# LunaJang/Metabuli_work

Hardware: AMD Instinct MI355X
Metric: reads/sec classified (150bp & 10kb) vs GTDB-scale DB at 1/2/4/8 MI355X (higher is better)
Workload: dtype u64

## Files before the change

metabuli_work_amd/csrc/mtb_api.hip:

```cpp
#include <chrono>
#include <cmath>
#include <cstdio>
#include <cstring>
#include <string>
#include <vector>
#include <algorithm>
#include <memory>
#include <charconv>
#include <mutex>
#include <unordered_map>

#include "mtb_host.h"
#include "mtb_launch.h"
#include <cstdlib>

using namespace mtb;

#define HIP_TRY(x)                                                                                   \
    do {                                                                                             \
        hipError_t e_ = (x);                                                                         \
        if (e_ != hipSuccess) {                                                                      \
            set_error(std::string("HIP error ") + hipGetErrorString(e_) + " at " #x);                 \
            return e_ == hipErrorOutOfMemory ? MTB_ERR_OOM : MTB_ERR_HIP;                            \
        }                                                                                            \
    } while (0)

namespace {

struct WsBudget {
    size_t cap = 0;
    size_t used = 0;
    double grow = 1.0;
};

struct DevBuf {
    void* p = nullptr;
    size_t bytes = 0;
    WsBudget* budget = nullptr;
    hipError_t ensure(size_t need) {
        if (need <= bytes) return hipSuccess;
        static const bool trace = getenv("MTB_ALLOC_TRACE") != nullptr;
        const auto t0 = std::chrono::steady_clock::now();
        const size_t old = bytes;
        if (p) hipFree(p);
        const auto t1 = std::chrono::steady_clock::now();
        p = nullptr;
        if (budget) budget->used -= bytes;
        bytes = 0;
        size_t b = need + need / 8 + 256;
        hipError_t e = hipErrorOutOfMemory;
        if (budget && budget->grow > 1.125) {
            const size_t big = (size_t)((double)need * budget->grow) + 256;
            if (!budget->cap || budget->used + big <= budget->cap) {
                e = hipMalloc(&p, big);
                if (e == hipSuccess) b = big;
                else (void)hipGetLastError();
            }
        }
        if (e != hipSuccess) {
            if (budget && budget->cap && budget->used + b > budget->cap) return hipErrorOutOfMemory;
            e = hipMalloc(&p, b);
        }
        if (e == hipSuccess) bytes = b;
        if (e == hipSuccess && budget) budget->used += b;
        if (trace) {
            const auto t2 = std::chrono::steady_clock::now();
            const double f = std::chrono::duration<double>(t1 - t0).count(), m = std::chrono::duration<double>(t2 - t1).count();
            if (f + m > 0.02) fprintf(stderr, "[alloc] %.3f GB -> %.3f GB: free %.3f s, malloc %.3f s\n", old * 1e-9, b * 1e-9, f, m);
        }
        return e;
    }
    void release() {
        if (!p) return;
        hipFree(p);
        p = nullptr;
        if (budget) budget->used -= bytes;
        bytes = 0;
    }
    DevBuf() = default;
    DevBuf(const DevBuf&) = delete;
    DevBuf& operator=(const DevBuf&) = delete;
    ~DevBuf() { release(); }
    template <typename T>
    T* as() const { return (T*)p; }
};

struct DbArrays {
    int device = 0;
    std::vector<void*> own;
    ~DbArrays() {
        hipSetDevice(device);
        for (void* p : own)
            if (p) hipFree(p);
    }
};

}

struct mtb_ctx {
    int device = 0;
    mtb_params par{};
    hipStream_t stream = nullptr;
    bool ownStream = false;
    HostTables tables{};
    uint64_t D = 0;
    DbRec* db = nullptr;
    bool borrowedDb = false;
    std::shared_ptr<DbArrays> dbArrays;
    uint64_t* dirMem = nullptr;
    ProbeLine* lines = nullptr;
    uint64_t* lineP = nullptr;
    uint16_t* runOff = nullptr;
    ProbeExt* lineExt = nullptr;
    uint64_t* link = nullptr;
    AADir dir{};
    uint64_t rankLo = 0, rankHi = ~0ull;
    int joinMode = 0;
    uint64_t* tileRec = nullptr;
    uint32_t* tilePre = nullptr;
    uint64_t nTiles = 0;
    uint32_t sweepNom = 2048;
    uint32_t sweepLdsCap = ~0u;
    bool sweepSmall = false;
    bool filterThreadMajor = false;
    int sweepPersist = 1;
    uint32_t matchWinCap = ~0u;
    bool directJoin = true;
    bool directRetry = false;
    int pruneAfter = 2;
    int bigGroups = 1;
    bool fuseFilter = true;
    bool radixDigits = true;
    bool radixAtomicFirst = false;
    int binnedSort = 0;
    uint64_t binRcForce = 0;
    bool binDigits = true;
    bool uniformUnits = true;
    uint32_t upr = 0;
    uint64_t binHost[kSortBins] = {};
    bool noFilter = false;
    uint32_t spillShift = 0;
    bool sparse = false;
    uint32_t maxW = 0;
    int sortLoFine = kQuerySortLoFine;
    bool forceGeneric = false;
    bool segsortGlobal = false;
    uint32_t mergeSeg = 0;
    int waveTaxon = -1;
    int emulateAll = 0;
    bool pruneCompact = true;
    bool noAlias = false;
    uint64_t aliasBytes = 0;
    int32_t* spOf = nullptr;
    int32_t maxTax = 0;
    int32_t *tNodeOf = nullptr, *tNodeTax = nullptr, *tParent = nullptr, *tDepth = nullptr, *tSpParent = nullptr;
    uint8_t* tFlags = nullptr;
    uint32_t cladePerMatch = 2;
    std::vector<int32_t> hNodeOf;
    std::vector<std::string> hRank;
    HostTaxonomy hTax;
    mutable std::vector<std::string> lineage;
    mutable std::once_flag lineageOnce;
    std::shared_ptr<void> pipelineCache;
    mutable mtb::TaxText taxText;
    mutable std::once_flag taxTextOnce;
    WsBudget ws;
    DevBuf seq1, off1, seq2, off2, meta, reserve, slotOff, qlen, scanTmp;
    DevBuf keysA, valsA, keysB, valsB, radixCounts, radixOffs;
    DevBuf readCnt, mOff, matches, matchesSorted, segScratch, maxSeg, errFlag;
    DevBuf ordKA, ordVA, ordKB, ordVB, matchWin, unitRead, unitInfo, mStage, mRank, mTotal, mDirect, ovFlag, waveList, waveCount, devStats;
    DevBuf qFrom, probeStats;
    DevBuf longList, longCnt;
    DevBuf qStart;
    uint32_t longCap = 0;
    DevBuf chunkIn, chunkCnt, chunkSrcOff;
    DevBuf liveCnt, liveOff;
    DevBuf segLen;
    DevBuf sizeLists;
    DevBuf digA, digB;
    DevBuf binCnt, binTab;
    DevBuf maskOut1, maskOut2, maskProb, maskScale;
    DevBuf readLens;
    DevBuf readCnt64;
    uint64_t liveM = 0;
    double openS[8] = {0, 0, 0, 0, 0, 0, 0, 0};
    static constexpr int kNumStats = 20;
    uint64_t stats[kNumStats] = {};
    uint32_t chunkC = 1;
    uint64_t stageRegion = 0;
    uint64_t spillCap = 0;
    DevBuf emMap, emCnt, emScratch, emPacked, emCnt32, emOff;
    bool emValid = false;
    bool emPackedValid = false;
    std::vector<mtb_em_map> emHost;
    std::vector<uint32_t> spKmers;
    std::string dbDir;
    DevBuf local, paths, comb, conn, spScore, spKeep,
        gFlag, sFlag, pathCnt, gScan, sScan, gStart, sStart, clade, tcPool, tcLen, tcOff, tcOut, results;
    uint32_t nReads = 0;
    uint64_t Q = 0, M = 0, nTaxcnt = 0;
    uint64_t Qall = 0;
    double presentShare = 0.5;
    const uint64_t* qKeys = nullptr;
    const uint32_t* qSlots = nullptr;
    bool keepStages = false;
    bool probed = false;
    bool matchOnly = false;
    float stageMs[5] = {0, 0, 0, 0, 0};
    hipEvent_t ev[6]{};
    static constexpr int kNumKern = 7;
    float kernMs[kNumKern] = {0, 0, 0, 0, 0, 0, 0};
    hipEvent_t kev[2 * kNumKern]{};
};

static std::vector<DevBuf*> batch_bufs(mtb_ctx* c);

static void bind_workspace(mtb_ctx* c, size_t cap) {
    c->ws.cap = cap;
    if (const char* e = getenv("MTB_WORKSPACE_CAP")) {
        char* end = nullptr;
        double v = strtod(e, &end);
        const char u = end ? *end : 0;
        v *= u == 'G' || u == 'g' ? 1e9 : u == 'M' || u == 'm' ? 1e6 : u == 'K' || u == 'k' ? 1e3 : 1.0;
        c->ws.cap = v > 0 ? (size_t)v : 0;
    }
    for (DevBuf* b : batch_bufs(c)) b->budget = &c->ws;
}

static void free_db(mtb_ctx* c) {
    if (c->dbArrays) {
        c->dbArrays.reset();
        c->db = nullptr;
        c->dirMem = nullptr;
        c->lines = nullptr;
        c->lineP = nullptr;
        c->runOff = nullptr;
        c->lineExt = nullptr;
        c->link = nullptr;
        return;
    }
    if (c->borrowedDb) c->db = nullptr;
    void* ptrs[] = {c->db, c->dirMem, c->lines, c->lineP, c->runOff, c->lineExt, c->link, c->spOf, c->tNodeOf, c->tNodeTax, c->tParent, c->tDepth, c->tSpParent, c->tFlags};
    for (void* p : ptrs)
        if (p) hipFree(p);
    c->db = nullptr;
    c->dirMem = nullptr;
    c->lines = nullptr;
    c->lineP = nullptr;
    c->runOff = nullptr;
    c->lineExt = nullptr;
    c->link = nullptr;
}

template <typename T>
static hipError_t upload(T** dst, const std::vector<T>& v, hipStream_t s) {
    hipError_t e = hipMalloc((void**)dst, std::max<size_t>(1, v.size()) * sizeof(T));
    if (e != hipSuccess) return e;
    if (!v.empty()) e = hipMemcpyAsync(*dst, v.data(), v.size() * sizeof(T), hipMemcpyHostToDevice, s);
    return e;
}

static int validate_params(const mtb_params* p) {
    if (p->reduced_aa) { set_error("reduced-AA DBs (ReducedKmerMatcher) are out of scope"); return MTB_ERR_UNSUPPORTED; }
    if (p->em && p->db_parts > 1) { set_error("--em needs the whole DB in one context"); return MTB_ERR_UNSUPPORTED; }
    if (p->mask_mode && !(p->mask_prob > 0.0f && p->mask_prob <= 1.0f)) { set_error("mask_prob must be in (0, 1]"); return MTB_ERR_ARG; }
    if (p->kmer_format != 1 && p->kmer_format != 2) { set_error("kmer_format must be 1 or 2"); return MTB_ERR_UNSUPPORTED; }
    if (p->syncmer && p->kmer_format != 2) { set_error("syncmer requires kmer_format 2"); return MTB_ERR_UNSUPPORTED; }
    if (p->syncmer && (p->smer_len < 1 || p->smer_len > 8)) { set_error("smer_len must be in [1, 8]"); return MTB_ERR_ARG; }
    if (p->seq_mode < 1 || p->seq_mode > 3) { set_error("seq_mode must be 1, 2 or 3"); return MTB_ERR_ARG; }
    return MTB_OK;
}

static double since(std::chrono::steady_clock::time_point& t) {
    const auto now = std::chrono::steady_clock::now();
    const double d = std::chrono::duration<double>(now - t).count();
    t = now;
    return d;
}

static int decode_db_chunked(mtb_ctx* c, HostDb& db, uint32_t mask, hipStream_t s) {
    const uint64_t nDiff = db.nDiff, D = c->D;
    uint64_t W = 1ull << 30;
    if (const char* e = getenv("MTB_DECODE_CHUNK_WORDS")) W = std::max<uint64_t>(8, strtoull(e, nullptr, 10));
    W = std::max<uint64_t>(std::min(W, nDiff), 1);
    DevBuf dDiff, dFlag, dIdx, dTmp, dVal, dInfo;
    HIP_TRY(dDiff.ensure(W * sizeof(uint16_t)));
    HIP_TRY(dFlag.ensure(W * sizeof(uint32_t)));
    HIP_TRY(dIdx.ensure((W + 2) * sizeof(uint64_t)));
    HIP_TRY(dTmp.ensure(scan_tmp_elems(W) * sizeof(uint64_t)));
    HIP_TRY(dVal.ensure(W * sizeof(uint64_t)));
    HIP_TRY(dInfo.ensure(W * sizeof(uint32_t)));
    auto a0 = std::chrono::steady_clock::now();
    HIP_TRY(hipMalloc(&c->db, (D + kDbPad) * sizeof(DbRec)));
    c->openS[7] = since(a0);
    const bool fromFile = !db.diffFile.empty();
    double upS = 0;
    auto l0 = std::chrono::steady_clock::now();
    StageLanes lanes(c->device);
    upS += since(l0);
    uint64_t w0 = 0, k0 = 0, carry = 0, seen = 0;
    HIP_TRY(hipStreamSynchronize(s));
    while (w0 < nDiff) {
        const uint64_t n = std::min(W, nDiff - w0);
        auto u0 = std::chrono::steady_clock::now();
        const bool got = fromFile ? read_to_device(db.diffFile, dDiff.p, n * sizeof(uint16_t), w0 * sizeof(uint16_t), &lanes)
                                  : upload_to_device(db.diffP + w0, dDiff.p, n * sizeof(uint16_t), &lanes);
        if (!got) return MTB_ERR_IO;
        upS += since(u0);
        uint64_t lastTerm = 0, lastValue = 0;
        const uint64_t terms = decode_diff_chunk(dDiff.as<uint16_t>(), n, carry, dVal.as<uint64_t>(),
                                                 dFlag.as<uint32_t>(), dIdx.as<uint64_t>(), dTmp.p, &lastTerm,
                                                 &lastValue, s);
        HIP_TRY(hipGetLastError());
        const bool lastChunk = w0 + n == nDiff;
        if (terms == 0) {
            set_error("diffIdx ends mid k-mer");
            return MTB_ERR_DB;
        }
        if (lastChunk && lastTerm != n - 1) {
            set_error("diffIdx ends mid k-mer");
            return MTB_ERR_DB;
        }
        seen += terms;
        if (seen <= D) {
            u0 = std::chrono::steady_clock::now();
            const bool gotInfo = fromFile ? read_to_device(db.infoFile, dInfo.p, terms * sizeof(uint32_t),
                                                           k0 * sizeof(uint32_t), &lanes)
                                          : upload_to_device(db.infoP + k0, dInfo.p, terms * sizeof(uint32_t), &lanes);
            if (!gotInfo) return MTB_ERR_IO;
            upS += since(u0);
            launch_mask_info(dInfo.as<uint32_t>(), terms, mask, s);
            if (c->par.kmer_format == 2) launch_to_rank_form(dVal.as<uint64_t>(), terms, s);
            launch_pack_db(dVal.as<uint64_t>(), dInfo.as<uint32_t>(), terms, c->db + k0, s);
            HIP_TRY(hipStreamSynchronize(s));
            k0 += terms;
        }
        carry = lastValue;
        w0 += lastTerm + 1;
    }
    if (seen != D) {
        set_error("diffIdx k-mer count " + std::to_string(seen) + " != info entries " + std::to_string(D));
        return MTB_ERR_DB;
    }
    c->openS[0] += upS;
    return MTB_OK;
}

static int open_into(mtb_ctx* c, HostDb& db, const mtb_params* par, int device, const mtb_db_resident* res,
                     double readS, std::chrono::steady_clock::time_point t0) {
    auto tp = t0;
    c->device = device;
// ... 163 lines not shown
        if (!res->records || res->n_kmers < 2) { set_error("resident DB needs >= 2 k-mers"); return MTB_ERR_DB; }
    } else {
        if (!check_db(db)) return MTB_ERR_DB;
        if (db.nInfo < 2) { set_error("DB has fewer than 2 k-mers"); return MTB_ERR_DB; }
        if (par->db_parts > 1 && !slice_db_part(db, par->db_part, par->db_parts)) return MTB_ERR_DB;
    }
    mtb_ctx* c = new mtb_ctx();
    rc = open_into(c, db, par, device, res, readS, t0);
    if (rc != MTB_OK) {
        const std::string msg = mtb_last_error();
        mtb_close(c);
        set_error(msg);
        return rc;
    }
    *out = c;
    return MTB_OK;
}

extern "C" {

int mtb_open(const char* db_dir, const mtb_params* par, int device, mtb_ctx** out) {
    if (!db_dir || !par || !out) { set_error("null argument"); return MTB_ERR_ARG; }
    HostDb db;
    const auto t0 = std::chrono::steady_clock::now();
    if (!load_db_files(db_dir, db, par->db_parts <= 1)) return MTB_ERR_IO;
    const double readS = std::chrono::duration<double>(std::chrono::steady_clock::now() - t0).count();
    const int rc = open_common(db, par, device, out, nullptr, readS);
    if (rc == MTB_OK) (*out)->dbDir = db_dir;
    return rc;
}

int mtb_open_host(const mtb_db_host* h, const mtb_params* par, int device, mtb_ctx** out) {
    if (!h || !par || !out) { set_error("null argument"); return MTB_ERR_ARG; }
    HostDb db;
    if (par->db_parts > 1) {
        db.diffIdx.assign(h->diff_idx, h->diff_idx + h->n_diff_idx);
        db.info.assign(h->info, h->info + h->n_info);
        db.use_vectors();
    } else {
        db.diffP = h->diff_idx;
        db.nDiff = h->n_diff_idx;
        db.infoP = h->info;
        db.nInfo = h->n_info;
    }
    if (h->split) db.split.assign(h->split, h->split + 3 * h->n_split);
    db.taxIdList.assign(h->taxid_list, h->taxid_list + h->n_taxid_list);
    std::vector<std::string> ranks(h->n_nodes), names(h->n_nodes);
    for (uint64_t i = 0; i < h->n_nodes; i++) {
        ranks[i] = h->rank_pool + h->rank_off[i];
        if (h->name_pool) names[i] = h->name_pool + h->name_off[i];
    }
    if (!build_taxonomy(h->node_taxid, h->node_parent, h->n_nodes, ranks, names, h->merged_old, h->merged_new,
                        h->n_merged, db.tax) ||
        !build_species_map(db))
        return MTB_ERR_DB;
    return open_common(db, par, device, out);
}

int mtb_open_resident(const mtb_db_resident* r, const mtb_db_host* h, const mtb_params* par, int device,
                      mtb_ctx** out) {
    if (!r || !h || !par || !out) { set_error("null argument"); return MTB_ERR_ARG; }
    HostDb db;
    db.taxIdList.assign(h->taxid_list, h->taxid_list + h->n_taxid_list);
    std::vector<std::string> ranks(h->n_nodes), names(h->n_nodes);
    for (uint64_t i = 0; i < h->n_nodes; i++) {
        ranks[i] = h->rank_pool + h->rank_off[i];
        if (h->name_pool) names[i] = h->name_pool + h->name_off[i];
    }
    if (!build_taxonomy(h->node_taxid, h->node_parent, h->n_nodes, ranks, names, h->merged_old, h->merged_new,
                        h->n_merged, db.tax) ||
        !build_species_map(db))
        return MTB_ERR_DB;
    return open_common(db, par, device, out, r);
}

int mtb_clone(const mtb_ctx* src, mtb_ctx** out) {
    if (!src || !out) { set_error("null argument"); return MTB_ERR_ARG; }
    mtb_ctx* c = new mtb_ctx();
    c->device = src->device;
    c->par = src->par;
    c->tables = src->tables;
    HIP_TRY(hipSetDevice(c->device));
    HIP_TRY(hipStreamCreateWithFlags(&c->stream, hipStreamNonBlocking));
    c->ownStream = true;
    for (auto& e : c->ev) HIP_TRY(hipEventCreate(&e));
    for (auto& e : c->kev) HIP_TRY(hipEventCreate(&e));
    c->dbArrays = src->dbArrays;
    c->D = src->D;
    c->db = src->db;
    c->borrowedDb = src->borrowedDb;
    c->dirMem = src->dirMem;
    c->lines = src->lines;
    c->lineP = src->lineP;
    c->runOff = src->runOff;
    c->lineExt = src->lineExt;
    c->link = src->link;
    c->dir = src->dir;
    c->rankLo = src->rankLo;
    c->rankHi = src->rankHi;
    c->spOf = src->spOf;
    c->maxTax = src->maxTax;
    c->tNodeOf = src->tNodeOf;
    c->tNodeTax = src->tNodeTax;
    c->tParent = src->tParent;
    c->tDepth = src->tDepth;
    c->tSpParent = src->tSpParent;
    c->tFlags = src->tFlags;
    c->cladePerMatch = src->cladePerMatch;
    c->hNodeOf = src->hNodeOf;
    c->hRank = src->hRank;
    c->hTax = src->hTax;
    c->dbDir = src->dbDir;
    c->spKmers = src->spKmers;
    c->joinMode = src->joinMode;
    c->sweepNom = src->sweepNom;
    c->sweepLdsCap = src->sweepLdsCap;
    c->sweepSmall = src->sweepSmall;
    c->filterThreadMajor = src->filterThreadMajor;
    c->sweepPersist = src->sweepPersist;
    c->matchWinCap = src->matchWinCap;
    c->directJoin = src->directJoin;
    c->directRetry = src->directRetry;
    c->pruneAfter = src->pruneAfter;
    c->bigGroups = src->bigGroups;
    c->fuseFilter = src->fuseFilter;
    c->presentShare = src->presentShare;
    c->spillShift = src->spillShift;
    c->sortLoFine = src->sortLoFine;
    c->forceGeneric = src->forceGeneric;
    c->segsortGlobal = src->segsortGlobal;
    c->mergeSeg = src->mergeSeg;
    c->waveTaxon = src->waveTaxon;
    c->emulateAll = src->emulateAll;
    c->pruneCompact = src->pruneCompact;
    c->noAlias = src->noAlias;
    c->noFilter = src->noFilter;
    c->radixDigits = src->radixDigits;
    c->radixAtomicFirst = src->radixAtomicFirst;
    c->binnedSort = src->binnedSort;
    c->binRcForce = src->binRcForce;
    c->binDigits = src->binDigits;
    c->uniformUnits = src->uniformUnits;
    bind_workspace(c, src->ws.cap);
    *out = c;
    return MTB_OK;
}

#define MTB_BATCH_BUFS(X) \
    X(seq1) X(off1) X(seq2) X(off2) X(meta) X(reserve) X(slotOff) X(qlen) X(scanTmp) X(keysA) X(valsA) X(keysB) \
    X(valsB) X(radixCounts) X(radixOffs) X(readCnt) X(mOff) X(matches) X(matchesSorted) X(segScratch) X(maxSeg) \
    X(errFlag) X(ordKA) X(ordVA) X(ordKB) X(ordVB) X(matchWin) X(unitRead) X(unitInfo) X(waveList) X(waveCount) \
    X(devStats) X(mStage) X(mRank) X(mDirect) X(ovFlag) X(mTotal) X(qFrom) X(probeStats) X(longList) X(longCnt) \
    X(qStart) X(chunkIn) X(chunkCnt) X(chunkSrcOff) X(liveCnt) X(liveOff) X(segLen) X(sizeLists) X(digA) \
    X(digB) X(binCnt) X(binTab) X(local) X(paths) X(comb) X(conn) X(spScore) X(spKeep) X(gFlag) X(sFlag) \
    X(pathCnt) X(gScan) X(sScan) X(gStart) X(sStart) X(clade) X(tcPool) X(tcLen) X(tcOff) X(tcOut) X(results) \
    X(emMap) X(emCnt) X(emScratch) X(emPacked) X(emCnt32) X(emOff) X(maskOut1) X(maskOut2) X(maskProb) \
    X(maskScale) X(readLens) X(readCnt64)
static std::vector<DevBuf*> batch_bufs(mtb_ctx* c) {
#define MTB_BUF_PTR(n) &c->n,
    return {MTB_BATCH_BUFS(MTB_BUF_PTR)};
#undef MTB_BUF_PTR
}

static const char* const* batch_buf_names() {
#define MTB_BUF_NAME(n) #n,
    static const char* const names[] = {MTB_BATCH_BUFS(MTB_BUF_NAME)};
#undef MTB_BUF_NAME
    return names;
}

void mtb_close(mtb_ctx* c) {
    if (!c) return;
    hipSetDevice(c->device);
    if (c->stream) hipStreamSynchronize(c->stream);
    free_db(c);
    if (c->tileRec) hipFree(c->tileRec);
    if (c->tilePre) hipFree(c->tilePre);
    c->pipelineCache.reset();
    hipSetDevice(c->device);
    for (DevBuf* b : batch_bufs(c)) b->release();
    for (auto& e : c->ev)
        if (e) hipEventDestroy(e);
    for (auto& e : c->kev)
        if (e) hipEventDestroy(e);
    if (c->ownStream && c->stream) hipStreamDestroy(c->stream);
    delete c;
}

int mtb_set_stream(mtb_ctx* c, void* stream) {
    if (!c) return MTB_ERR_ARG;
    if (c->ownStream && c->stream) hipStreamDestroy(c->stream);
    if (stream) {
        c->stream = (hipStream_t)stream;
        c->ownStream = false;
    } else {
        HIP_TRY(hipStreamCreateWithFlags(&c->stream, hipStreamNonBlocking));
        c->ownStream = true;
    }
    return MTB_OK;
}

uint64_t mtb_db_kmers(const mtb_ctx* c) { return c ? c->D : 0; }

uint64_t mtb_workspace_bytes(const mtb_ctx* c) { return c ? c->ws.used : 0; }

int mtb_open_phases(const mtb_ctx* c, double* sec, int n) {
    if (!c || !sec) return MTB_ERR_ARG;
    for (int i = 0; i < n && i < 8; i++) sec[i] = c->openS[i];
    return MTB_OK;
}

int mtb_set_workspace_cap(mtb_ctx* c, uint64_t bytes) {
    if (!c) return MTB_ERR_ARG;
    c->ws.cap = bytes;
    return MTB_OK;
}

int mtb_release_workspace(mtb_ctx* c) {
    if (!c) return MTB_ERR_ARG;
    mtb::ctx_release_workspace(c);
    void* p = nullptr;
    if (hipMalloc(&p, 64u << 20) == hipSuccess) hipFree(p);
    return hipDeviceSynchronize() == hipSuccess ? MTB_OK : MTB_ERR_HIP;
}

int mtb_ctx_device(const mtb_ctx* c) { return c ? c->device : 0; }

}

static AssignArgs assign_args(const mtb_params& p) {
    AssignArgs a;
    a.em = p.em ? 1 : 0;
    a.kmerFormat = p.kmer_format;
    if (p.syncmer) {
        a.dnaShift = (8 - p.smer_len) * 3;
        a.maxCodonShift = 8 - p.smer_len;
    } else {
        a.dnaShift = 3;
        a.maxCodonShift = 1;
    }
    a.denominator = (p.seq_mode == 1 || p.seq_mode == 2) ? 100 : 1000;
    a.minConsCnt = p.min_cons_cnt;
    a.minConsCntEuk = p.min_cons_cnt_euk;
    a.accessionLevel = p.accession_level;
    a.minScore = p.min_score;
    a.minSpScore = p.min_sp_score;
    a.tieRatio = p.tie_ratio;
    a.generic = 0;
    return a;
}

static int assign_stage(mtb_ctx* c, uint32_t n, bool keep) {
    hipStream_t s = c->stream;
    HIP_TRY(c->errFlag.ensure(sizeof(int)));
    const uint64_t M = c->M;
    AssignArgs a = assign_args(c->par);
    a.generic = c->forceGeneric ? 1 : 0;
    a.waveTaxon = c->waveTaxon;
    a.bigGroups = c->bigGroups;
    a.emulateAll = c->emulateAll;
    if (a.dnaShift <= 0) { set_error("syncmer smer_len 8 gives a zero dnaShift"); return MTB_ERR_ARG; }
    HIP_TRY(c->readCnt.ensure(sizeof(uint32_t) * (n + 1)));
    const uint64_t Mc = std::max<uint64_t>(M, 1);
    HIP_TRY(c->results.ensure(sizeof(mtb_result) * std::max<uint32_t>(n, 1)));
    HIP_TRY(c->matchesSorted.ensure(sizeof(mtb_match) * Mc));
    HIP_TRY(c->maxSeg.ensure(sizeof(uint32_t)));
    launch_max_seg(c->mOff.as<uint64_t>(), n, c->maxSeg.as<uint32_t>(), s);
    uint32_t maxSeg = 0;
    HIP_TRY(hipMemcpyAsync(&maxSeg, c->maxSeg.p, sizeof(uint32_t), hipMemcpyDeviceToHost, s));
    HIP_TRY(hipStreamSynchronize(s));
    const bool prune = !keep && !c->forceGeneric;
    if (maxSeg > kSegSortLds || c->forceGeneric || c->segsortGlobal || (c->mergeSeg && maxSeg > c->mergeSeg))
        HIP_TRY(c->segScratch.ensure(6 * sizeof(uint64_t) * Mc));
    const bool compact = prune && maxSeg > kSegSortRegs && !c->segsortGlobal && c->pruneCompact;
    if (compact) HIP_TRY(c->segLen.ensure(sizeof(uint32_t) * (n + 1)));
    if (maxSeg > 128) HIP_TRY(c->sizeLists.ensure(sizeof(uint32_t) * (4 * (size_t)n + 4)));
    c->keepStages = !prune;
    HIP_TRY(c->liveCnt.ensure(sizeof(uint32_t) * (n + 1)));
    HIP_TRY(c->liveOff.ensure(sizeof(uint64_t) * (n + 1)));
    HIP_TRY(c->scanTmp.ensure(sizeof(uint64_t) * scan_tmp_elems(n + 1)));
    HIP_TRY(hipEventRecord(c->kev[10], s));
    if (c->sparse && (!prune || (maxSeg > kSegSortSparse && !compact) || c->segsortGlobal ||
                      (c->mergeSeg && maxSeg > c->mergeSeg))) {
        launch_compact_segments(c->mDirect.as<SegMatch>(), c->slotOff.as<uint64_t>(), c->chunkC,
                                c->mOff.as<uint64_t>(), n, c->matches.as<mtb_match>(), c->spillShift, s,
                                c->stats[13] ? 2 : 0);
        c->sparse = false;
    }
    HIP_TRY(launch_segsort(c->matches.as<mtb_match>(), c->mOff.as<uint64_t>(), n, Mc, c->matchesSorted.as<mtb_match>(),
                           c->segScratch.as<uint64_t>(), maxSeg, c->forceGeneric || c->segsortGlobal,
                           prune ? c->liveCnt.as<uint32_t>() : nullptr, c->mergeSeg,
                           prune_min_matches(a.minConsCnt, a.minConsCntEuk, a.maxCodonShift), s,
                           c->sparse ? c->mDirect.as<SegMatch>() : nullptr, c->slotOff.as<uint64_t>(),
                           c->chunkC | c->spillShift << 16,
                           compact ? c->segLen.as<uint32_t>() : nullptr,
                           c->maxSeg.as<uint32_t>(), c->pruneAfter, maxSeg > 128 ? c->sizeLists.as<uint32_t>() : nullptr));
    c->sparse = false;
    const mtb_match* kIn = c->matchesSorted.as<mtb_match>();
    const uint64_t* kOff = c->mOff.as<uint64_t>();
    uint64_t kM = M;
    if (prune) {
        exclusive_scan_u32(c->liveCnt.as<uint32_t>(), n, c->liveOff.as<uint64_t>(), c->scanTmp.p, s);
        HIP_TRY(hipMemcpyAsync(&kM, c->liveOff.as<uint64_t>() + n, sizeof(uint64_t), hipMemcpyDeviceToHost, s));
        launch_pack_live(c->matchesSorted.as<mtb_match>(), c->mOff.as<uint64_t>(), c->liveOff.as<uint64_t>(), n,
                         c->matches.as<mtb_match>(), c->errFlag.as<int>(), s);
        HIP_TRY(hipStreamSynchronize(s));
        if (kM > M) { set_error("internal error: K5 kept more matches than it sorted"); return MTB_ERR_INTERNAL; }
        kIn = c->matches.as<mtb_match>();
        kOff = c->liveOff.as<uint64_t>();
    }
    c->liveM = kM;
    c->stats[11] = kM;
    const uint64_t Kc = std::max<uint64_t>(kM, 1);
    const uint64_t Mn = std::max<uint64_t>(Kc, n);
    std::vector<std::pair<char*, size_t>> dead;
    if (!c->noAlias) {
        std::vector<DevBuf*> d = {&c->mDirect, &c->segScratch, &c->mStage, &c->mRank, &c->matchWin, &c->chunkIn};
        if (prune) {
            for (DevBuf* b : {&c->matchesSorted, &c->keysA, &c->valsA, &c->keysB, &c->valsB}) d.push_back(b);
        } else {
            d.push_back(&c->matches);
        }
        for (DevBuf* b : d)
            if (b->p && b->bytes >= (1u << 20)) dead.push_back({b->as<char>(), b->bytes});
        std::sort(dead.begin(), dead.end(), [](auto& a, auto& b) { return a.second > b.second; });
    }
    struct Need {
        DevBuf* own;
        uint64_t bytes;
        void* p;
    };
    Need need[] = {{&c->local, path_bytes() * Kc, nullptr},
                   {&c->paths, path_bytes() * Kc, nullptr},
                   {&c->comb, path_bytes() * Kc, nullptr},
                   {&c->conn, Kc, nullptr},
                   {&c->spScore, sizeof(float) * Kc, nullptr},
                   {&c->spKeep, Kc, nullptr},
                   {&c->waveList, sizeof(uint64_t) * Kc, nullptr},
                   {&c->gFlag, sizeof(uint32_t) * (Kc + 1), nullptr},
                   {&c->pathCnt, sizeof(uint32_t) * (Kc + 1), nullptr},
                   {&c->sFlag, std::max<uint64_t>(sizeof(uint32_t) * (Kc + 1), run_index_tmp_bytes(Kc)), nullptr},
                   {&c->gScan, sizeof(uint64_t) * (Kc + 1), nullptr},
                   {&c->sScan, sizeof(uint64_t) * (Kc + 1), nullptr},
                   {&c->gStart, sizeof(uint64_t) * (Kc + 1), nullptr},
                   {&c->sStart, sizeof(uint64_t) * (Kc + 1), nullptr},
                   {&c->clade, clade_bytes() * Kc * c->cladePerMatch, nullptr},
                   {&c->tcPool, sizeof(mtb_taxcnt) * Kc, nullptr},
                   {&c->ordKA, sizeof(uint64_t) * (Mn + 1), nullptr},
                   {&c->ordVA, sizeof(uint64_t) * (Mn + 1), nullptr},
                   {&c->ordKB, sizeof(uint64_t) * (Mn + 1), nullptr},
                   {&c->ordVB, sizeof(uint64_t) * (Mn + 1), nullptr}};
    std::vector<Need*> order;
    for (Need& x : need) order.push_back(&x);
    std::stable_sort(order.begin(), order.end(), [](Need* a, Need* b) { return a->bytes > b->bytes; });
    c->aliasBytes = 0;
    for (Need* x : order) {
        const size_t b = (x->bytes + 255) & ~(size_t)255;
        for (auto& r : dead)
            if (r.second >= b) {
                x->p = r.first;
                r.first += b;
                r.second -= b;
                c->aliasBytes += b;
                break;
            }
        if (!x->p) {
            HIP_TRY(x->own->ensure(x->bytes));
            x->p = x->own->p;
        }
    }
    HIP_TRY(c->waveCount.ensure(sizeof(uint32_t)));
    HIP_TRY(hipEventRecord(c->kev[11], s));
    HIP_TRY(hipEventRecord(c->kev[12], s));
    HIP_TRY(c->radixCounts.ensure(sizeof(uint32_t) * radix_counts_elems(Mn + 1)));
    HIP_TRY(c->radixOffs.ensure(sizeof(uint64_t) * (radix_counts_elems(Mn + 1) + 1)));
    HIP_TRY(c->scanTmp.ensure(sizeof(uint64_t) * scan_tmp_elems(radix_counts_elems(Mn + 1) + n + Mn + 2)));
    TaxDevice t{c->tNodeOf, c->tNodeTax, c->tParent, c->tDepth, c->tFlags, c->tSpParent, c->maxTax};
    AssignScratch sc{need[0].p,
                     need[1].p,
                     need[2].p,
                     (uint8_t*)need[3].p,
                     (uint32_t*)need[7].p,
                     (uint32_t*)need[9].p,
                     (uint32_t*)need[8].p,
                     (uint64_t*)need[10].p,
                     (uint64_t*)need[11].p,
                     (uint64_t*)need[12].p,
                     (uint64_t*)need[13].p,
                     (float*)need[4].p,
                     (uint64_t*)need[6].p,
                     c->waveCount.as<uint32_t>(),
                     (uint8_t*)need[5].p,
                     c->scanTmp.p,
                     (uint64_t*)need[16].p,
                     (uint64_t*)need[17].p,
                     (uint64_t*)need[18].p,
                     (uint64_t*)need[19].p,
                     c->radixCounts.as<uint32_t>(),
                     c->radixOffs.as<uint64_t>(),
                     need[14].p,
                     c->cladePerMatch};
    mtb_taxcnt* tcPool = (mtb_taxcnt*)need[15].p;
    c->stats[3] = M;
    c->stats[4] = maxSeg;
    launch_assign(kIn, kOff, c->qlen.as<uint32_t>(), n, kM, a, t, sc, tcPool,
                  c->results.as<mtb_result>(), c->devStats.as<unsigned long long>(), c->stats + 5, s);
    HIP_TRY(hipEventRecord(c->kev[13], s));
    HIP_TRY(c->tcLen.ensure(sizeof(uint32_t) * (n + 1)));
    HIP_TRY(c->tcOff.ensure(sizeof(uint64_t) * (n + 1)));
    launch_taxcnt_len(c->results.as<mtb_result>(), n, c->tcLen.as<uint32_t>(), s);
    exclusive_scan_u32(c->tcLen.as<uint32_t>(), n, c->tcOff.as<uint64_t>(), c->scanTmp.p, s);
    uint64_t NT = 0;
    HIP_TRY(hipMemcpyAsync(&NT, c->tcOff.as<uint64_t>() + n, sizeof(uint64_t), hipMemcpyDeviceToHost, s));
    HIP_TRY(hipStreamSynchronize(s));
    HIP_TRY(c->tcOut.ensure(sizeof(mtb_taxcnt) * std::max<uint64_t>(NT, 1)));
    launch_compact_taxcnt(tcPool, kOff, c->results.as<mtb_result>(), c->tcOff.as<uint64_t>(), n,
                          c->tcOut.as<mtb_taxcnt>(), s);
    c->nTaxcnt = NT;
    c->emValid = false;
    c->emPackedValid = false;
    if (c->par.em) {
        const uint64_t nS = std::max<uint64_t>(c->stats[7], 1);
        HIP_TRY(c->emScratch.ensure(8 * nS));
        HIP_TRY(c->emMap.ensure(8 * (uint64_t)kEmTop * std::max<uint32_t>(n, 1)));
        HIP_TRY(c->emCnt.ensure(std::max<uint32_t>(n, 1)));
        launch_em_top(kIn, kOff, n, sc, c->results.as<mtb_result>(), c->emScratch.p, c->emMap.p,
                      c->emCnt.as<uint8_t>(), s);
        HIP_TRY(hipGetLastError());
        c->emValid = true;
    }
    return MTB_OK;
}

static int join_stage(mtb_ctx* c, const uint8_t* dSeq1, const uint64_t* dOff1, const uint8_t* dSeq2,
                      const uint64_t* dOff2, uint32_t n, uint64_t U, uint32_t C, uint64_t R, uint64_t Rc) {
    hipStream_t s = c->stream;
    const bool probe = c->probed;
    const bool filt = c->lines && (!c->noFilter || probe);
    const bool fused = filt && !probe && c->fuseFilter;
    if (!fused) {
        HIP_TRY(c->keysA.ensure(8 * Rc));
        HIP_TRY(c->valsA.ensure(4 * Rc));
        HIP_TRY(c->keysB.ensure(8 * Rc));
        HIP_TRY(c->valsB.ensure(4 * Rc));
    }
    HIP_TRY(c->radixCounts.ensure(sizeof(uint32_t) * radix_counts_elems(Rc)));
    HIP_TRY(c->radixOffs.ensure(sizeof(uint64_t) * (radix_counts_elems(Rc) + 1)));
    HIP_TRY(c->scanTmp.ensure(sizeof(uint64_t) * scan_tmp_elems(radix_counts_elems(Rc) + n + 1)));
    HIP_TRY(c->mTotal.ensure(sizeof(unsigned long long) * kStageRegions));
    HIP_TRY(c->probeStats.ensure(sizeof(unsigned long long) * kProbeStatsLen));
    HIP_TRY(hipMemsetAsync(c->probeStats.p, 0, sizeof(unsigned long long) * kProbeStatsLen, s));
    HIP_TRY(hipEventRecord(c->kev[0], s));
    if (!fused)
        launch_extract(dSeq1, dOff1, dSeq2, dOff2, c->meta.as<ReadMeta>(), c->slotOff.as<uint64_t>(),
                       c->unitRead.as<uint32_t>(), U, C, c->tables, c->par.kmer_format, c->par.syncmer,
                       c->par.smer_len, c->keysA.as<uint64_t>(), c->unitInfo.as<uint64_t>(), s, c->upr);
    HIP_TRY(hipEventRecord(c->kev[1], s));
    uint64_t Q = R;
    const uint64_t* qk = c->keysA.as<uint64_t>();
    const uint32_t* qi = nullptr;
    const uint64_t* qf = nullptr;
    HIP_TRY(hipEventRecord(c->kev[2], s));
    const bool digits = fused && c->radixDigits && c->sortLoFine == kQuerySortLo;
    uint64_t binRc = 0;
    if (fused) {
        uint64_t cap = std::min<uint64_t>(R, (uint64_t)((double)R * c->presentShare) + 4096);
        bool binned = digits && c->binnedSort && (c->binnedSort == 2 || cap >= (1ull << 22));
        for (int pass = 0; pass < 2 && binned; pass++) {
            uint64_t rc = c->binRcForce ? c->binRcForce : (cap + cap / 16) / kSortBins + 256;
            rc = (rc + 63) / 64 * 64;
            const uint64_t slots = rc * kSortBins;
            HIP_TRY(c->keysB.ensure(8 * slots));
            HIP_TRY(c->valsB.ensure(4 * slots));
            HIP_TRY(c->digA.ensure(slots));
            HIP_TRY(c->binCnt.ensure(sizeof(unsigned long long) * kSortBins));
            Q = launch_extract_filter(dSeq1, dOff1, dSeq2, dOff2, c->meta.as<ReadMeta>(), c->slotOff.as<uint64_t>(),
                                      c->unitRead.as<uint32_t>(), U, C, c->tables, c->par.kmer_format, c->par.syncmer,
                                      c->par.smer_len, c->unitInfo.as<uint64_t>(), c->lines, c->keysB.as<uint64_t>(),
                                      c->valsB.as<uint32_t>(), c->mTotal.as<unsigned long long>(), c->rankLo,
                                      c->rankHi, &c->Qall, slots, false, s,
                                      c->binDigits ? c->digA.as<uint8_t>() : nullptr,
                                      c->binCnt.as<unsigned long long>(), rc, c->binHost, c->upr);
            HIP_TRY(hipGetLastError());
            if (R) c->presentShare = std::max(c->presentShare, std::min(1.0, 1.125 * (double)Q / (double)R));
            bool over = false;
            for (int r = 0; r < kSortBins; r++) over |= c->binHost[r] > rc;
            if (!over) {
                binRc = rc;
                break;
            }
            c->stats[15]++;
            cap = std::min<uint64_t>(R, Q + Q / 8);
            binned = false;
        }
        for (int pass = 0; pass < 2 && !binRc; pass++) {
            HIP_TRY(c->keysB.ensure(8 * cap));
            HIP_TRY(c->valsB.ensure(4 * cap));
            if (digits) HIP_TRY(c->digA.ensure(cap));
            cap = std::min<uint64_t>(c->keysB.bytes / 8, c->valsB.bytes / 4);
            if (digits) cap = std::min<uint64_t>(cap, c->digA.bytes);
            Q = launch_extract_filter(dSeq1, dOff1, dSeq2, dOff2, c->meta.as<ReadMeta>(), c->slotOff.as<uint64_t>(),
                                      c->unitRead.as<uint32_t>(), U, C, c->tables, c->par.kmer_format, c->par.syncmer,
                                      c->par.smer_len, c->unitInfo.as<uint64_t>(), c->lines, c->keysB.as<uint64_t>(),
                                      c->valsB.as<uint32_t>(), c->mTotal.as<unsigned long long>(), c->rankLo,
                                      c->rankHi, &c->Qall, cap, c->filterThreadMajor, s,
                                      digits ? c->digA.as<uint8_t>() : nullptr, nullptr, 0, nullptr, c->upr, c->link);
            HIP_TRY(hipGetLastError());
            if (Q == ~0ull) {
                set_error("internal error: K1F sequence stage overflow");
                return MTB_ERR_INTERNAL;
            }
            if (R) c->presentShare = std::max(c->presentShare, std::min(1.0, 1.125 * (double)Q / (double)R));
            if (Q <= cap) break;
            cap = std::min<uint64_t>(R, Q + Q / 8);
            c->stats[15]++;
        }
        HIP_TRY(c->keysA.ensure(8 * std::max<uint64_t>(Q, 1)));
        HIP_TRY(c->valsA.ensure(4 * std::max<uint64_t>(Q, 1)));
        if (digits) HIP_TRY(c->digB.ensure(std::max<uint64_t>(Q, 16)));
        qk = c->keysB.as<uint64_t>();
        qi = c->valsB.as<uint32_t>();
    } else if (filt) {
        if (probe) HIP_TRY(c->qFrom.ensure(8 * Rc + 8 * kDbPad));
        Q = launch_filter(c->keysA.as<uint64_t>(), R, c->lines, c->keysB.as<uint64_t>(), c->valsB.as<uint32_t>(),
                          probe ? c->qFrom.as<uint64_t>() : nullptr, c->mTotal.as<unsigned long long>(), c->rankLo,
                          c->rankHi, &c->Qall, s);
        qk = c->keysB.as<uint64_t>();
        qi = c->valsB.as<uint32_t>();
        qf = c->qFrom.as<uint64_t>();
    }
    HIP_TRY(hipEventRecord(c->kev[3], s));
    HIP_TRY(hipEventRecord(c->ev[1], s));
    HIP_TRY(hipEventRecord(c->kev[4], s));
    const bool sweepJoin = c->joinMode == 3 && !probe && c->directJoin && !c->forceGeneric;
    const int sortLo = !sweepJoin && unstaged_join(c->lines != nullptr, c->D, Q, std::min<uint32_t>(c->matchWinCap, 3072))
                           ? c->sortLoFine : kQuerySortLo;
    if (!probe) {
        bool inB = false;
        if (binRc) {
            HIP_TRY(c->binTab.ensure(sizeof(uint64_t) * std::max<uint64_t>(radix_binned_tiles(c->binHost, binRc), 1)));
            const uint64_t rcn = radix_counts_elems(Q) + 256ull * kSortBins;
            HIP_TRY(c->radixCounts.ensure(sizeof(uint32_t) * rcn));
            HIP_TRY(c->radixOffs.ensure(sizeof(uint64_t) * (rcn + 1)));
            HIP_TRY(c->scanTmp.ensure(sizeof(uint64_t) * scan_tmp_elems(rcn + n + 1)));
            Q = radix_sort_binned(c->keysB.as<uint64_t>(), c->valsB.as<uint32_t>(), c->keysA.as<uint64_t>(),
                                  c->valsA.as<uint32_t>(), c->binHost, c->binCnt.as<unsigned long long>(), binRc,
                                  kQuerySortLo, kQuerySortHi, c->radixCounts.as<uint32_t>(),
                                  c->radixOffs.as<uint64_t>(), c->scanTmp.p, c->binTab.as<uint64_t>(), &inB, s,
                                  c->binDigits ? c->digA.as<uint8_t>() : nullptr, c->digB.as<uint8_t>());
            qk = inB ? c->keysA.as<uint64_t>() : c->keysB.as<uint64_t>();
            qi = inB ? c->valsA.as<uint32_t>() : c->valsB.as<uint32_t>();
        } else if (filt) {
            const bool dg = digits && sortLo == kQuerySortLo;
            Q = radix_sort_pairs(c->keysB.as<uint64_t>(), c->valsB.as<uint32_t>(), c->keysA.as<uint64_t>(),
                                 c->valsA.as<uint32_t>(), Q, sortLo, kQuerySortHi, false, false,
// ... 1175 lines not shown
```

metabuli_work_amd/csrc/mtb_assign.hip:

```cpp
#include <algorithm>
#include <vector>

#include "mtb_launch.h"
#include "mtb_stdsort.h"

namespace mtb {

struct Path {
    int start, end;
    float score;
    int hd, depth;
    uint32_t sm, em;
};

__device__ __forceinline__ void match_key(const mtb_match& m, uint64_t& hi, uint64_t& lo) {
    hi = ((uint64_t)m.species_id << 32) | ((uint64_t)info_frame(m.qinfo) << 29) | (info_pos(m.qinfo) & 0x1FFFFFFFu);
    lo = ((uint64_t)m.hamming << 56) | ((uint64_t)(m.dna_encoding & 0xFFFFFFu) << 32) | m.target_id;
}

__device__ __forceinline__ bool key_gt(uint64_t ah, uint64_t al, uint64_t bh, uint64_t bl) {
    return ah > bh || (ah == bh && al > bl);
}

constexpr int kSmallSeg = 512;
// ... 1351 lines not shown
        for (long i = threadIdx.x; i < (long)surv; i += kLargeThreads) io[base + i] = stage[base + i];
    if (threadIdx.x == 0) segLen[r] = surv;
}

__global__ void __launch_bounds__(256) k_max_seg_len(const uint32_t* __restrict__ segLen, uint32_t n,
                                                     uint32_t* __restrict__ out) {
    uint32_t v = 0;
#pragma unroll
    for (uint32_t k = 0; k < kMaxPer; k++)
        if (max_elem(k) < n && segLen[max_elem(k)] != kSegSkip) v = max(v, segLen[max_elem(k)]);
    block_max_to(v, out);
}

constexpr int kSizeClasses = 4;
constexpr int kSizeListReads = 1024;

__global__ void __launch_bounds__(256) k_size_lists(const uint64_t* __restrict__ mOff, const uint32_t* __restrict__ segLen,
                                                    uint32_t nReads, uint32_t maxSeg, uint32_t* __restrict__ lists,
                                                    uint32_t* __restrict__ counts) {
    __shared__ uint32_t sCnt[kSizeClasses], sBase[kSizeClasses];
    if (threadIdx.x < kSizeClasses) sCnt[threadIdx.x] = 0;
    __syncthreads();
    constexpr int kPer = kSizeListReads / 256;
    int cls[kPer];
    uint32_t at[kPer];
#pragma unroll
    for (int k = 0; k < kPer; k++) {
        const uint32_t r = blockIdx.x * kSizeListReads + k * 256 + threadIdx.x;
        cls[k] = -1;
        at[k] = 0;
        if (r < nReads) {
            const long n = seg_len(mOff, segLen, r);
            cls[k] = n > (long)maxSeg ? -1 : n > kMidSeg ? 3 : n > kSmallSeg ? 2 : n > 256 ? 1 : n > 128 ? 0 : -1;
        }
        if (cls[k] >= 0) at[k] = atomicAdd(&sCnt[cls[k]], 1u);
    }
    __syncthreads();
    if (threadIdx.x < kSizeClasses)
        sBase[threadIdx.x] = sCnt[threadIdx.x] ? atomicAdd(&counts[threadIdx.x], sCnt[threadIdx.x]) : 0u;
    __syncthreads();
#pragma unroll
    for (int k = 0; k < kPer; k++)
        if (cls[k] >= 0)
            lists[(uint64_t)cls[k] * nReads + sBase[cls[k]] + at[k]] = blockIdx.x * kSizeListReads + k * 256 + threadIdx.x;
}

static hipError_t launch_sorts(const mtb_match* in, const uint64_t* mOff, uint32_t nReads, uint64_t M, mtb_match* out,
                               uint64_t* gScratch, uint32_t maxSeg, uint32_t* liveCnt, long chunk, uint32_t pm,
                               const uint32_t* segLen, hipStream_t s, const SegMatch* seg, const uint64_t* inOff,
                               uint32_t inC, int mode, uint32_t* lists) {
    k_segsort_small<<<nReads, 64, 0, s>>>(in, mOff, seg, inOff, inC, nReads, out, liveCnt, pm, segLen);
    if (maxSeg <= 128) return hipGetLastError();
    static const bool useLists = !(getenv("MTB_SIZE_LISTS") && atoi(getenv("MTB_SIZE_LISTS")) == 0);
    if (!useLists || !lists) {
#define MTB_REGS(E, M) k_segsort_regs<E, M><<<nReads, 64, 0, s>>>(in, mOff, seg, inOff, inC, nReads, out, liveCnt, pm, segLen, nullptr)
        if (!liveCnt) mode = 3;
        if (maxSeg > 128) {
            if (mode == 1) MTB_REGS(4, 1);
            else if (mode == 0) MTB_REGS(4, 0);
            else if (mode == 3) MTB_REGS(4, 3);
            else MTB_REGS(4, 2);
        }
        if (maxSeg > 256) {
            if (mode == 1) MTB_REGS(8, 1);
            else if (mode == 0) MTB_REGS(8, 0);
            else if (mode == 3) MTB_REGS(8, 3);
            else MTB_REGS(8, 2);
        }
#undef MTB_REGS
        if (maxSeg > kSmallSeg)
            k_segsort_mid<<<nReads, kMidThreads, 0, s>>>(in, mOff, nReads, out, liveCnt, chunk, pm, segLen, seg, inOff,
                                                         inC, mode == 2 ? 1 : mode == 4 ? 2 : 0, nullptr);
        if (maxSeg > kMidSeg)
            k_segsort_large<<<nReads, kLargeThreads, 0, s>>>(in, mOff, nReads, M, out, gScratch, 0, liveCnt, chunk, pm,
                                                             segLen, mode == 2 ? 1 : mode == 4 ? 2 : 0, nullptr);
        MTB_HIP_RET(hipGetLastError());
        if (maxSeg > chunk) return launch_merge_path(in, mOff, nReads, M, out, gScratch, liveCnt, chunk, pm, segLen, s);
        return hipSuccess;
    }
    uint32_t* dCnt = lists + (size_t)kSizeClasses * nReads;
    uint32_t cnt[kSizeClasses] = {0, 0, 0, 0};
    hipError_t e = hipMemsetAsync(dCnt, 0, sizeof(cnt), s);
    if (e == hipSuccess) {
        k_size_lists<<<(nReads + kSizeListReads - 1) / kSizeListReads, 256, 0, s>>>(mOff, segLen, nReads, maxSeg, lists, dCnt);
        e = hipGetLastError();
    }
    if (e == hipSuccess) e = hipMemcpyAsync(cnt, dCnt, sizeof(cnt), hipMemcpyDeviceToHost, s);
    if (e == hipSuccess) e = hipStreamSynchronize(s);
    const uint32_t* list4 = lists;
    const uint32_t* list8 = lists + (size_t)nReads;
    const uint32_t* listMid = lists + 2 * (size_t)nReads;
    const uint32_t* listLarge = lists + 3 * (size_t)nReads;
    static const size_t segPad = getenv("MTB_SEGSORT_PAD") ? (size_t)atoi(getenv("MTB_SEGSORT_PAD")) : 0;
#define MTB_REGS(E, M, N, L) \
    k_segsort_regs<E, M><<<N, 64, segPad, s>>>(in, mOff, seg, inOff, inC, nReads, out, liveCnt, pm, segLen, L)
    if (!liveCnt) mode = 3;
    if (e == hipSuccess && cnt[0]) {
        if (mode == 1) MTB_REGS(4, 1, cnt[0], list4);
        else if (mode == 0) MTB_REGS(4, 0, cnt[0], list4);
        else if (mode == 3) MTB_REGS(4, 3, cnt[0], list4);
        else MTB_REGS(4, 2, cnt[0], list4);
    }
    if (e == hipSuccess && cnt[1]) {
        if (mode == 1) MTB_REGS(8, 1, cnt[1], list8);
        else if (mode == 0) MTB_REGS(8, 0, cnt[1], list8);
        else if (mode == 3) MTB_REGS(8, 3, cnt[1], list8);
        else MTB_REGS(8, 2, cnt[1], list8);
    }
#undef MTB_REGS
    if (e == hipSuccess && cnt[2])
        k_segsort_mid<<<cnt[2], kMidThreads, 0, s>>>(in, mOff, nReads, out, liveCnt, chunk, pm, segLen, seg, inOff, inC,
                                                     mode == 2 ? 1 : mode == 4 ? 2 : 0, listMid);
    if (e == hipSuccess && cnt[3])
        k_segsort_large<<<cnt[3], kLargeThreads, 0, s>>>(in, mOff, nReads, M, out, gScratch, 0, liveCnt, chunk, pm,
                                                         segLen, mode == 2 ? 1 : mode == 4 ? 2 : 0, listLarge);
    if (e == hipSuccess) e = hipGetLastError();
    MTB_HIP_RET(e);
    if (maxSeg > chunk) return launch_merge_path(in, mOff, nReads, M, out, gScratch, liveCnt, chunk, pm, segLen, s);
    return hipSuccess;
}

hipError_t launch_segsort(const mtb_match* in, const uint64_t* mOff, uint32_t nReads, uint64_t M, mtb_match* out,
                          uint64_t* gScratch, uint32_t maxSeg, bool global, uint32_t* liveCnt, uint32_t mergeSeg,
                          uint32_t pm, hipStream_t s, const SegMatch* seg, const uint64_t* inOff, uint32_t inC,
                          uint32_t* segLen, uint32_t* maxTmp, int after, uint32_t* lists) {
    pm = max(pm, 2u);
    if (nReads == 0) return hipSuccess;
    const bool thin = liveCnt && segLen;
    if (seg && (global || (maxSeg > kSegSortSparse && !thin))) return hipErrorInvalidValue;
    const long chunk = std::max<long>(kSmallSeg, std::min<long>(mergeSeg ? mergeSeg : kBlockSeg, kBlockSeg));
    if (global) {
        k_segsort_large<<<nReads, kLargeThreads, 0, s>>>(in, mOff, nReads, M, out, gScratch, 1, liveCnt, chunk, pm,
                                                         nullptr, 0, nullptr);
        return hipGetLastError();
    }
    const long thinAbove = std::min<long>(chunk, kMidSeg);
    if (!liveCnt || maxSeg <= (uint32_t)thinAbove || !segLen)
        return launch_sorts(in, mOff, nReads, M, out, gScratch, maxSeg, liveCnt, chunk, pm, nullptr, s, seg, inOff, inC, after,
                            lists);
    MTB_HIP_RET(launch_sorts(in, mOff, nReads, M, out, gScratch, (uint32_t)thinAbove, liveCnt, chunk, pm, nullptr, s,
                             seg, inOff, inC, after, lists));
    mtb_match* io = const_cast<mtb_match*>(in);
    k_thin_big<<<nReads, kLargeThreads, 0, s>>>(io, out, mOff, nReads, thinAbove, pm, segLen, seg, inOff, inC);
    MTB_HIP_RET(hipMemsetAsync(maxTmp, 0, sizeof(uint32_t), s));
    k_max_seg_len<<<max_blocks(nReads), 256, 0, s>>>(segLen, nReads, maxTmp);
    uint32_t maxSurv = 0;
    MTB_HIP_RET(hipMemcpyAsync(&maxSurv, maxTmp, sizeof(uint32_t), hipMemcpyDeviceToHost, s));
    MTB_HIP_RET(hipStreamSynchronize(s));
    if (maxSurv == 0) return hipSuccess;
    return launch_sorts(in, mOff, nReads, M, out, gScratch, maxSurv, liveCnt, chunk, pm, segLen, s, nullptr, nullptr, 0, after,
                        lists);
}

__global__ void __launch_bounds__(256) k_pack_live(const mtb_match* __restrict__ in, const uint64_t* __restrict__ mOff,
                                                   const uint64_t* __restrict__ liveOff, uint32_t nReads,
                                                   mtb_match* __restrict__ out, int* __restrict__ err) {
    const uint32_t r = blockIdx.x * 4 + threadIdx.x / 64;
    const uint32_t lane = threadIdx.x & 63;
    if (r >= nReads) return;
    const uint64_t live = liveOff[r + 1] - liveOff[r];
    if (live > mOff[r + 1] - mOff[r] || liveOff[r + 1] > mOff[nReads]) {
        if (lane == 0) atomicExch(err, kErrLiveCount);
        return;
    }
    const uint64_t* src = reinterpret_cast<const uint64_t*>(in + mOff[r]);
    uint64_t* dst = reinterpret_cast<uint64_t*>(out + liveOff[r]);
    for (uint64_t w = lane; w < live * 3; w += 64) dst[w] = src[w];
}

void launch_pack_live(const mtb_match* in, const uint64_t* mOff, const uint64_t* liveOff, uint32_t nReads,
                      mtb_match* out, int* err, hipStream_t s) {
    if (nReads) k_pack_live<<<(nReads + 3) / 4, 256, 0, s>>>(in, mOff, liveOff, nReads, out, err);
}

__global__ void __launch_bounds__(256) k_max_seg(const uint64_t* __restrict__ off, uint32_t n, uint32_t* __restrict__ out) {
    uint32_t v = 0;
#pragma unroll
    for (uint32_t k = 0; k < kMaxPer; k++)
        if (max_elem(k) < n) v = max(v, (uint32_t)min<uint64_t>(off[max_elem(k) + 1] - off[max_elem(k)], 0xFFFFFFFFull));
    block_max_to(v, out);
}

void launch_max_seg(const uint64_t* off, uint32_t n, uint32_t* out, hipStream_t s) {
    hipMemsetAsync(out, 0, sizeof(uint32_t), s);
    if (n) k_max_seg<<<max_blocks(n), 256, 0, s>>>(off, n, out);
}

void launch_max_u32(const uint32_t* x, uint32_t n, uint32_t* out, hipStream_t s) {
    hipMemsetAsync(out, 0, sizeof(uint32_t), s);
    if (n) k_max_u32<<<max_blocks(n), 256, 0, s>>>(x, n, out);
}

struct TaxView {
    const int32_t* nodeOf;
    const int32_t* nodeTax;
    const int32_t* parent;
    const int32_t* depth;
    const uint8_t* flags;
    const int32_t* spParent;
    int32_t maxTax;
    __device__ bool exists(int32_t t) const { return t >= 0 && t <= maxTax && nodeOf[t] >= 0; }
    __device__ int lca_node(int i, int j) const {
        if (i == 0 || j == 0) return 0;
        while (i != j) {
            int di = depth[i], dj = depth[j];
            if (di >= dj) i = parent[i];
            if (dj >= di) j = parent[j];
        }
        return i;
    }
    __device__ int32_t lca(int32_t a, int32_t b) const {
        if (!exists(a)) return b;
        if (!exists(b)) return a;
        return nodeTax[lca_node(nodeOf[a], nodeOf[b])];
    }
};

struct AssignCfg {
    int kmerFormat, dnaShift, maxCodonShift, denominator, minConsCnt, minConsCntEuk, accessionLevel;
    float minScore, minSpScore, tieRatio;
    int generic;
    int emulateAll;
    int em;
};

struct Clade {
    int32_t tax, parentTax;
    uint32_t count;
    int32_t removed;
};




__global__ void k_group_keys(const uint64_t* __restrict__ gStart, uint64_t nG, uint64_t* __restrict__ keys,
                             uint64_t* __restrict__ vals, uint32_t* __restrict__ pathCnt, uint32_t minGroup) {
    const uint64_t g = (uint64_t)blockIdx.x * blockDim.x + threadIdx.x;
    if (g >= nG) return;
    const uint64_t n = gStart[g + 1] - gStart[g];
    if (n < minGroup) {
        pathCnt[g] = 0;
        keys[g] = kSentinel;
    } else {
        keys[g] = g;
    }
    vals[g] = 0;
}


constexpr int kRegPos = 4;
constexpr uint64_t kBigGroup = 256;

struct GlobalRecs {
    const mtb_match* __restrict__ M;
    __device__ __forceinline__ uint32_t pos(uint64_t k) const { return info_pos(M[k].qinfo); }
    __device__ __forceinline__ uint32_t dna(uint64_t k) const { return M[k].dna_encoding; }
    __device__ __forceinline__ uint32_t reh(uint64_t k) const { return M[k].right_end_hamming; }
    __device__ __forceinline__ uint32_t ham(uint64_t k) const { return M[k].hamming; }
};
struct LdsRecs {
    const uint32_t* p;
    const uint32_t* dh;
    const uint16_t* rh;
    uint64_t base;
    __device__ __forceinline__ uint32_t pos(uint64_t k) const { return p[k - base]; }
    __device__ __forceinline__ uint32_t dna(uint64_t k) const { return dh[k - base] & 0xFFFFFFu; }
    __device__ __forceinline__ uint32_t reh(uint64_t k) const { return rh[k - base]; }
    __device__ __forceinline__ uint32_t ham(uint64_t k) const { return dh[k - base] >> 24; }
};

template <typename R>
__device__ __forceinline__ bool match_paths_regs(const R& M, uint64_t start, uint64_t end,
                                                 const AssignCfg& cfg, int minDepth, bool fwd,
                                                 Path* __restrict__ P, uint64_t& nPout, bool emitLone = false) {
    Path cp[kRegPos], np[kRegPos];
    uint32_t cd[kRegPos], nd[kRegPos], nr[kRegPos];
    bool cc[kRegPos];
    int nc = 0, nn = 0;
    uint64_t nP = start;
    uint64_t k = start;
    uint32_t currPos = M.pos(k);
    while (k < end) {
        if (M.pos(k) != currPos) break;
        if (nc == kRegPos) return false;
        const uint32_t mreh = M.reh(k), mham = M.ham(k), mdna = M.dna(k);
#pragma unroll
        for (int x = 0; x < kRegPos; x++)
            if (x == nc) {
                cp[x].start = (int)currPos;
                cp[x].end = (int)currPos + 23;
                cp[x].score = score_fields(mreh, 8, false);
                cp[x].hd = (int)mham;
                cp[x].depth = 1;
                cp[x].sm = cp[x].em = (uint32_t)k;
                cd[x] = mdna;
                cc[x] = false;
            }
        nc++;
        k++;
    }
    const bool stepped = k < end;
    while (k < end) {
        const uint32_t nextPos = M.pos(k);
        nn = 0;
        while (k < end) {
            if (M.pos(k) != nextPos) break;
            if (nn == kRegPos) return false;
            const uint32_t mreh = M.reh(k), mham = M.ham(k), mdna = M.dna(k);
#pragma unroll
            for (int x = 0; x < kRegPos; x++)
                if (x == nn) {
                    np[x].start = (int)nextPos;
                    np[x].end = (int)nextPos + 23;
                    np[x].score = score_fields(mreh, 8, false);
                    np[x].hd = (int)mham;
                    np[x].depth = 1;
                    np[x].sm = np[x].em = (uint32_t)k;
                    nd[x] = mdna;
                    nr[x] = mreh;
                }
            nn++;
            k++;
        }
        const int shift = (int)((nextPos - currPos) / 3);
        if (shift > 0 && shift <= cfg.maxCodonShift) {
            const uint32_t sh = kBitsPerCodon * (uint32_t)shift;
            const uint32_t lowMask = (1u << (kTotalDnaBits - sh)) - 1u;
#pragma unroll
            for (int x = 0; x < kRegPos; x++) {
                if (x >= nn) continue;
                const float inc = score_fields(nr[x], shift, false);
                const int hinc = ham_fields(nr[x], shift, false);
                bool found = false;
                float bestScore = 0.0f;
                Path bp{};
#pragma unroll
                for (int y = 0; y < kRegPos; y++) {
                    if (y >= nc) continue;
                    if (consecutive(cd[y], nd[x], sh, lowMask, fwd, cfg.kmerFormat)) {
                        cc[y] = true;
                        if (cp[y].score > bestScore) { found = true; bestScore = cp[y].score; bp = cp[y]; }
                    }
                }
                if (found) {
                    np[x].start = bp.start;
                    np[x].score = bp.score + inc;
                    np[x].hd = bp.hd + hinc;
                    np[x].depth = bp.depth + shift;
                    np[x].sm = bp.sm;
                }
            }
        }
#pragma unroll
        for (int y = 0; y < kRegPos; y++)
            if (y < nc && !cc[y] && cp[y].depth >= minDepth) P[nP++] = cp[y];
        if (k == end) {
#pragma unroll
            for (int x = 0; x < kRegPos; x++)
                if (x < nn && np[x].depth >= minDepth) P[nP++] = np[x];
        }
#pragma unroll
        for (int x = 0; x < kRegPos; x++) {
            cp[x] = np[x];
            cd[x] = nd[x];
            cc[x] = false;
        }
        nc = nn;
        currPos = nextPos;
    }
    if (!stepped && emitLone)
#pragma unroll
        for (int y = 0; y < kRegPos; y++)
            if (y < nc && cp[y].depth >= minDepth) P[nP++] = cp[y];
    nPout = nP;
    return true;
}

template <typename R>
__device__ uint64_t match_paths_serial(const R& M, uint64_t start, uint64_t end,
                                       const AssignCfg& cfg, int minDepth, bool fwd, Path* __restrict__ L,
                                       Path* __restrict__ P, uint8_t* __restrict__ conn, bool emitLone) {
    for (uint64_t x = start; x < end; x++) conn[x] = 0;
    uint64_t nP = start;
    uint64_t k = start;
    uint64_t currPos = M.pos(start);
    bool stepped = false;
    auto initPath = [&](uint64_t idx) {
        Path p;
        p.start = (int)M.pos(idx);
        p.end = p.start + 23;
        p.score = score_fields(M.reh(idx), 8, false);
        p.hd = (int)M.ham(idx);
        p.depth = 1;
        p.sm = p.em = (uint32_t)idx;
        L[idx] = p;
    };
    uint64_t curS = k;
    while (k < end && M.pos(k) == currPos) { initPath(k); ++k; }
    uint64_t curE = k;
    while (k < end) {
        const uint32_t nextPos = M.pos(k);
        const uint64_t nxS = k;
        while (k < end && M.pos(k) == nextPos) { initPath(k); ++k; }
        const uint64_t nxE = k;
        stepped = true;
        const int shift = (int)(((uint64_t)nextPos - currPos) / 3);
        if (shift > 0 && shift <= cfg.maxCodonShift) {
            const uint32_t sh = kBitsPerCodon * (uint32_t)shift;
            const uint32_t lowMask = (1u << (kTotalDnaBits - sh)) - 1u;
            for (uint64_t nx = nxS; nx < nxE; nx++) {
                const uint32_t nreh = M.reh(nx);
                const float inc = score_fields(nreh, shift, false);
                const int hinc = ham_fields(nreh, shift, false);
                int64_t best = -1;
                float bestScore = 0.0f;
                const uint32_t dn = M.dna(nx);
                for (uint64_t cu = curS; cu < curE; cu++) {
                    const uint32_t dc = M.dna(cu);
                    if (consecutive(dc, dn, sh, lowMask, fwd, cfg.kmerFormat)) {
                        conn[cu] = 1;
                        if (L[cu].score > bestScore) { best = (int64_t)cu; bestScore = L[cu].score; }
                    }
                }
                if (best >= 0) {
                    const Path bp = L[best];
                    Path& np = L[nx];
                    np.start = bp.start;
                    np.score = bp.score + inc;
                    np.hd = bp.hd + hinc;
                    np.depth = bp.depth + shift;
                    np.sm = bp.sm;
                }
            }
        }
        for (uint64_t cu = curS; cu < curE; cu++)
            if (!conn[cu] && L[cu].depth >= minDepth) P[nP++] = L[cu];
        if (k == end)
            for (uint64_t nx = nxS; nx < nxE; nx++)
                if (L[nx].depth >= minDepth) P[nP++] = L[nx];
        curS = nxS;
        curE = nxE;
        currPos = nextPos;
    }
    if (!stepped && emitLone)
        for (uint64_t cu = start; cu < end; cu++)
            if (L[cu].depth >= minDepth) P[nP++] = L[cu];
    return nP;
}

template <typename R>
__device__ __forceinline__ void match_paths_group(const R& recs, const mtb_match* __restrict__ M, uint64_t g,
                                                  uint64_t start, uint64_t end, const AssignCfg& cfg,
                                                  const TaxView& tax, Path* __restrict__ L, Path* __restrict__ P,
                                                  uint8_t* __restrict__ conn, uint32_t* __restrict__ pathCnt) {
    const int32_t sp = (int32_t)M[start].species_id;
    const uint32_t curFrame = info_frame(M[start].qinfo);
    int minDepth = cfg.minConsCnt;
    if (tax.exists(sp) && (tax.flags[tax.nodeOf[sp]] & 1u)) minDepth = cfg.minConsCntEuk;
    const bool fwd = curFrame < 3;
    {
        uint64_t nPr = start;
        if (!cfg.generic && match_paths_regs(recs, start, end, cfg, minDepth, fwd, P, nPr)) {
            pathCnt[g] = (uint32_t)(nPr - start);
            return;
        }
    }
    const uint64_t nP = match_paths_serial(recs, start, end, cfg, minDepth, fwd, L, P, conn, false);
    pathCnt[g] = (uint32_t)(nP - start);
}

constexpr int kPathStage = 1024;

template <bool kLds, int kW>
__global__ void __launch_bounds__(64) __attribute__((amdgpu_waves_per_eu(kW))) k_match_paths(const mtb_match* __restrict__ M, const uint64_t* __restrict__ gStart,
                                                    const uint64_t* __restrict__ order, uint64_t nWork, AssignCfg cfg,
                                                    TaxView tax, Path* __restrict__ L, Path* __restrict__ P,
                                                    uint8_t* __restrict__ conn, uint32_t* __restrict__ pathCnt,
                                                    uint64_t* __restrict__ bigList, uint32_t* __restrict__ bigCount) {
    __shared__ uint32_t sPos[kLds ? kPathStage : 1], sDh[kLds ? kPathStage : 1];
    __shared__ uint16_t sReh[kLds ? kPathStage : 1];
    const uint64_t w0 = (uint64_t)blockIdx.x * 64;
    const uint64_t i = w0 + threadIdx.x;
    const uint64_t wLast = min(w0 + 63, nWork - 1);
    const uint64_t spanLo = kLds ? gStart[(uint32_t)order[w0]] : 0, spanHi = kLds ? gStart[(uint32_t)order[wLast] + 1] : 0;
    const bool staged = kLds && spanHi - spanLo <= (uint64_t)kPathStage;
    if (staged) {
        for (uint64_t k = spanLo + threadIdx.x; k < spanHi; k += 64) {
            const mtb_match m = M[k];
            sPos[k - spanLo] = info_pos(m.qinfo);
            sDh[k - spanLo] = (m.dna_encoding & 0xFFFFFFu) | ((uint32_t)m.hamming << 24);
            sReh[k - spanLo] = m.right_end_hamming;
        }
        __syncthreads();
    }
    if (i >= nWork) return;
    const uint64_t g = (uint32_t)order[i];
    const uint64_t start = gStart[g], end = gStart[g + 1];
    if (bigList && end - start >= kBigGroup) {
        bigList[atomicAdd(bigCount, 1u)] = g;
        return;
    }
    if (staged)
        match_paths_group(LdsRecs{sPos, sDh, sReh, spanLo}, M, g, start, end, cfg, tax, L, P, conn, pathCnt);
    else
        match_paths_group(GlobalRecs{M}, M, g, start, end, cfg, tax, L, P, conn, pathCnt);
}

__device__ __forceinline__ bool group_break(const mtb_match* __restrict__ M, uint64_t start, uint64_t i,
                                            int maxCodonShift) {
    if (i == start) return true;
    const uint32_t p = info_pos(M[i].qinfo), pp = info_pos(M[i - 1].qinfo);
    if (p == pp) return false;
    const int shift = (int)((p - pp) / 3);
    return !(shift > 0 && shift <= maxCodonShift);
}

__global__ void __launch_bounds__(64) k_match_paths_wave(const mtb_match* __restrict__ M,
                                                         const uint64_t* __restrict__ gStart,
                                                         const uint64_t* __restrict__ bigList, AssignCfg cfg,
                                                         TaxView tax, Path* __restrict__ L, Path* __restrict__ P,
                                                         uint8_t* __restrict__ conn, uint32_t* __restrict__ pathCnt) {
    const uint64_t g = bigList[blockIdx.x];
    const int lane = threadIdx.x;
    const uint64_t start = gStart[g], end = gStart[g + 1], n = end - start;
    const int32_t sp = (int32_t)M[start].species_id;
    int minDepth = cfg.minConsCnt;
    if (tax.exists(sp) && (tax.flags[tax.nodeOf[sp]] & 1u)) minDepth = cfg.minConsCntEuk;
    const bool fwd = info_frame(M[start].qinfo) < 3;
    const bool multi = info_pos(M[start].qinfo) != info_pos(M[end - 1].qinfo);
    uint64_t a = start + n * (uint64_t)lane / 64;
    while (a < end && !group_break(M, start, a, cfg.maxCodonShift)) a++;
    uint64_t b = __shfl_down(a, 1, 64);
    if (lane == 63) b = end;
    if (b < a) b = a;
    uint64_t cnt = 0;
    if (a < b) {
        uint64_t nPr = a;
        if (!cfg.generic && match_paths_regs(GlobalRecs{M}, a, b, cfg, minDepth, fwd, P, nPr, multi)) cnt = nPr - a;
        else cnt = match_paths_serial(GlobalRecs{M}, a, b, cfg, minDepth, fwd, L, P, conn, multi) - a;
    }
    uint64_t inc = cnt;
#pragma unroll
    for (int d = 1; d < 64; d <<= 1) {
        const uint64_t y = __shfl_up(inc, d, 64);
        if (lane >= d) inc += y;
    }
    const uint64_t off = inc - cnt, total = __shfl(inc, 63, 64);
    __syncthreads();
    for (uint64_t k = 0; k < cnt; k++) L[start + off + k] = P[a + k];
    __syncthreads();
    for (uint64_t k = lane; k < total; k += 64) P[start + k] = L[start + k];
    if (lane == 0) pathCnt[g] = (uint32_t)total;
}

__device__ __forceinline__ void trim_path(const mtb_match* __restrict__ M, Path& p, const Path& c, int ol) {
    const int range = ol / 3;
    if (p.start < c.start) {
        const uint32_t reh = M[p.em].right_end_hamming;
        p.end = c.start - 1;
        p.hd = max(0, p.hd - ham_fields(reh, range, false));
        p.score = p.score - score_fields(reh, range, false) - (float)(ol % 3);
    } else {
        const uint32_t reh = M[p.sm].right_end_hamming;
        p.start = c.end + 1;
        p.hd = max(0, p.hd - ham_fields(reh, range, true));
        p.score = p.score - score_fields(reh, range, true) - (float)(ol % 3);
    }
}

__device__ __forceinline__ void trim_path_reh(Path& p, const Path& c, int ol, uint32_t rehS, uint32_t rehE) {
    const int range = ol / 3;
    if (p.start < c.start) {
        p.end = c.start - 1;
        p.hd = max(0, p.hd - ham_fields(rehE, range, false));
        p.score = p.score - score_fields(rehE, range, false) - (float)(ol % 3);
    } else {
        p.start = c.end + 1;
        p.hd = max(0, p.hd - ham_fields(rehS, range, true));
        p.score = p.score - score_fields(rehS, range, true) - (float)(ol % 3);
    }
}

__device__ float combine_serial(const mtb_match* __restrict__ M, Path* Ps, long nP, Path* Cs) {
    stdsort::sort(Ps, Ps + nP, [](const Path& a, const Path& b) {
        if (a.score != b.score) return a.score > b.score;
        if (a.hd != b.hd) return a.hd < b.hd;
        return a.start > b.start;
    });
    long nC = 0;
    float score = 0.0f;
    for (long pi = 0; pi < nP; pi++) {
        if (nC == 0) {
            Cs[nC++] = Ps[pi];
            score += Ps[pi].score;
            continue;
        }
        bool overlapped = false;
        for (long j = 0; j < nC; j++) {
            Path& p = Ps[pi];
            const Path c = Cs[j];
            if ((p.end < c.start) || (c.end < p.start)) continue;
            const int ol = min(p.end, c.end) - max(p.start, c.start) + 1;
            if (ol == p.end - p.start + 1) { overlapped = true; break; }
            if (ol < 24) {
                trim_path(M, p, c, ol);
                continue;
            }
            overlapped = true;
            break;
        }
        if (!overlapped) {
            Cs[nC++] = Ps[pi];
            score += Ps[pi].score;
        }
    }
    return score;
}

__device__ __forceinline__ void species_score(float score, int readLength, const AssignCfg& cfg, float* spScore,
                                              uint8_t* spKeep, uint64_t s) {
    score = score / (float)readLength;
    score = (1.0f < score) ? 1.0f : score;
    spScore[s] = score;
    spKeep[s] = !(score < cfg.minScore);
}

constexpr int kWaveCombineMin = 24;
constexpr int kWaveCombineMax = 1024;

__global__ void __launch_bounds__(256) k_combine_paths(const mtb_match* __restrict__ M, const uint64_t* __restrict__ sStart,
                                                       uint64_t nS, const uint64_t* __restrict__ gScan,
                                                       const uint64_t* __restrict__ gStart,
                                                       const uint32_t* __restrict__ pathCnt,
                                                       const uint32_t* __restrict__ qlen, AssignCfg cfg,
                                                       Path* __restrict__ P, Path* __restrict__ C,
                                                       float* __restrict__ spScore, uint8_t* __restrict__ spKeep,
                                                       uint64_t* __restrict__ waveList, uint32_t* __restrict__ waveCount) {
    const uint64_t s = (uint64_t)blockIdx.x * blockDim.x + threadIdx.x;
    if (s >= nS) return;
    const uint64_t ss = sStart[s], se = sStart[s + 1];
    uint64_t w = ss;
    for (uint64_t g = gScan[ss]; gStart[g] < se; g++) {
        const uint64_t src = gStart[g];
        const uint32_t cnt = pathCnt[g];
        if (src != w)
            for (uint32_t k = 0; k < cnt; k++) P[w + k] = P[src + k];
        w += cnt;
    }
    if (w == ss) { spKeep[s] = 0; return; }
    const long nP = (long)(w - ss);
    if (!cfg.generic && nP > kWaveCombineMin && nP <= kWaveCombineMax) {
        waveList[atomicAdd(waveCount, 1u)] = ((uint64_t)nP << 32) | s;
        return;
    }
    const int readLength = (int)qlen[info_seq(M[ss].qinfo) - 1];
    species_score(combine_serial(M, P + ss, nP, C + ss), readLength, cfg, spScore, spKeep, s);
}

__global__ void __launch_bounds__(64) k_combine_wave(const mtb_match* __restrict__ M, const uint64_t* __restrict__ sStart,
                                                     const uint64_t* __restrict__ waveList,
                                                     const uint32_t* __restrict__ qlen, AssignCfg cfg,
                                                     Path* __restrict__ P, Path* __restrict__ C,
                                                     float* __restrict__ spScore, uint8_t* __restrict__ spKeep,
                                                     unsigned long long* __restrict__ stats,
                                                     const uint64_t* __restrict__ order) {
    __shared__ uint64_t kbuf[2 * kWaveCombineMax];
    uint64_t* kh = kbuf;
    uint64_t* kl = kbuf + kWaveCombineMax;
    __shared__ uint16_t qrs[kWaveCombineMax], qre[kWaveCombineMax];
    const uint64_t e = waveList[order ? order[blockIdx.x] : blockIdx.x];
    const uint64_t s = (uint32_t)e;
    const int nP = (int)(e >> 32);
    const uint64_t ss = sStart[s];
    const Path* Ps = P + ss;
    const int lane = threadIdx.x;
    const int readLength = (int)qlen[info_seq(M[ss].qinfo) - 1];
    int p2 = 2;
    while (p2 < nP) p2 <<= 1;
    for (int i = lane; i < p2; i += 64) {
        if (i < nP) {
            const Path p = Ps[i];
            kh[i] = ((uint64_t)(~__float_as_uint(p.score)) << 32) | (uint32_t)p.hd;
            kl[i] = ((uint64_t)(~(uint32_t)p.start) << 32) | (uint32_t)i;
        } else {
            kh[i] = ~0ull;
            kl[i] = ~0ull;
        }
    }
    __syncthreads();
    for (int k = 2; k <= p2; k <<= 1) {
        for (int j = k >> 1; j > 0; j >>= 1) {
            for (int t = lane; t < (p2 >> 1); t += 64) {
                const int i = ((t & ~(j - 1)) << 1) | (t & (j - 1));
                const int ixj = i + j;
                const bool up = (i & k) == 0;
                const uint64_t ah = kh[i], al = kl[i], bh = kh[ixj], bl = kl[ixj];
                if (key_gt(ah, al, bh, bl) == up) {
                    kh[i] = bh; kl[i] = bl; kh[ixj] = ah; kl[ixj] = al;
                }
            }
            __syncthreads();
        }
    }
    bool tie = false;
    for (int i = lane; i + 1 < nP; i += 64) {
        if (kh[i] != kh[i + 1] || (kl[i] >> 32) != (kl[i + 1] >> 32)) continue;
        const Path a = Ps[(uint32_t)kl[i]], b = Ps[(uint32_t)kl[i + 1]];
        tie |= a.end != b.end || M[a.sm].right_end_hamming != M[b.sm].right_end_hamming ||
               M[a.em].right_end_hamming != M[b.em].right_end_hamming;
    }
    struct EmuKey {
        float score;
        int hd, start;
        uint32_t idx;
    };
    static_assert(sizeof(EmuKey) * kWaveCombineMax == sizeof(uint64_t) * 2 * kWaveCombineMax, "emulation keys fit");
    EmuKey* K = reinterpret_cast<EmuKey*>(kbuf);
    const bool emulate = __syncthreads_or(tie || cfg.emulateAll);
    if (emulate) {
        if (lane == 0) atomicAdd(&stats[1], 1ull);
        for (int i = lane; i < nP; i += 64) {
            const Path q = Ps[i];
            K[i] = EmuKey{q.score, q.hd, q.start, (uint32_t)i};
        }
        __syncthreads();
        if (lane == 0)
            stdsort::sort(K, K + nP, [](const EmuKey& a, const EmuKey& b) {
                if (a.score != b.score) return a.score > b.score;
                if (a.hd != b.hd) return a.hd < b.hd;
                return a.start > b.start;
            });
        __syncthreads();
    }
    constexpr int kPerLane = kWaveCombineMax / 64;
    uint32_t src[kPerLane];
#pragma unroll
    for (int t = 0; t < kPerLane; t++) {
        const int i = lane + 64 * t;
        src[t] = i < nP ? (emulate ? K[i].idx : (uint32_t)kl[i]) : 0u;
    }
    __syncthreads();
    int* qs = reinterpret_cast<int*>(kh);
    int* qe = qs + kWaveCombineMax;
    float* qsc = reinterpret_cast<float*>(kl);
    int* qhd = reinterpret_cast<int*>(kl) + kWaveCombineMax;
#pragma unroll
    for (int t = 0; t < kPerLane; t++) {
        const int i = lane + 64 * t;
        if (i < nP) {
            const Path q = Ps[src[t]];
            qs[i] = q.start; qe[i] = q.end; qsc[i] = q.score; qhd[i] = q.hd;
            qrs[i] = M[q.sm].right_end_hamming;
            qre[i] = M[q.em].right_end_hamming;
        }
    }
    __syncthreads();
    constexpr int kSlots = kWaveCombineMax / 64;
    int rs[kSlots], re[kSlots];
#pragma unroll
    for (int t = 0; t < kSlots; t++) { rs[t] = 0; re[t] = -1; }
    float score = 0.0f;
    int nC = 0;
    for (int pi = 0; pi < nP; pi++) {
        Path p;
        p.start = qs[pi]; p.end = qe[pi]; p.score = qsc[pi]; p.hd = qhd[pi]; p.sm = 0; p.em = 0;
        const uint32_t rehS = qrs[pi], rehE = qre[pi];
        p.depth = 0;
        bool keep = true;
#pragma unroll
        for (int t = 0; t < kSlots; t++) {
            if (!keep || 64 * t >= nC) break;
            unsigned long long m = __ballot(64 * t + lane < nC && !(p.end < rs[t] || re[t] < p.start));
            while (keep && m) {
                const int l = __ffsll((long long)m) - 1;
                m &= m - 1;
                Path c;
                c.start = __shfl(rs[t], l, 64);
                c.end = __shfl(re[t], l, 64);
                if ((p.end < c.start) || (c.end < p.start)) continue;
                const int ol = min(p.end, c.end) - max(p.start, c.start) + 1;
                if (ol == p.end - p.start + 1) { keep = false; break; }
                if (ol < 24) { trim_path_reh(p, c, ol, rehS, rehE); continue; }
                keep = false;
            }
        }
        if (keep) {
#pragma unroll
            for (int t = 0; t < kSlots; t++)
                if (t == (nC >> 6) && lane == (nC & 63)) { rs[t] = p.start; re[t] = p.end; }
            nC++;
            score += p.score;
        }
    }
    if (lane == 0) species_score(score, readLength, cfg, spScore, spKeep, s);
}

__device__ long filter_redundant_serial(const mtb_match* __restrict__ M, uint64_t bestFirst, uint64_t bestSecond,
                                        const uint64_t* __restrict__ gScan, const uint64_t* __restrict__ gStart,
                                        uint32_t dnaShift, const TaxView& tax, mtb_taxcnt* __restrict__ tc) {
    uint32_t fc[6], fin[6], head[6];
    const mtb_match* B = M + bestFirst;
    int nf = 0;
    for (uint64_t g = gScan[bestFirst]; nf < 6 && gStart[g] < bestSecond; g++) {
        fc[nf] = (uint32_t)(gStart[g] - bestFirst);
        fin[nf] = (uint32_t)(gStart[g + 1] - bestFirst);
        nf++;
    }
#pragma unroll
    for (int f = 0; f < 6; f++) head[f] = (f < nf) ? info_pos(B[fc[f]].qinfo) / dnaShift : 0xFFFFFFFFu;
    constexpr int kRegTc = 4;
    int32_t rt[kRegTc];
    uint32_t rc[kRegTc];
    long nTc = 0;
    while (true) {
        uint32_t qmin = 0xFFFFFFFFu;
#pragma unroll
        for (int f = 0; f < 6; f++) qmin = min(qmin, head[f]);
        if (qmin == 0xFFFFFFFFu) break;
        uint32_t minH = 256;
        int32_t t = 0;
#pragma unroll
        for (int f = 0; f < 6; f++) {
            while (head[f] == qmin) {
                const mtb_match& x = B[fc[f]];
                const uint32_t h = x.hamming;
                if (h < minH) { minH = h; t = (int32_t)x.target_id; }
                else if (h == minH) t = tax.lca(t, (int32_t)x.target_id);
                fc[f]++;
                head[f] = fc[f] < fin[f] ? info_pos(B[fc[f]].qinfo) / dnaShift : 0xFFFFFFFFu;
            }
        }
        long e = -1;
#pragma unroll
        for (int k = 0; k < kRegTc; k++)
            if (k < nTc && rt[k] == t) e = k;
        if (e >= 0) {
#pragma unroll
            for (int k = 0; k < kRegTc; k++)
                if (k == e) rc[k]++;
            continue;
        }
        if (nTc < kRegTc) {
#pragma unroll
            for (int k = 0; k < kRegTc; k++)
                if (k == nTc) { rt[k] = t; rc[k] = 1; }
            nTc++;
            continue;
        }
        e = kRegTc;
        while (e < nTc && tc[e].tax_id != t) e++;
        if (e == nTc) { tc[nTc].tax_id = t; tc[nTc].count = 0; nTc++; }
        tc[e].count++;
    }
#pragma unroll
    for (int k = 0; k < kRegTc; k++)
        if (k < nTc) { tc[k].tax_id = rt[k]; tc[k].count = rc[k]; }
    for (long a = 1; a < nTc; a++) {
        mtb_taxcnt v = tc[a];
        long b = a;
        while (b > 0 && tc[b - 1].tax_id > v.tax_id) { tc[b] = tc[b - 1]; b--; }
        tc[b] = v;
    }
    return nTc;
}

__device__ void classify_tail(mtb_result& res, const mtb_taxcnt* __restrict__ tc, long nTc, float spTotal,
                              int32_t bestTax, int readLength, const AssignCfg& cfg, const TaxView& tax,
                              Clade* __restrict__ cl, long clCap) {
    res.taxcnt_offset = (uint32_t)0;
    res.taxcnt_len = (uint32_t)nTc;
    res.is_classified = 1;
    res.score = spTotal;
    if (spTotal < cfg.minSpScore) {
        res.classification = tax.exists(bestTax) ? tax.spParent[tax.nodeOf[bestTax]] : 0;
        return;
    }
    if (cfg.em) {
        res.classification = bestTax;
        return;
    }
    const int32_t spT = bestTax;
    long nCl = 0;
    auto findOrAdd = [&](int32_t t) -> long {
        for (long z = 0; z < nCl; z++)
            if (cl[z].tax == t) return z;
        if (nCl >= clCap) return -1;
        cl[nCl].tax = t;
        cl[nCl].parentTax = 0;
        cl[nCl].count = 0;
        cl[nCl].removed = 0;
        return nCl++;
    };
    for (long e = 0; e < nTc; e++) {
        const uint32_t c = tc[e].count;
        int node = tax.nodeOf[tc[e].tax_id];
        int32_t t = tax.nodeTax[node];
        long z = findOrAdd(t);
        if (z < 0) break;
        cl[z].count += c;
        int guard = 0;
        while (t != spT && guard++ < 64) {
            const int pnode = tax.parent[node];
            const int32_t pt = tax.nodeTax[pnode];
            cl[z].parentTax = pt;
            long pz = findOrAdd(pt);
            if (pz < 0) break;
            cl[pz].count += c;
            node = pnode;
            t = pt;
            z = pz;
        }
    }
    if (cfg.accessionLevel == 2) {
        for (long z = 0; z < nCl; z++)
            if (cl[z].tax != spT && (tax.flags[tax.nodeOf[cl[z].tax]] & 2u)) cl[z].removed = 1;
    }
    const uint32_t thr = (uint32_t)((readLength - 1) / cfg.denominator);
    int32_t cur = spT;
    for (int step = 0; step < 64; step++) {
        uint32_t maxCnt = thr;
        long nBest = 0, best = -1, nChild = 0;
        for (long z = 0; z < nCl; z++) {
            if (cl[z].tax == spT || cl[z].removed || cl[z].parentTax != cur) continue;
            nChild++;
            const uint32_t cc = cl[z].count;
            if (cc > maxCnt) { maxCnt = cc; best = z; nBest = 1; }
            else if (cc == maxCnt) { if (nBest == 0) best = z; nBest++; }
        }
        if (nChild == 0 || nBest != 1) break;
        cur = cl[best].tax;
    }
    res.classification = cur;
}

__device__ __forceinline__ mtb_result empty_result(int readLength) {
    mtb_result res;
    res.classification = 0;
    res.score = 0.0f;
    res.hamming_dist = 0;
    res.query_length = (uint32_t)readLength;
    res.taxcnt_offset = (uint32_t)0;
    res.taxcnt_len = 0;
    res.is_classified = 0;
    for (int k = 0; k < 7; k++) res.pad[k] = 0;
    return res;
}

__global__ void __launch_bounds__(256) k_choose_taxon(const mtb_match* __restrict__ M, const uint64_t* __restrict__ mOff,
                                                      const uint32_t* __restrict__ qlen, uint32_t nReads,
                                                      const uint64_t* __restrict__ sScan,
                                                      const uint64_t* __restrict__ sStart,
                                                      const uint64_t* __restrict__ gScan,
                                                      const uint64_t* __restrict__ gStart,
                                                      const float* __restrict__ spScore,
                                                      const uint8_t* __restrict__ spKeep, AssignCfg cfg, TaxView tax,
                                                      Clade* __restrict__ cladeP,
                                                      uint32_t cladePerMatch, mtb_taxcnt* __restrict__ tcP,
                                                      mtb_result* __restrict__ results) {
    const uint32_t r = blockIdx.x * blockDim.x + threadIdx.x;
    if (r >= nReads) return;
    const uint64_t base = mOff[r];
    const long n = (long)(mOff[r + 1] - base);
    const int readLength = (int)qlen[r];
    mtb_result res = empty_result(readLength);
    if (n == 0) { results[r] = res; return; }

    const uint64_t s0 = sScan[base], s1 = sScan[base + n];
    long meaningful = 0;
    float bestSpScore = 0.0f;
    uint64_t bestFirst = 0, bestSecond = 0;
    for (uint64_t s = s0; s < s1; s++) {
        if (!spKeep[s]) continue;
        const float score = spScore[s];
        if (score > 0.f) meaningful++;
        if (score > bestSpScore) { bestSpScore = score; bestFirst = sStart[s]; bestSecond = sStart[s + 1]; }
    }

    float spTotal = 0.0f;
    int32_t bestTax = 0;
    bool isLCA = false;
    if (meaningful > 0) {
        const float thr = bestSpScore * cfg.tieRatio;
        long cnt = 0;
        int lcaNode = -1;
        for (uint64_t s = s0; s < s1; s++) {
            if (!spKeep[s]) continue;
            if (spScore[s] >= thr) {
                cnt++;
                spTotal += spScore[s];
                const int32_t t = (int32_t)M[sStart[s]].species_id;
                if (cnt == 1) bestTax = t;
                if (tax.exists(t)) lcaNode = lcaNode < 0 ? tax.nodeOf[t] : tax.lca_node(lcaNode, tax.nodeOf[t]);
            }
        }
        if (cnt > 1) {
            isLCA = true;
            bestTax = lcaNode >= 0 ? tax.nodeTax[lcaNode] : 0;
            spTotal = spTotal / (float)cnt;
        }
    }
    if (spTotal == 0 || spTotal < cfg.minScore) {
        res.score = spTotal;
        results[r] = res;
        return;
    }
    if (isLCA) {
        res.is_classified = 1;
        res.classification = bestTax;
        res.score = spTotal;
        results[r] = res;
        return;
    }
    mtb_taxcnt* tc = tcP + base;
    const long nTc = filter_redundant_serial(M, bestFirst, bestSecond, gScan, gStart, (uint32_t)cfg.dnaShift, tax, tc);
    classify_tail(res, tc, nTc, spTotal, bestTax, readLength, cfg, tax, cladeP + base * cladePerMatch,
                  n * (long)cladePerMatch);
    results[r] = res;
}

constexpr int kWavePerReadMatches = 256;
constexpr int kQuotLds = 4096;
constexpr int kTcHash = 256;

__device__ __forceinline__ float wave_max_f(float x) {
#pragma unroll
    for (int d = 32; d > 0; d >>= 1) x = fmaxf(x, __shfl_xor(x, d, 64));
    return x;
}
__device__ __forceinline__ long wave_sum_l(long x) {
#pragma unroll
    for (int d = 32; d > 0; d >>= 1) x += __shfl_xor(x, d, 64);
    return x;
}

__global__ void __launch_bounds__(64) k_choose_taxon_wave(const mtb_match* __restrict__ M, const uint64_t* __restrict__ mOff,
                                                          const uint32_t* __restrict__ qlen, uint32_t nReads,
                                                          const uint64_t* __restrict__ sScan,
                                                          const uint64_t* __restrict__ sStart,
                                                          const uint64_t* __restrict__ gScan,
                                                          const uint64_t* __restrict__ gStart,
                                                          const float* __restrict__ spScore,
                                                          const uint8_t* __restrict__ spKeep, AssignCfg cfg,
                                                          TaxView tax, Clade* __restrict__ cladeP,
                                                          uint32_t cladePerMatch, mtb_taxcnt* __restrict__ tcP,
                                                          mtb_result* __restrict__ results,
                                                          const uint64_t* __restrict__ order) {
    __shared__ uint32_t qw[kQuotLds];
    __shared__ int32_t hk[kTcHash];
    __shared__ uint32_t hc[kTcHash];
    __shared__ int sFlag;
    if (blockIdx.x >= nReads) return;
    const uint32_t r = order ? (uint32_t)order[blockIdx.x] : blockIdx.x;
    const int lane = threadIdx.x;
    const uint64_t base = mOff[r];
    const long n = (long)(mOff[r + 1] - base);
    const int readLength = (int)qlen[r];
    mtb_result res = empty_result(readLength);
    if (n == 0) {
        if (lane == 0) results[r] = res;
        return;
    }
    const uint64_t s0 = sScan[base], s1 = sScan[base + n];
    long meaningful = 0;
    float bestSpScore = 0.0f;
    for (uint64_t s = s0 + lane; s < s1; s += 64) {
        if (!spKeep[s]) continue;
        const float score = spScore[s];
        meaningful += score > 0.f;
        bestSpScore = fmaxf(bestSpScore, score);
    }
    meaningful = wave_sum_l(meaningful);
    bestSpScore = wave_max_f(bestSpScore);
    float spTotal = 0.0f;
    int32_t bestTax = 0;
    bool isLCA = false;
    uint64_t bestFirst = 0, bestSecond = 0;
    if (meaningful > 0) {
        for (uint64_t c = s0; c < s1; c += 64) {
            const uint64_t s = c + lane;
            const bool hit = s < s1 && spKeep[s] && spScore[s] == bestSpScore;
            const unsigned long long m = __ballot(hit);
            if (m) {
                const uint64_t sb = c + (uint64_t)(__ffsll((long long)m) - 1);
                bestFirst = sStart[sb];
                bestSecond = sStart[sb + 1];
                break;
            }
        }
        const float thr = bestSpScore * cfg.tieRatio;
        long cnt = 0;
        int lcaNode = -1;
        for (uint64_t c = s0; c < s1; c += 64) {
            const uint64_t s = c + lane;
            const bool in = s < s1 && spKeep[s] && spScore[s] >= thr;
            const float sc = in ? spScore[s] : 0.0f;
            const int32_t sp = in ? (int32_t)M[sStart[s]].species_id : 0;
            unsigned long long m = __ballot(in);
            while (m) {
                const int b = __ffsll((long long)m) - 1;
                m &= m - 1;
                const float v = __shfl(sc, b, 64);
                const int32_t t = __shfl(sp, b, 64);
                cnt++;
                spTotal += v;
                if (cnt == 1) bestTax = t;
                if (tax.exists(t)) lcaNode = lcaNode < 0 ? tax.nodeOf[t] : tax.lca_node(lcaNode, tax.nodeOf[t]);
            }
        }
        if (cnt > 1) {
            isLCA = true;
            bestTax = lcaNode >= 0 ? tax.nodeTax[lcaNode] : 0;
            spTotal = spTotal / (float)cnt;
        }
    }
    if (spTotal == 0 || spTotal < cfg.minScore || isLCA) {
        if (lane == 0) {
            res.score = spTotal;
            if (isLCA && !(spTotal == 0 || spTotal < cfg.minScore)) {
                res.is_classified = 1;
                res.classification = bestTax;
            }
            results[r] = res;
        }
        return;
    }
    mtb_taxcnt* tc = tcP + base;
    const uint32_t dnaShift = (uint32_t)cfg.dnaShift;
    const long maxQ = (readLength + 3) / (long)dnaShift;
    const long nb = (long)(bestSecond - bestFirst);
    const mtb_match* B = M + bestFirst;
    long nTc = -1;
    if (tax.maxTax < 0xFFFFFF) {
        for (int k = lane; k < kTcHash; k += 64) { hk[k] = 0; hc[k] = 0; }
        if (lane == 0) sFlag = 0;
        for (long q0 = 0; q0 <= maxQ; q0 += kQuotLds) {
            const long q1 = min(maxQ + 1, q0 + (long)kQuotLds);
            for (long q = q0 + lane; q < q1; q += 64) qw[q - q0] = 0xFFFFFFFFu;
            __syncthreads();
            for (long i = lane; i < nb; i += 64) {
                const uint32_t q = info_pos(B[i].qinfo) / dnaShift;
                if (q > (uint32_t)maxQ || B[i].hamming > 254u) { sFlag = 1; continue; }
                if ((long)q < q0 || (long)q >= q1) continue;
                atomicMin(&qw[q - q0], (uint32_t)B[i].hamming << 24 | 0xFFFFFFu);
            }
            __syncthreads();
            if (sFlag) break;
            for (long i = lane; i < nb; i += 64) {
                const uint32_t q = info_pos(B[i].qinfo) / dnaShift;
                if ((long)q < q0 || (long)q >= q1) continue;
                const uint32_t h = (uint32_t)B[i].hamming << 24;
                uint32_t old = qw[q - q0];
                if ((old & 0xFF000000u) != h) continue;
                const int32_t t = (int32_t)B[i].target_id;
                while (true) {
                    const uint32_t cur = old & 0xFFFFFFu;
                    const uint32_t nv = h | (uint32_t)(cur == 0xFFFFFFu ? t : tax.lca((int32_t)cur, t));
                    if (nv == old) break;
                    const uint32_t prev = atomicCAS(&qw[q - q0], old, nv);
                    if (prev == old) break;
                    old = prev;
                }
            }
            __syncthreads();
            for (long q = q0 + lane; q < q1; q += 64) {
                const uint32_t wq = qw[q - q0];
                const int32_t t = wq == 0xFFFFFFFFu ? 0 : (int32_t)(wq & 0xFFFFFFu);
                if (t == 0) continue;
                uint32_t h = ((uint32_t)t * 2654435761u) & (kTcHash - 1);
                int probes = 0;
                while (true) {
                    const int32_t prev = atomicCAS(&hk[h], 0, t);
                    if (prev == 0 || prev == t) { atomicAdd(&hc[h], 1u); break; }
                    h = (h + 1) & (kTcHash - 1);
                    if (++probes == kTcHash) { sFlag = 1; break; }
                }
            }
            __syncthreads();
            if (sFlag) break;
        }
        if (!sFlag) {
            long at = 0;
            for (int k0 = 0; k0 < kTcHash; k0 += 64) {
                const int k = k0 + lane;
                const bool v = hk[k] != 0;
                const unsigned long long m = __ballot(v);
                if (v) {
                    const long p = at + (long)__popcll(m & ((1ull << lane) - 1));
                    tc[p].tax_id = hk[k];
                    tc[p].count = hc[k];
                }
                at += (long)__popcll(m);
            }
            nTc = at;
        }
    }
    if (lane != 0) return;
    if (nTc < 0) {
        nTc = filter_redundant_serial(M, bestFirst, bestSecond, gScan, gStart, dnaShift, tax, tc);
    } else {
        for (long a = 1; a < nTc; a++) {
            mtb_taxcnt v = tc[a];
            long b = a;
            while (b > 0 && tc[b - 1].tax_id > v.tax_id) { tc[b] = tc[b - 1]; b--; }
            tc[b] = v;
        }
    }
    classify_tail(res, tc, nTc, spTotal, bestTax, readLength, cfg, tax, cladeP + base * cladePerMatch,
                  n * (long)cladePerMatch);
    results[r] = res;
}

constexpr int kGroupLanes = 16;
constexpr int kGroupQ = 128;
constexpr int kGroupHash = 64;

__device__ __forceinline__ float group_max_f(float x) {
#pragma unroll
    for (int d = kGroupLanes / 2; d > 0; d >>= 1) x = fmaxf(x, __shfl_xor(x, d, kGroupLanes));
    return x;
}
__device__ __forceinline__ long group_sum_l(long x) {
#pragma unroll
    for (int d = kGroupLanes / 2; d > 0; d >>= 1) x += __shfl_xor(x, d, kGroupLanes);
    return x;
}

__global__ void __launch_bounds__(256) k_choose_taxon_group(const mtb_match* __restrict__ M,
                                                            const uint64_t* __restrict__ mOff,
                                                            const uint32_t* __restrict__ qlen, uint32_t nReads,
                                                            const uint64_t* __restrict__ sScan,
                                                            const uint64_t* __restrict__ sStart,
                                                            const uint64_t* __restrict__ gScan,
                                                            const uint64_t* __restrict__ gStart,
                                                            const float* __restrict__ spScore,
                                                            const uint8_t* __restrict__ spKeep, AssignCfg cfg,
                                                            TaxView tax, Clade* __restrict__ cladeP,
                                                            uint32_t cladePerMatch, mtb_taxcnt* __restrict__ tcP,
                                                            mtb_result* __restrict__ results) {
    constexpr int kGroups = 256 / kGroupLanes;
    __shared__ uint32_t qw[kGroups][kGroupQ];
    __shared__ int32_t hk[kGroups][kGroupHash];
    __shared__ uint32_t hc[kGroups][kGroupHash];
    __shared__ int gFlag[kGroups];
    const int g = threadIdx.x / kGroupLanes, gl = threadIdx.x % kGroupLanes;
    const int gLane0 = (threadIdx.x & 63) & ~(kGroupLanes - 1);
    const uint32_t r = blockIdx.x * kGroups + g;
    const bool valid = r < nReads;
    const uint64_t base = valid ? mOff[r] : 0;
    const long n = valid ? (long)(mOff[r + 1] - base) : 0;
    const int readLength = valid ? (int)qlen[r] : 0;
    mtb_result res = empty_result(readLength);
    float spTotal = 0.0f;
    int32_t bestTax = 0;
    bool isLCA = false, filter = false;
    uint64_t bestFirst = 0, bestSecond = 0;
    if (n > 0) {
        const uint64_t s0 = sScan[base], s1 = sScan[base + n];
        long meaningful = 0;
        float bestSpScore = 0.0f;
        for (uint64_t s = s0 + gl; s < s1; s += kGroupLanes) {
            if (!spKeep[s]) continue;
            const float score = spScore[s];
            meaningful += score > 0.f;
            bestSpScore = fmaxf(bestSpScore, score);
        }
        meaningful = group_sum_l(meaningful);
        bestSpScore = group_max_f(bestSpScore);
        if (meaningful > 0) {
            for (uint64_t c = s0; c < s1; c += kGroupLanes) {
                const uint64_t s = c + gl;
                const bool hit = s < s1 && spKeep[s] && spScore[s] == bestSpScore;
                const uint32_t m = (uint32_t)(__ballot(hit) >> gLane0) & 0xFFFFu;
                if (m) {
                    const uint64_t sb = c + (uint64_t)(__ffs((int)m) - 1);
                    bestFirst = sStart[sb];
                    bestSecond = sStart[sb + 1];
                    break;
                }
            }
            const float thr = bestSpScore * cfg.tieRatio;
            long cnt = 0;
            int lcaNode = -1;
            for (uint64_t c = s0; c < s1; c += kGroupLanes) {
                const uint64_t s = c + gl;
                const bool in = s < s1 && spKeep[s] && spScore[s] >= thr;
                const float sc = in ? spScore[s] : 0.0f;
                const int32_t sp = in ? (int32_t)M[sStart[s]].species_id : 0;
                uint32_t m = (uint32_t)(__ballot(in) >> gLane0) & 0xFFFFu;
                while (m) {
                    const int b = __ffs((int)m) - 1;
                    m &= m - 1;
                    const float v = __shfl(sc, b, kGroupLanes);
                    const int32_t t = __shfl(sp, b, kGroupLanes);
                    cnt++;
                    spTotal += v;
                    if (cnt == 1) bestTax = t;
                    if (tax.exists(t)) lcaNode = lcaNode < 0 ? tax.nodeOf[t] : tax.lca_node(lcaNode, tax.nodeOf[t]);
                }
            }
            if (cnt > 1) {
                isLCA = true;
                bestTax = lcaNode >= 0 ? tax.nodeTax[lcaNode] : 0;
                spTotal = spTotal / (float)cnt;
            }
        }
        filter = !(spTotal == 0 || spTotal < cfg.minScore || isLCA);
    }
    const uint32_t dnaShift = (uint32_t)cfg.dnaShift;
    const long maxQ = (readLength + 3) / (long)dnaShift;
    const long nb = (long)(bestSecond - bestFirst);
    const mtb_match* B = M + bestFirst;
    const bool lds = filter && maxQ < kGroupQ && tax.maxTax < 0xFFFFFF;
    if (lds) {
        for (long q = gl; q <= maxQ; q += kGroupLanes) qw[g][q] = 0xFFFFFFFFu;
        for (int k = gl; k < kGroupHash; k += kGroupLanes) {
            hk[g][k] = 0;
            hc[g][k] = 0;
        }
        if (gl == 0) gFlag[g] = 0;
    }
    __syncthreads();
    if (lds) {
        for (long i = gl; i < nb; i += kGroupLanes) {
            const uint32_t q = info_pos(B[i].qinfo) / dnaShift;
            if (q > (uint32_t)maxQ || B[i].hamming > 254u) {
                gFlag[g] = 1;
                continue;
            }
            atomicMin(&qw[g][q], (uint32_t)B[i].hamming << 24 | 0xFFFFFFu);
        }
    }
    __syncthreads();
    const bool ok = lds && !gFlag[g];
    if (ok) {
        for (long i = gl; i < nb; i += kGroupLanes) {
            const uint32_t q = info_pos(B[i].qinfo) / dnaShift;
            const uint32_t h = (uint32_t)B[i].hamming << 24;
            uint32_t old = qw[g][q];
            if ((old & 0xFF000000u) != h) continue;
            const int32_t t = (int32_t)B[i].target_id;
            while (true) {
                const uint32_t cur = old & 0xFFFFFFu;
                const uint32_t nv = h | (uint32_t)(cur == 0xFFFFFFu ? t : tax.lca((int32_t)cur, t));
                if (nv == old) break;
                const uint32_t prev = atomicCAS(&qw[g][q], old, nv);
                if (prev == old) break;
                old = prev;
            }
        }
    }
    __syncthreads();
    if (ok) {
        for (long q = gl; q <= maxQ; q += kGroupLanes) {
            const uint32_t wq = qw[g][q];
            const int32_t t = wq == 0xFFFFFFFFu ? 0 : (int32_t)(wq & 0xFFFFFFu);
            if (t == 0) continue;
            uint32_t h = ((uint32_t)t * 2654435761u) & (kGroupHash - 1);
            int probes = 0;
            while (true) {
                const int32_t prev = atomicCAS(&hk[g][h], 0, t);
                if (prev == 0 || prev == t) {
                    atomicAdd(&hc[g][h], 1u);
                    break;
                }
                h = (h + 1) & (kGroupHash - 1);
                if (++probes == kGroupHash) {
                    gFlag[g] = 1;
                    break;
                }
            }
        }
    }
    __syncthreads();
    mtb_taxcnt* tc = tcP + base;
    long nTc = -1;
    if (ok && !gFlag[g]) {
        long at = 0;
        for (int k0 = 0; k0 < kGroupHash; k0 += kGroupLanes) {
            const int k = k0 + gl;
            const bool v = hk[g][k] != 0;
            const uint32_t m = (uint32_t)(__ballot(v) >> gLane0) & 0xFFFFu;
            if (v) {
                const long p = at + (long)__popc(m & ((1u << gl) - 1));
                tc[p].tax_id = hk[g][k];
                tc[p].count = hc[g][k];
            }
            at += (long)__popc(m);
        }
        nTc = at;
    }
    if (gl != 0 || !valid) return;
    if (!filter) {
        res.score = spTotal;
        if (isLCA && n > 0 && !(spTotal == 0 || spTotal < cfg.minScore)) {
            res.is_classified = 1;
            res.classification = bestTax;
        }
        results[r] = res;
        return;
    }
    if (nTc < 0) {
        nTc = filter_redundant_serial(M, bestFirst, bestSecond, gScan, gStart, dnaShift, tax, tc);
    } else {
        for (long a = 1; a < nTc; a++) {
            mtb_taxcnt v = tc[a];
            long b = a;
            while (b > 0 && tc[b - 1].tax_id > v.tax_id) {
                tc[b] = tc[b - 1];
                b--;
            }
            tc[b] = v;
        }
    }
    classify_tail(res, tc, nTc, spTotal, bestTax, readLength, cfg, tax, cladeP + base * cladePerMatch,
                  n * (long)cladePerMatch);
    results[r] = res;
}

__global__ void k_wave_size_keys(const uint64_t* __restrict__ waveList, uint32_t n, uint64_t* __restrict__ keys) {
    const uint32_t i = blockIdx.x * blockDim.x + threadIdx.x;
    if (i < n) keys[i] = (uint64_t)(kWaveCombineMax - (uint32_t)(waveList[i] >> 32));
}
__global__ void k_read_size_keys(const uint64_t* __restrict__ mOff, uint32_t n, uint64_t* __restrict__ keys) {
    const uint32_t i = blockIdx.x * blockDim.x + threadIdx.x;
    if (i < n) keys[i] = 0xFFFFFFull - min<uint64_t>(mOff[i + 1] - mOff[i], 0xFFFFFFull);
}

static const uint64_t* longest_first(uint32_t n, int bits, const AssignScratch& s, hipStream_t st) {
    bool inB = false;
    radix_sort_pairs(s.ordKA, s.ordVA, s.ordKB, s.ordVB, n, 0, bits, false, true, s.radixCounts, s.radixOffs,
                     s.scanTmp, &inB, st);
    return inB ? s.ordVB : s.ordVA;
}

void launch_assign(const mtb_match* matches, const uint64_t* mOff, const uint32_t* qlen, uint32_t nReads, uint64_t nM, const AssignArgs& a, const TaxDevice& t, const AssignScratch& s,
                   mtb_taxcnt* tcPool, mtb_result* results, unsigned long long* devStats, uint64_t* hostStats,
                   hipStream_t st) {
    for (int i = 0; i < 4; i++) hostStats[i] = 0;
    if (nReads == 0) return;
    AssignCfg cfg{a.kmerFormat, a.dnaShift, a.maxCodonShift, a.denominator, a.minConsCnt, a.minConsCntEuk,
                  a.accessionLevel, a.minScore, a.minSpScore, a.tieRatio, a.generic, a.emulateAll, a.em};
    TaxView tv{t.nodeOf, t.nodeTax, t.parent, t.depth, t.flags, t.spParent, t.maxTax};
    if (nM) {
        launch_run_index(matches, nM, reinterpret_cast<uint8_t*>(s.gFlag),
                         reinterpret_cast<unsigned long long*>(s.sFlag), s.gScan, s.sScan, s.gStart, s.sStart, st);
        uint64_t cnt[2] = {0, 0};
        hipMemcpyAsync(&cnt[0], s.gScan + nM, sizeof(uint64_t), hipMemcpyDeviceToHost, st);
        hipMemcpyAsync(&cnt[1], s.sScan + nM, sizeof(uint64_t), hipMemcpyDeviceToHost, st);
        hipStreamSynchronize(st);
        hostStats[0] = cnt[0];
        hostStats[2] = cnt[1];
        if (cnt[0]) {
            k_group_keys<<<(unsigned)((cnt[0] + 255) / 256), 256, 0, st>>>(
                s.gStart, cnt[0], s.ordKA, s.ordVA, s.pathCnt,
                prune_min_matches(a.minConsCnt, a.minConsCntEuk, a.maxCodonShift));
            bool inB = false;
            const uint64_t heavy = radix_sort_pairs(s.ordKA, s.ordVA, s.ordKB, s.ordVB, cnt[0], 32, 40, true, false,
                                                    s.radixCounts, s.radixOffs, s.scanTmp, &inB, st);
            hostStats[1] = heavy;
            if (heavy) {
                const bool waves = !a.generic && a.bigGroups && nM >= kBigGroup;
                if (waves) hipMemsetAsync(s.waveCount, 0, sizeof(uint32_t), st);
                const char* nl = getenv("MTB_PATHS_NOLDS");
                const int nlw = nl ? atoi(nl) : 0;
#define MTB_PATHS(L, W)                                                                                             \
    k_match_paths<L, W><<<(unsigned)((heavy + 63) / 64), 64, 0, st>>>(                                              \
        matches, s.gStart, inB ? s.ordKB : s.ordKA, heavy, cfg, tv, (Path*)s.local, (Path*)s.paths, s.conn,         \
        s.pathCnt, waves ? s.waveList : nullptr, s.waveCount)
                if (nlw == 6) MTB_PATHS(false, 6);
                else if (nlw == 5) MTB_PATHS(false, 5);
                else if (nlw == 4) MTB_PATHS(false, 4);
                else MTB_PATHS(true, 1);
#undef MTB_PATHS
                if (waves) {
                    uint32_t nBig = 0;
                    hipMemcpyAsync(&nBig, s.waveCount, sizeof(uint32_t), hipMemcpyDeviceToHost, st);
                    hipStreamSynchronize(st);
                    if (nBig)
                        k_match_paths_wave<<<nBig, 64, 0, st>>>(matches, s.gStart, s.waveList, cfg, tv, (Path*)s.local,
                                                                (Path*)s.paths, s.conn, s.pathCnt);
                }
            }
        }
        if (cnt[1]) {
            hipMemsetAsync(s.waveCount, 0, sizeof(uint32_t), st);
            k_combine_paths<<<(unsigned)((cnt[1] + 255) / 256), 256, 0, st>>>(
                matches, s.sStart, cnt[1], s.gScan, s.gStart, s.pathCnt, qlen, cfg, (Path*)s.paths, (Path*)s.comb,
                s.spScore, s.spKeep, s.waveList, s.waveCount);
            uint32_t nWave = 0;
            hipMemcpyAsync(&nWave, s.waveCount, sizeof(uint32_t), hipMemcpyDeviceToHost, st);
            hipStreamSynchronize(st);
            if (nWave) {
                k_wave_size_keys<<<(nWave + 255) / 256, 256, 0, st>>>(s.waveList, nWave, s.ordKA);
                const uint64_t* order = longest_first(nWave, 16, s, st);
                k_combine_wave<<<nWave, 64, 0, st>>>(matches, s.sStart, s.waveList, qlen, cfg, (Path*)s.paths,
                                                     (Path*)s.comb, s.spScore, s.spKeep, devStats, order);
            }
            hostStats[3] = nWave;
        }
    } else {
        hipMemsetAsync(s.sScan, 0, sizeof(uint64_t), st);
    }
    const bool wave = a.waveTaxon >= 0 ? a.waveTaxon == 1 : (!a.generic && nM > (uint64_t)kWavePerReadMatches * nReads);
    const bool group = a.waveTaxon == 2 || (a.waveTaxon < 0 && !wave && !a.generic);
    if (group) {
        k_choose_taxon_group<<<(nReads + 15) / 16, 256, 0, st>>>(matches, mOff, qlen, nReads, s.sScan, s.sStart,
                                                                 s.gScan, s.gStart, s.spScore, s.spKeep, cfg, tv,
                                                                 (Clade*)s.clade, s.cladePerMatch, tcPool, results);
    } else if (wave) {
        k_read_size_keys<<<(nReads + 255) / 256, 256, 0, st>>>(mOff, nReads, s.ordKA);
        const uint64_t* order = longest_first(nReads, 24, s, st);
        k_choose_taxon_wave<<<nReads, 64, 0, st>>>(matches, mOff, qlen, nReads, s.sScan, s.sStart, s.gScan, s.gStart,
                                                   s.spScore, s.spKeep, cfg, tv, (Clade*)s.clade, s.cladePerMatch,
                                                   tcPool, results, order);
    } else {
        const unsigned ctT = nReads < 256u * 256u ? 64u : 256u;
        k_choose_taxon<<<(nReads + ctT - 1) / ctT, ctT, 0, st>>>(matches, mOff, qlen, nReads, s.sScan, s.sStart,
                                                             s.gScan, s.gStart, s.spScore, s.spKeep, cfg, tv,
                                                             (Clade*)s.clade, s.cladePerMatch, tcPool, results);
    }
}

uint64_t path_bytes() { return sizeof(Path); }
uint64_t clade_bytes() { return sizeof(Clade); }

__global__ void k_compact_taxcnt(const mtb_taxcnt* __restrict__ pool, const uint64_t* __restrict__ mOff,
                                 mtb_result* __restrict__ results, const uint64_t* __restrict__ tcOff, uint32_t nReads,
                                 mtb_taxcnt* __restrict__ out) {
    uint32_t r = blockIdx.x * blockDim.x + threadIdx.x;
    if (r >= nReads) return;
    uint32_t len = results[r].taxcnt_len;
    uint64_t dst = tcOff[r];
    results[r].taxcnt_offset = (uint32_t)dst;
    for (uint32_t k = 0; k < len; k++) out[dst + k] = pool[mOff[r] + k];
}

__global__ void k_taxcnt_len(const mtb_result* __restrict__ results, uint32_t nReads, uint32_t* __restrict__ len) {
    uint32_t r = blockIdx.x * blockDim.x + threadIdx.x;
    if (r < nReads) len[r] = results[r].taxcnt_len;
}

void launch_taxcnt_len(const mtb_result* results, uint32_t nReads, uint32_t* len, hipStream_t s) {
    if (nReads) k_taxcnt_len<<<(nReads + 255) / 256, 256, 0, s>>>(results, nReads, len);
}
void launch_compact_taxcnt(const mtb_taxcnt* pool, const uint64_t* mOff, mtb_result* results, const uint64_t* tcOff,
                           uint32_t nReads, mtb_taxcnt* out, hipStream_t s) {
    if (nReads) k_compact_taxcnt<<<(nReads + 255) / 256, 256, 0, s>>>(pool, mOff, results, tcOff, nReads, out);
}

__global__ void k_chunk_totals(const uint32_t* __restrict__ cnt, uint32_t nChunks, uint32_t n,
                               uint32_t* __restrict__ tot) {
    const uint32_t r = blockIdx.x * blockDim.x + threadIdx.x;
    if (r >= n) return;
    uint32_t t = 0;
    for (uint32_t c = 0; c < nChunks; c++) t += cnt[(uint64_t)c * n + r];
    tot[r] = t;
}

__global__ void __launch_bounds__(256) k_regroup_chunks(const uint64_t* __restrict__ src, const uint32_t* __restrict__ cnt,
                                                        const uint64_t* __restrict__ srcOff, uint32_t nChunks, uint32_t n,
                                                        const uint64_t* __restrict__ mOff, uint64_t* __restrict__ dst) {
    const uint32_t r = blockIdx.x * 4 + threadIdx.x / 64;
    const uint32_t lane = threadIdx.x & 63;
    if (r >= n) return;
    uint64_t at = mOff[r] * 3;
    for (uint32_t c = 0; c < nChunks; c++) {
        const uint64_t k = (uint64_t)c * n + r;
        const uint64_t words = (uint64_t)cnt[k] * 3, from = srcOff[k] * 3;
        for (uint64_t w = lane; w < words; w += 64) dst[at + w] = src[from + w];
        at += words;
    }
}

void launch_regroup_chunks(const mtb_match* src, const uint32_t* cnt, uint32_t nChunks, uint32_t n, uint32_t* tot,
                           uint64_t* srcOff, uint64_t* mOff, void* scanTmp, mtb_match* dst, hipStream_t s) {
    if (!n) return;
    k_chunk_totals<<<(n + 255) / 256, 256, 0, s>>>(cnt, nChunks, n, tot);
    exclusive_scan_u32(tot, n, mOff, scanTmp, s);
    exclusive_scan_u32(cnt, (uint64_t)nChunks * n, srcOff, scanTmp, s);
    k_regroup_chunks<<<(n + 3) / 4, 256, 0, s>>>((const uint64_t*)src, cnt, srcOff, nChunks, n, mOff, (uint64_t*)dst);
}

struct EmPair {
    int32_t sp;
    float sc;
};

__global__ void k_em_top(const mtb_match* __restrict__ M, const uint64_t* __restrict__ mOff, uint32_t n,
                         const uint64_t* __restrict__ sScan, const uint64_t* __restrict__ sStart,
                         const float* __restrict__ spScore, const uint8_t* __restrict__ spKeep,
                         const mtb_result* __restrict__ results, EmPair* __restrict__ scratch,
                         EmPair* __restrict__ maps, uint8_t* __restrict__ cnt) {
    const uint32_t r = blockIdx.x * blockDim.x + threadIdx.x;
    if (r >= n) return;
    cnt[r] = 0;
    if (!results[r].is_classified) return;
    const uint64_t base = mOff[r], end = mOff[r + 1];
    const uint64_t s0 = sScan[base], s1 = sScan[end];
    EmPair* v = scratch + s0;
    long k = 0;
    for (uint64_t s = s0; s < s1; s++)
        if (spKeep[s]) v[k++] = EmPair{(int32_t)M[sStart[s]].species_id, spScore[s]};
    stdsort::sort(v, v + k, [](const EmPair& a, const EmPair& b) { return a.sc > b.sc; });
    const long m = k < kEmTop ? k : kEmTop;
    for (long i = 0; i < m; i++) maps[(uint64_t)r * kEmTop + i] = EmPair{v[i].sp, v[i].sc * v[i].sc};
    cnt[r] = (uint8_t)m;
}

void launch_em_top(const mtb_match* M, const uint64_t* mOff, uint32_t n, const AssignScratch& s,
                   const mtb_result* results, void* scratch, void* maps, uint8_t* cnt, hipStream_t st) {
    if (!n) return;
    k_em_top<<<(n + 255) / 256, 256, 0, st>>>(M, mOff, n, s.sScan, s.sStart, s.spScore, s.spKeep, results,
                                              (EmPair*)scratch, (EmPair*)maps, cnt);
}

__global__ void k_em_pack(const EmPair* __restrict__ maps, const uint8_t* __restrict__ cnt,
                          const uint64_t* __restrict__ off, uint32_t n, mtb_em_map* __restrict__ out) {
    const uint32_t r = blockIdx.x * blockDim.x + threadIdx.x;
    if (r >= n) return;
    const uint64_t o = off[r];
    for (uint32_t k = 0; k < cnt[r]; k++) {
        const EmPair e = maps[(uint64_t)r * kEmTop + k];
        out[o + k] = mtb_em_map{r, e.sp, e.sc};
    }
}

__global__ void k_u8_to_u32(const uint8_t* __restrict__ in, uint32_t n, uint32_t* __restrict__ out) {
    const uint32_t i = blockIdx.x * blockDim.x + threadIdx.x;
    if (i < n) out[i] = in[i];
}

void launch_em_pack(const void* maps, const uint8_t* cnt, uint32_t n, uint32_t* cnt32, uint64_t* off, void* scanTmp,
                    mtb_em_map* out, hipStream_t s) {
    if (!n) return;
    k_u8_to_u32<<<(n + 255) / 256, 256, 0, s>>>(cnt, n, cnt32);
    exclusive_scan_u32(cnt32, n, off, scanTmp, s);
    k_em_pack<<<(n + 255) / 256, 256, 0, s>>>((const EmPair*)maps, cnt, off, n, out);
}

__global__ void k_species_kmers(const DbRec* __restrict__ db, uint64_t D, const int32_t* __restrict__ spOf,
                                uint32_t maxTax, uint32_t* __restrict__ cnt) {
    MTB_GRID_STRIDE(i, D) {
        const uint32_t t = db[i].tax;
        const int32_t sp = t <= maxTax ? spOf[t] : 0;
        if (sp > 0) atomicAdd(&cnt[sp], 1u);
    }
}

void launch_species_kmers(const DbRec* db, uint64_t D, const int32_t* spOf, uint32_t maxTax, uint32_t* cnt,
                          hipStream_t s) {
    if (D) k_species_kmers<<<stride_grid(D), 256, 0, s>>>(db, D, spOf, maxTax, cnt);
}

__global__ void k_em_estep(const float* __restrict__ score, const uint32_t* __restrict__ spIdx,
                           const uint64_t* __restrict__ qOff, uint64_t nQ, const uint64_t* __restrict__ pos,
                           const double* __restrict__ p, const double* __restrict__ lf, double* __restrict__ wS,
                           unsigned long long* __restrict__ qCount) {
    const uint64_t q = (uint64_t)blockIdx.x * blockDim.x + threadIdx.x;
    bool counted = false;
    if (q < nQ) {
        const uint64_t a = qOff[q], b = qOff[q + 1];
        double denom = 0.0;
        for (uint64_t j = a; j < b; j++) denom += (double)score[j] * p[spIdx[j]] * lf[spIdx[j]];
        counted = !(denom == 0.0);
        for (uint64_t j = a; j < b; j++)
            wS[pos[j]] = counted ? ((double)score[j] * p[spIdx[j]] * lf[spIdx[j]]) / denom : 0.0;
    }
    const int c = __syncthreads_count(counted);
    if (threadIdx.x == 0 && c) atomicAdd(qCount, (unsigned long long)c);
}

__global__ void k_em_slices(const double* __restrict__ wS, const uint64_t* __restrict__ sliceOff, uint64_t nSl,
                            double* __restrict__ part) {
    const uint64_t i = (uint64_t)blockIdx.x * blockDim.x + threadIdx.x;
    if (i >= nSl) return;
    double f = 0.0;
    for (uint64_t j = sliceOff[i]; j < sliceOff[i + 1]; j++) f += wS[j];
    part[i] = f;
}

__global__ void k_em_mstep(const double* __restrict__ part, const uint64_t* __restrict__ spSlice, uint32_t S,
                           const uint8_t* __restrict__ isTop, const unsigned long long* __restrict__ qCount,
                           const double* __restrict__ p, double* __restrict__ pNew, double* __restrict__ absd,
                           int afterTen) {
    const uint32_t i = blockIdx.x * blockDim.x + threadIdx.x;
    if (i >= S) return;
    double f = 0.0;
    for (uint64_t k = spSlice[i]; k < spSlice[i + 1]; k++) f += part[k];
    if (isTop[i]) {
        f /= (double)*qCount;
        absd[i] = fabs(f - p[i]);
        if (afterTen && f < 1e-5) f = 0.0;
    } else {
        absd[i] = 0.0;
    }
    pNew[i] = f;
}

__global__ void __launch_bounds__(256) k_em_delta(const double* __restrict__ absd, uint32_t S, double* __restrict__ out) {
    __shared__ double part[256];
    const uint32_t per = (S + 255) / 256, a = threadIdx.x * per, b = min(S, a + per);
    double d = 0.0;
    for (uint32_t i = a; i < b; i++) d += absd[i];
    part[threadIdx.x] = d;
    __syncthreads();
    if (threadIdx.x == 0) {
        double t = 0.0;
        for (int k = 0; k < 256; k++) t += part[k];
        *out = t;
    }
}

void launch_em_iteration(const float* score, const uint32_t* spIdx, const uint64_t* qOff, uint64_t nQ,
                         const uint64_t* pos, const double* p, const double* lf, double* wS,
                         unsigned long long* qCount, const uint64_t* sliceOff, uint64_t nSl, double* part,
                         const uint64_t* spSlice, uint32_t S, const uint8_t* isTop, double* pNew, double* absd,
                         int afterTen, double* delta, hipStream_t s) {
    (void)hipMemsetAsync(qCount, 0, sizeof(unsigned long long), s);
    if (nQ) k_em_estep<<<(unsigned)((nQ + 255) / 256), 256, 0, s>>>(score, spIdx, qOff, nQ, pos, p, lf, wS, qCount);
    if (nSl) k_em_slices<<<(unsigned)((nSl + 255) / 256), 256, 0, s>>>(wS, sliceOff, nSl, part);
    if (S) k_em_mstep<<<(S + 255) / 256, 256, 0, s>>>(part, spSlice, S, isTop, qCount, p, pNew, absd, afterTen);
    k_em_delta<<<1, 256, 0, s>>>(absd, S, delta);
}

struct EmPairD {
    int32_t sp;
    double pr;
};

__global__ void k_em_reclassify(const float* __restrict__ score, const uint32_t* __restrict__ spIdx,
                                const int32_t* __restrict__ spTax, const uint64_t* __restrict__ qOff,
                                const uint32_t* __restrict__ qId, uint64_t nQ, const double* __restrict__ p,
                                const double* __restrict__ lf, TaxView tax, mtb_em_read* __restrict__ out) {
    const uint64_t q = (uint64_t)blockIdx.x * blockDim.x + threadIdx.x;
    if (q >= nQ) return;
    const uint64_t a = qOff[q], b = qOff[q + 1];
    EmPairD v[kEmTop];
    double denom = 0.0;
    long k = 0;
    for (uint64_t j = a; j < b && k < kEmTop; j++, k++) {
        const double sc = p[spIdx[j]] * (double)score[j] * lf[spIdx[j]];
        denom += sc;
        v[k] = EmPairD{spTax[spIdx[j]], sc};
    }
    mtb_em_read r;
    r.tax_id = 0;
    r.score = 0.0;
    if (denom == 0.0) {
        r.mapped = 2;
        out[qId[q]] = r;
        return;
    }
    for (long i = 0; i < k; i++) v[i].pr /= denom;
    stdsort::sort(v, v + k, [](const EmPairD& x, const EmPairD& y) { return x.pr > y.pr; });
    double sum = 0.0;
    int lcaNode = -1;
    for (long i = 0; i < k && sum < 0.5; i++) {
        sum += v[i].pr;
        const int32_t t = v[i].sp;
        if (tax.exists(t)) lcaNode = lcaNode < 0 ? tax.nodeOf[t] : tax.lca_node(lcaNode, tax.nodeOf[t]);
    }
    r.tax_id = lcaNode >= 0 ? tax.nodeTax[lcaNode] : 0;
    r.score = sum;
    r.mapped = 1;
    out[qId[q]] = r;
// ... 42 lines not shown
```

metabuli_work_amd/csrc/mtb_kernels.hip:

```cpp
#include "mtb_launch.h"

#include <cstring>

namespace mtb {

constexpr int kBlock = 256;
constexpr int kWaves = kBlock / 64;

__device__ __forceinline__ unsigned long long wave_inclusive_scan(unsigned long long x) {
    const int lane = threadIdx.x & 63;
#pragma unroll
    for (int d = 1; d < 64; d <<= 1) {
        unsigned long long y = __shfl_up(x, d, 64);
        if (lane >= d) x += y;
    }
    return x;
}

__device__ __forceinline__ unsigned long long block_exclusive_scan(unsigned long long x, unsigned long long* total) {
    __shared__ unsigned long long wsum[kWaves];
    const int lane = threadIdx.x & 63, w = threadIdx.x >> 6;
    unsigned long long inc = wave_inclusive_scan(x);
    if (lane == 63) wsum[w] = inc;
    __syncthreads();
    unsigned long long off = 0, tot = 0;
#pragma unroll
    for (int i = 0; i < kWaves; i++) {
        if (i < w) off += wsum[i];
        tot += wsum[i];
    }
    __syncthreads();
    *total = tot;
    return off + inc - x;
}

constexpr int kScanItems = 16;
constexpr int kScanTile = kBlock * kScanItems;

template <typename T>
__global__ void k_scan_tiles(const T* __restrict__ in, uint64_t n, unsigned long long* __restrict__ tileSum) {
    const uint64_t base = (uint64_t)blockIdx.x * kScanTile;
    unsigned long long s = 0;
#pragma unroll
    for (int k = 0; k < kScanItems; k++) {
        uint64_t i = base + (uint64_t)k * kBlock + threadIdx.x;
        if (i < n) s += (unsigned long long)in[i];
    }
    unsigned long long tot;
    block_exclusive_scan(s, &tot);
    if (threadIdx.x == 0) tileSum[blockIdx.x] = tot;
}

__global__ void k_scan_tile_sums(unsigned long long* __restrict__ tileSum, uint64_t nTiles) {
    unsigned long long carry = 0;
    for (uint64_t b = 0; b < nTiles; b += kBlock) {
        uint64_t i = b + threadIdx.x;
        unsigned long long x = i < nTiles ? tileSum[i] : 0ull;
        unsigned long long tot;
        unsigned long long ex = block_exclusive_scan(x, &tot);
        if (i < nTiles) tileSum[i] = carry + ex;
        carry += tot;
        __syncthreads();
    }
    if (threadIdx.x == 0) tileSum[nTiles] = carry;
}

template <typename T>
__global__ void k_scan_apply(const T* __restrict__ in, uint64_t n, const unsigned long long* __restrict__ tileSum,
                             uint64_t* __restrict__ out) {
    const uint64_t base = (uint64_t)blockIdx.x * kScanTile + (uint64_t)threadIdx.x * kScanItems;
    unsigned long long v[kScanItems];
    unsigned long long s = 0;
#pragma unroll
    for (int k = 0; k < kScanItems; k++) {
        uint64_t i = base + k;
        v[k] = i < n ? (unsigned long long)in[i] : 0ull;
        s += v[k];
    }
    unsigned long long tot;
    unsigned long long run = block_exclusive_scan(s, &tot) + tileSum[blockIdx.x];
#pragma unroll
    for (int k = 0; k < kScanItems; k++) {
        uint64_t i = base + k;
        if (i < n) out[i] = run;
        run += v[k];
    }
    if (blockIdx.x == gridDim.x - 1 && threadIdx.x == kBlock - 1) out[n] = tileSum[gridDim.x];
}

template <typename T>
static void scan_impl(const T* in, uint64_t n, uint64_t* out, unsigned long long* tmp, hipStream_t s) {
    uint64_t tiles = (n + kScanTile - 1) / kScanTile;
    if (tiles == 0) {
        hipMemsetAsync(out, 0, sizeof(uint64_t), s);
        return;
    }
    k_scan_tiles<T><<<(unsigned)tiles, kBlock, 0, s>>>(in, n, tmp);
    k_scan_tile_sums<<<1, kBlock, 0, s>>>(tmp, tiles);
    k_scan_apply<T><<<(unsigned)tiles, kBlock, 0, s>>>(in, n, tmp, out);
}

uint64_t scan_tmp_elems(uint64_t n) { return (n + kScanTile - 1) / kScanTile + 1; }

constexpr int kRunItems = 32;
constexpr int kRunTile = kBlock * kRunItems;

__global__ void __launch_bounds__(256) k_run_tiles(const mtb_match* __restrict__ M, uint64_t nM,
                                                   uint8_t* __restrict__ flags, unsigned long long* __restrict__ tileSum) {
    const uint64_t base = (uint64_t)blockIdx.x * kRunTile;
    unsigned long long s = 0;
#pragma unroll 8
    for (int k = 0; k < kRunItems; k++) {
        const uint64_t i = base + (uint64_t)k * kBlock + threadIdx.x;
        if (i >= nM) break;
        uint32_t g = 1, sp = 1;
        if (i > 0) {
            const uint64_t qa = M[i - 1].qinfo, qb = M[i].qinfo;
            const bool newSp = info_seq(qa) != info_seq(qb) || M[i - 1].species_id != M[i].species_id;
            sp = newSp;
            g = newSp || info_frame(qa) != info_frame(qb);
        }
        flags[i] = (uint8_t)(g | sp << 1);
        s += (unsigned long long)g | (unsigned long long)sp << 32;
    }
    unsigned long long tot;
    block_exclusive_scan(s, &tot);
    if (threadIdx.x == 0) tileSum[blockIdx.x] = tot;
}

__global__ void __launch_bounds__(256) k_run_index(const uint8_t* __restrict__ flags, uint64_t nM,
                                                   const unsigned long long* __restrict__ tileSum,
                                                   uint64_t* __restrict__ gScan, uint64_t* __restrict__ sScan,
                                                   uint64_t* __restrict__ gStart, uint64_t* __restrict__ sStart) {
    __shared__ uint32_t sIdx[kRunTile];
    __shared__ uint8_t sF[kRunTile];
    const uint64_t base = (uint64_t)blockIdx.x * kRunTile;
    const uint32_t nT = (uint32_t)min<uint64_t>(kRunTile, nM - base);
    const int tid = threadIdx.x;
    if (nT == kRunTile) {
        const uint4* src = reinterpret_cast<const uint4*>(flags + base);
        uint4* dst = reinterpret_cast<uint4*>(sF);
        for (int x = tid; x < kRunTile / 16; x += kBlock) dst[x] = src[x];
    } else {
        for (uint32_t x = tid; x < nT; x += kBlock) sF[x] = flags[base + x];
    }
    __syncthreads();
    uint32_t f[kRunItems];
    unsigned long long s = 0;
#pragma unroll
    for (int k = 0; k < kRunItems; k++) {
        const uint32_t x = (uint32_t)tid * kRunItems + k;
        f[k] = x < nT ? sF[x] : 0u;
        s += (unsigned long long)(f[k] & 1u) | (unsigned long long)(f[k] >> 1) << 32;
    }
    unsigned long long tot;
    const unsigned long long ex = block_exclusive_scan(s, &tot);
    const unsigned long long tb = tileSum[blockIdx.x];
    const uint64_t gBase = tb & 0xFFFFFFFFull, sBase = tb >> 32;
#pragma unroll
    for (int kind = 0; kind < 2; kind++) {
        uint32_t run = kind ? (uint32_t)(ex >> 32) : (uint32_t)ex;
#pragma unroll
        for (int k = 0; k < kRunItems; k++) {
            sIdx[tid * kRunItems + k] = run;
            run += (f[k] >> kind) & 1u;
        }
        __syncthreads();
        uint64_t* scan = kind ? sScan : gScan;
        uint64_t* start = kind ? sStart : gStart;
        const uint64_t b0 = kind ? sBase : gBase;
        for (uint32_t x = tid; x < nT; x += kBlock) {
            const uint64_t v = b0 + sIdx[x];
            scan[base + x] = v;
            if ((sF[x] >> kind) & 1u) start[v] = base + x;
        }
        __syncthreads();
    }
    if (blockIdx.x == gridDim.x - 1 && tid == 0) {
        const unsigned long long all = tileSum[gridDim.x];
        gScan[nM] = all & 0xFFFFFFFFull;
        sScan[nM] = all >> 32;
        gStart[all & 0xFFFFFFFFull] = nM;
        sStart[all >> 32] = nM;
    }
}

uint64_t run_index_tmp_bytes(uint64_t nM) { return 8 * ((nM + kRunTile - 1) / kRunTile + 2); }

void launch_run_index(const mtb_match* M, uint64_t nM, uint8_t* flags, unsigned long long* tileSum, uint64_t* gScan,
                      uint64_t* sScan, uint64_t* gStart, uint64_t* sStart, hipStream_t s) {
    if (nM == 0) return;
    const uint64_t tiles = (nM + kRunTile - 1) / kRunTile;
    k_run_tiles<<<(unsigned)tiles, kBlock, 0, s>>>(M, nM, flags, tileSum);
    k_scan_tile_sums<<<1, kBlock, 0, s>>>(tileSum, tiles);
    k_run_index<<<(unsigned)tiles, kBlock, 0, s>>>(flags, nM, tileSum, gScan, sScan, gStart, sStart);
}
void exclusive_scan_u32(const uint32_t* in, uint64_t n, uint64_t* out, void* tmp, hipStream_t s) {
    scan_impl<uint32_t>(in, n, out, (unsigned long long*)tmp, s);
}
void exclusive_scan_u64(const uint64_t* in, uint64_t n, uint64_t* out, void* tmp, hipStream_t s) {
    scan_impl<uint64_t>(in, n, out, (unsigned long long*)tmp, s);
}

__global__ void k_read_meta(const uint64_t* __restrict__ off1, const uint64_t* __restrict__ off2, uint32_t n,
                            int paired, ReadMeta* __restrict__ meta, uint32_t* __restrict__ qlen,
                            uint32_t* __restrict__ maxW, uint32_t* __restrict__ readLens) {
    uint32_t i = blockIdx.x * blockDim.x + threadIdx.x;
    if (i >= n) return;
    int len1 = (int)(off1[i + 1] - off1[i]);
    int ql1 = max_covered_length(len1);
    int w1 = query_kmer_number(len1) / 6;
    int len2 = 0, ql2 = 0, w2 = 0;
    bool empty = w1 < 1;
    if (paired) {
        len2 = (int)(off2[i + 1] - off2[i]);
        ql2 = max_covered_length(len2);
        w2 = query_kmer_number(len2) / 6;
        if (w2 < 1) empty = true;
    }
    ReadMeta m;
    m.len1 = len1; m.len2 = len2; m.ql1 = ql1; m.ql2 = ql2;
    m.w1 = empty ? 0 : w1;
    m.w2 = (empty || !paired) ? 0 : w2;
    meta[i] = m;
    qlen[i] = (uint32_t)(ql1 + ql2);
    readLens[i] = (uint32_t)min(len1, 0xFFFF) | (uint32_t)min(len2, 0xFFFF) << 16;
    const uint32_t w = (uint32_t)max(m.w1, m.w2);
    if (w) atomicMax(maxW, w);
}

__global__ void k_read_units(const ReadMeta* __restrict__ meta, uint32_t n, uint32_t C, uint32_t upr,
                             uint32_t* __restrict__ units) {
    uint32_t i = blockIdx.x * blockDim.x + threadIdx.x;
    if (i >= n) return;
    const ReadMeta m = meta[i];
    units[i] = upr ? upr : 6u * ((uint32_t)(m.w1 + C - 1) / C + (uint32_t)(m.w2 + C - 1) / C);
}

__global__ void k_unit_read(const uint64_t* __restrict__ uOff, uint32_t n, uint32_t* __restrict__ unitRead) {
    uint32_t i = blockIdx.x * blockDim.x + threadIdx.x;
    if (i >= n) return;
    for (uint64_t u = uOff[i]; u < uOff[i + 1]; u++) unitRead[u] = i;
}

void launch_read_meta(const uint64_t* off1, const uint64_t* off2, uint32_t n, int paired, ReadMeta* meta,
                      uint32_t* qlen, uint32_t* maxW, uint32_t* readLens, hipStream_t s) {
    hipMemsetAsync(maxW, 0, sizeof(uint32_t), s);
    if (n == 0) return;
    k_read_meta<<<(n + 255) / 256, 256, 0, s>>>(off1, off2, n, paired, meta, qlen, maxW, readLens);
}

void launch_read_units(const ReadMeta* meta, uint32_t n, uint32_t C, uint32_t upr, uint32_t* units, hipStream_t s) {
    if (n) k_read_units<<<(n + 255) / 256, 256, 0, s>>>(meta, n, C, upr, units);
}

void launch_unit_read(const uint64_t* uOff, uint32_t n, uint32_t* unitRead, hipStream_t s) {
    if (n) k_unit_read<<<(n + 255) / 256, 256, 0, s>>>(uOff, n, unitRead);
}

struct ExtractTables {
    uint8_t base[256];
    int8_t aa[64];
    int8_t num[64];
};

struct UnitWindows {
    const uint8_t* seq;
    int s0, e0;
    int pFirst, nWin;
    bool fromLeft, comp;
    uint64_t info0;
    uint64_t stretch;
};

__device__ __forceinline__ UnitWindows unit_windows(uint64_t u, uint64_t nUnits, uint32_t C,
                                                    const uint8_t* __restrict__ seq1, const uint64_t* __restrict__ off1,
                                                    const uint8_t* __restrict__ seq2, const uint64_t* __restrict__ off2,
                                                    const ReadMeta* __restrict__ meta, const uint64_t* __restrict__ uOff,
                                                    const uint32_t* __restrict__ unitRead, int kmerFormat,
                                                    uint32_t upr) {
    UnitWindows w{};
    if (u >= nUnits) return w;
    const uint32_t r = upr ? (uint32_t)(u / upr) : unitRead[u];
    const ReadMeta m = meta[r];
    const uint64_t first = upr ? (uint64_t)r * upr : uOff[r];
    w.stretch = first | (upr ? (uint64_t)upr : uOff[r + 1] - first) << 40;
    uint32_t local = (uint32_t)(u - first);
    const uint32_t c1 = upr ? 1u : (uint32_t)(m.w1 + C - 1) / C, c2 = upr ? 1u : (uint32_t)(m.w2 + C - 1) / C;
    uint32_t cpf = c1;
    int mate = 0;
    if (local >= 6 * c1) { local -= 6 * c1; mate = 1; cpf = c2; }
    const int frame = (int)(local / cpf);
    const int chunk = (int)(local % cpf);
    const int W = mate ? m.w2 : m.w1;
    w.pFirst = chunk * (int)C;
    w.nWin = min((int)C, W - w.pFirst);
    if (w.nWin <= 0) return w;
    w.seq = mate ? seq2 + off2[r] : seq1 + off1[r];
    const int len = mate ? m.len2 : m.len1;
    const int used = mate ? m.ql2 : m.ql1;
    const uint32_t posOffset = mate ? (uint32_t)m.ql1 + 3u : 0u;
    const bool fwd = frame < 3;
    int begin;
    if (fwd) begin = frame;
    else { begin = (len % 3) - (frame % 3); if (begin < 0) begin += 3; }
    w.s0 = begin;
    w.e0 = begin + used - 1;
    w.fromLeft = (kmerFormat == 2) ? fwd : !fwd;
    w.comp = !fwd;
    const uint32_t pos0 = w.fromLeft ? (uint32_t)(w.s0 + 3 * w.pFirst) : (uint32_t)(w.e0 - 3 * (w.pFirst + 8) + 1);
    w.info0 = pack_info(r + 1, pos0 + posOffset, (uint32_t)frame);
    return w;
}

struct WinScanner {
    const UnitWindows& w;
    const uint8_t* seq;
    const uint8_t* sBase;
    const int8_t *sAA, *sNum;
    int syncmer, nSm;
    uint64_t smMask;
    uint64_t aaAcc = 0, dnaAcc = 0, smAcc = 0;
    uint64_t sm0 = 0, sm1 = 0, sm2 = 0, sm3 = 0, sm4 = 0, sm5 = 0, sm6 = 0, sm7 = 0;
    int run = 0, j;
    uint32_t first7 = 0, firstAA = 0, lastAA = 0;

    __device__ __forceinline__ WinScanner(const UnitWindows& w_, const uint8_t* b, const int8_t* a, const int8_t* n,
                                          int sync, int smerLen, const uint8_t* seqAt)
        : w(w_), seq(seqAt), sBase(b), sAA(a), sNum(n), syncmer(sync), nSm(8 - smerLen + 1),
          smMask((smerLen >= 13) ? ~0ull : ((1ull << (5 * smerLen)) - 1)), j(w_.pFirst) {
        if (w.nWin > 0)
            for (int k = 0; k < 7; k++) codon();
    }
    __device__ __forceinline__ void codon() {
        const int d = w.fromLeft ? 1 : -1;
        const int c0 = w.fromLeft ? w.s0 + 3 * j : w.e0 - 3 * j;
        const uint32_t x = sBase[seq[c0]], y = sBase[seq[c0 + d]], z = sBase[seq[c0 + 2 * d]];
        const bool back = w.fromLeft == w.comp;
        const uint32_t cm = w.comp ? 2u : 0u;
        const uint32_t b1 = (back ? z : x) ^ cm, b2 = y ^ cm, b3 = (back ? x : z) ^ cm;
        const bool valid = ((x | y | z) < 4u);
        const int idx = (int)(((b1 << 4) | (b2 << 2) | b3) & 63u);
        const int aaT = sAA[idx], numT = sNum[idx];
        const int aa = valid ? aaT : -1, num = valid ? numT : 0;
        const bool ok = aa >= 0;
        run = ok ? run + 1 : 0;
        aaAcc = ok ? (aaAcc << 5) | (uint64_t)aa : aaAcc;
        dnaAcc = ok ? (dnaAcc << 3) | (uint64_t)num : dnaAcc;
// ... 3456 lines not shown
```

metabuli_work_amd/csrc/mtb_launch.h:

```cpp
#pragma once
#include <hip/hip_runtime.h>
#include <stdint.h>

#include <utility>

#include "mtb_device.h"

namespace mtb {

constexpr int kErrTaxid = 1;
constexpr int kErrStagedRead = 2;
constexpr int kErrProbeStash = 3;
constexpr int kErrProbeCount = 4;
constexpr int kErrRunOutsideDb = 5;
constexpr int kErrLiveCount = 6;

struct ReadMeta {
    int32_t len1, len2, ql1, ql2, w1, w2;
};

struct HostTables {
    uint8_t base[256];
    int8_t aa[64];
    int8_t num[64];
};

struct TaxDevice {
    const int32_t* nodeOf;
    const int32_t* nodeTax;
    const int32_t* parent;
    const int32_t* depth;
    const uint8_t* flags;
    const int32_t* spParent;
    int32_t maxTax;
};

struct AssignArgs {
    int kmerFormat, dnaShift, maxCodonShift, denominator, minConsCnt, minConsCntEuk, accessionLevel;
    float minScore, minSpScore, tieRatio;
    int generic;
    int waveTaxon = -1;
    int emulateAll = 0;
    int em = 0;
    int bigGroups = 1;
};

struct AssignScratch {
    void* local;
    void* paths;
    void* comb;
    uint8_t* conn;
    uint32_t *gFlag, *sFlag, *pathCnt;
    uint64_t *gScan, *sScan, *gStart, *sStart;
    float* spScore;
    uint64_t* waveList;
    uint32_t* waveCount;
    uint8_t* spKeep;
    void* scanTmp;
    uint64_t *ordKA, *ordVA, *ordKB, *ordVB;
    uint32_t* radixCounts;
    uint64_t* radixOffs;
    void* clade;
    uint32_t cladePerMatch;
};

uint64_t scan_tmp_elems(uint64_t n);
inline unsigned stride_grid(uint64_t n, unsigned block = 256) {
    const uint64_t b = (n + block - 1) / block;
    return (unsigned)(b < 1 ? 1 : (b > (1ull << 22) ? (1ull << 22) : b));
}
#define MTB_GRID_STRIDE(i, n) \
    for (uint64_t i = (uint64_t)blockIdx.x * blockDim.x + threadIdx.x; i < (n); i += (uint64_t)gridDim.x * blockDim.x)
void exclusive_scan_u32(const uint32_t* in, uint64_t n, uint64_t* out, void* tmp, hipStream_t s);
void exclusive_scan_u64(const uint64_t* in, uint64_t n, uint64_t* out, void* tmp, hipStream_t s);
uint64_t run_index_tmp_bytes(uint64_t nM);
void launch_run_index(const mtb_match* M, uint64_t nM, uint8_t* flags, unsigned long long* tileSum, uint64_t* gScan,
                      uint64_t* sScan, uint64_t* gStart, uint64_t* sStart, hipStream_t s);

void launch_read_meta(const uint64_t* off1, const uint64_t* off2, uint32_t n, int paired, ReadMeta* meta,
                      uint32_t* qlen, uint32_t* maxW, uint32_t* readLens, hipStream_t s);
void launch_read_units(const ReadMeta* meta, uint32_t n, uint32_t C, uint32_t upr, uint32_t* units, hipStream_t s);
void launch_unit_read(const uint64_t* uOff, uint32_t n, uint32_t* unitRead, hipStream_t s);
uint64_t extract_slots(uint64_t nUnits, uint32_t C);
void launch_extract(const uint8_t* seq1, const uint64_t* off1, const uint8_t* seq2, const uint64_t* off2,
                    const ReadMeta* meta, const uint64_t* uOff, const uint32_t* unitRead, uint64_t nUnits,
                    uint32_t C, const HostTables& t, int kmerFormat, int syncmer, int smerLen, uint64_t* keys,
                    uint64_t* unitInfo, hipStream_t s, uint32_t upr = 0);

uint64_t radix_counts_elems(uint64_t n);
template <typename V>
uint64_t radix_sort_pairs(uint64_t* keysA, V* valsA, uint64_t* keysB, V* valsB, uint64_t n, int bitLo, int bitHi,
                          bool filter, bool genVals, uint32_t* counts, uint64_t* offs, void* scanTmp, bool* inB,
                          hipStream_t s, uint8_t* digA = nullptr, uint8_t* digB = nullptr, bool unstableFirst = false);
constexpr int kSortBins = 2048;
uint64_t radix_binned_tiles(const uint64_t* binHost, uint64_t rc);
template <typename V>
uint64_t radix_sort_binned(uint64_t* keysR, V* valsR, uint64_t* keysT, V* valsT, const uint64_t* binHost,
                           const unsigned long long* binDev, uint64_t rc, int bitLo, int bitHi, uint32_t* counts,
                           uint64_t* offs, void* scanTmp, uint64_t* tileTab, bool* inT, hipStream_t s, uint8_t* digR,
                           uint8_t* digT);
void launch_to_rank_form(uint64_t* v, uint64_t n, hipStream_t s);
uint64_t host_from_rank_form(uint64_t v);
constexpr uint64_t kAARankEnd = 37822859361ull;
constexpr int kQuerySortLo = 36, kQuerySortHi = 60;
constexpr int kQuerySortLoFine = 36;

uint64_t decode_diff_chunk(const uint16_t* diff, uint64_t n, uint64_t carry, uint64_t* values, uint32_t* flagTmp,
                           uint64_t* idxTmp, void* scanTmp, uint64_t* lastTerm, uint64_t* lastValue, hipStream_t s);
void launch_mask_info(uint32_t* info, uint64_t n, uint32_t mask, hipStream_t s);

struct DbRec {
    uint32_t lo, hi, tax;
};
static_assert(sizeof(DbRec) == 12, "12-B DB records");
void launch_pack_db(const uint64_t* v, const uint32_t* tax, uint64_t n, DbRec* out, hipStream_t s);
void launch_rec_rank_form(DbRec* db, uint64_t n, hipStream_t s);
void launch_rec_mask_info(DbRec* db, uint64_t n, uint32_t mask, hipStream_t s);

struct AADir {
    const uint64_t* dir;
    uint64_t R;
    uint64_t div;
    int L;
    int fmt;
};
AADir make_aa_dir(uint64_t D, int kmerFormat);
void build_aa_dir(const DbRec* db, uint64_t D, const AADir& d, uint64_t* dir, hipStream_t s);

constexpr uint32_t kLineRanks = 448;
struct alignas(64) ProbeLine {
    uint64_t base;
    uint32_t bits[kLineRanks / 32];
};
static_assert(sizeof(ProbeLine) == 64, "one probe line per 64-B segment");
constexpr uint32_t kStatStripes = 256;
constexpr uint32_t kProbeStatsLen = 2 * kStatStripes + 1;
constexpr uint64_t kDbPad = 8;
constexpr uint64_t kProbeLines = (kAARankEnd + kLineRanks - 1) / kLineRanks + 1;
void build_probe_lines(const DbRec* db, uint64_t D, const AADir& dir, ProbeLine* lines,
                       hipStream_t s);

constexpr uint64_t kRunIdxMax = 0xFFFF;
void build_line_prefix(const ProbeLine* lines, uint64_t* lineP, uint32_t* popTmp, void* scanTmp, hipStream_t s);
void build_run_offsets(const DbRec* db, uint64_t D, const ProbeLine* lines, const uint64_t* lineP,
                       uint16_t* runOff, hipStream_t s);
constexpr uint32_t kExtRanks = 256;
struct alignas(64) ProbeExt {
    uint32_t w[kExtRanks / 16];
};
static_assert(sizeof(ProbeExt) == 64, "one run-length line per probe line");
void build_line_ext(const ProbeLine* lines, const uint64_t* lineP, const uint16_t* runOff, ProbeExt* ext,
                    hipStream_t s);
void launch_line_ext_check(const ProbeLine* lines, const uint64_t* lineP, const uint16_t* runOff, const ProbeExt* ext,
                           unsigned long long* out, hipStream_t s);

constexpr uint64_t kLinkSlots = 1801088541ull;
static_assert(kLinkSlots * 21 == kAARankEnd, "21^8 AA ranks");
void build_link_lines(const ProbeLine* lines, uint64_t* link, hipStream_t s);
void launch_link_check(const ProbeLine* lines, const uint64_t* link, unsigned long long* out, hipStream_t s);

uint64_t launch_extract_filter(const uint8_t* seq1, const uint64_t* off1, const uint8_t* seq2, const uint64_t* off2,
                               const ReadMeta* meta, const uint64_t* uOff, const uint32_t* unitRead, uint64_t nUnits,
                               uint32_t C, const HostTables& t, int kmerFormat, int syncmer, int smerLen,
                               uint64_t* unitInfo, const ProbeLine* lines, uint64_t* qkey, uint32_t* qslot,
                               unsigned long long* counter, uint64_t rankLo, uint64_t rankHi, uint64_t* emitted,
                               uint64_t cap, bool threadMajor, hipStream_t s,
                               uint8_t* qdig = nullptr, unsigned long long* binCnt = nullptr, uint64_t binRc = 0,
                               uint64_t* binHost = nullptr, uint32_t upr = 0, const uint64_t* link = nullptr);
uint64_t launch_filter(const uint64_t* keys, uint64_t R, const ProbeLine* lines, uint64_t* qkey, uint32_t* qslot,
                       uint64_t* qfrom, unsigned long long* counter, uint64_t rankLo, uint64_t rankHi,
                       uint64_t* emitted, hipStream_t s);
void launch_probe(const uint64_t* qkey, const uint32_t* qslot, const uint64_t* qfrom, uint64_t Q,
                  const uint64_t* unitInfo, uint32_t C, const DbRec* db, uint64_t D,
                  const int32_t* spOf, uint32_t maxTax, int kmerFormat, uint32_t* readCnt, unsigned long long* total,
                  mtb_match* buf, uint32_t* bufRank, uint64_t region, int* err, unsigned long long* stats,
                  hipStream_t s);

constexpr uint32_t kSegMaxTax = (1u << 24) - 1;
struct SegMatch {
    uint32_t posFrame, targetHam, speciesReh, dnaReh;
};
static_assert(sizeof(SegMatch) == 16, "16-B segment matches");
__host__ __device__ inline SegMatch seg_pack(const mtb_match& m) {
    return SegMatch{(uint32_t)m.qinfo | (uint32_t)(m.qinfo >> 61) << 29, m.target_id | (uint32_t)m.hamming << 24,
                    m.species_id | (uint32_t)(m.right_end_hamming & 0xFFu) << 24,
                    (m.dna_encoding & 0xFFFFFFu) | (uint32_t)(m.right_end_hamming >> 8) << 24};
}
__host__ __device__ inline mtb_match seg_expand(const SegMatch& s, uint64_t seqBits) {
    mtb_match m;
    m.qinfo = (uint64_t)(s.posFrame >> 29) << 61 | seqBits | (s.posFrame & 0x1FFFFFFFu);
    m.target_id = s.targetHam & 0xFFFFFFu;
    m.species_id = s.speciesReh & 0xFFFFFFu;
    m.dna_encoding = s.dnaReh & 0xFFFFFFu;
    m.right_end_hamming = (uint16_t)((s.speciesReh >> 24) | (s.dnaReh >> 24) << 8);
    m.hamming = (uint8_t)(s.targetHam >> 24);
    m.pad = 0;
    return m;
}

constexpr uint32_t kStageRegions = 256;
void set_ab_rank_free(int on);
void set_match_xcd(int on);
void set_share_runs(int on);
void set_match_prefetch(int m);
void set_pair_read(int on);
void set_ab_sweep_count(int on);

struct LongRun {
    uint64_t q;
    uint64_t lo, hi;
};
void launch_match_long(const LongRun* list, uint32_t n, const uint64_t* qkey, const uint32_t* qslot,
                       const uint64_t* unitInfo, uint32_t C, const DbRec* db, uint64_t D, const int32_t* spOf,
                       uint32_t maxTax, int kmerFormat, uint32_t* readCnt, unsigned long long* total, mtb_match* buf,
                       uint32_t* bufRank, uint64_t region, int* err, SegMatch* direct, const uint64_t* dirOff,
                       int* overflow, uint32_t capShift, unsigned long long* stats, hipStream_t s, unsigned long long* cnt64 = nullptr);
uint64_t sweep_tiles(uint64_t D, uint32_t nom);
constexpr uint64_t kSweepStarts = (1ull << 24) + 1;
constexpr uint64_t kSweepStartsTmp = kSweepStarts + (kSweepStarts + 1023) / 1024;
void build_sweep_tiles(const DbRec* db, uint64_t D, uint32_t nom, uint64_t* pstartTmp, uint64_t* tileRec,
                       uint32_t* tilePre, hipStream_t s);
void build_query_starts(const uint64_t* qkey, uint64_t Q, uint32_t* qStart, const uint32_t* tilePre, uint64_t nTiles,
                        uint32_t* tileQ, hipStream_t s);
void launch_sweep(const uint64_t* tileRec, const uint32_t* tileQ, uint64_t nTiles, const uint64_t* qkey,
                  const uint32_t* qslot, const uint64_t* unitInfo, uint32_t C, const DbRec* db, uint64_t D,
                  const int32_t* spOf, uint32_t maxTax, int kmerFormat, uint32_t* readCnt, unsigned long long* total,
                  mtb_match* buf, uint32_t* bufRank, uint64_t region, int* err, unsigned long long* stats,
                  SegMatch* direct, int* overflow, uint32_t capShift, LongRun* longList, uint32_t longCap,
                  uint32_t* longCnt, uint32_t ldsCap, bool small, int persist, hipStream_t s);
void launch_match(const uint64_t* qkey, const uint32_t* qslot, const uint64_t* unitInfo, uint32_t C, uint64_t Q,
                  const DbRec* db, uint64_t D, const AADir& dir, const int32_t* spOf,
                  uint32_t maxTax, int kmerFormat, uint32_t* readCnt, unsigned long long* total, mtb_match* buf,
                  uint32_t* bufRank, uint64_t region, int* err, uint32_t winCap, const uint64_t* win,
                  const ProbeLine* lines, const uint64_t* lineP, const uint16_t* runOff, int sortLo,
                  unsigned long long* stats, SegMatch* direct, const uint64_t* dirOff, int* overflow,
                  uint32_t capShift, LongRun* longList, uint32_t longCap, uint32_t* longCnt, hipStream_t s,
                  const ProbeExt* lineExt = nullptr, uint32_t upr = 0, unsigned long long* cnt64 = nullptr);
void launch_cnt64_init(const uint32_t* readLens, uint32_t n, unsigned long long* cnt64, hipStream_t s);
void launch_cnt64_counts(const unsigned long long* cnt64, uint32_t n, uint32_t* readCnt, hipStream_t s);
void launch_compact_segments(const SegMatch* in, const uint64_t* dirOff, uint32_t C, const uint64_t* readOff,
                             uint32_t nReads, mtb_match* out, uint32_t capShift, hipStream_t s, int mode = 0);
void launch_spill_scatter(const mtb_match* spill, const uint32_t* spillRank, const unsigned long long* total,
                          uint64_t nSpill, const uint64_t* readOff, uint32_t nReads, mtb_match* out, int* err,
                          hipStream_t s);
bool unstaged_join(bool lines, uint64_t D, uint64_t Q, uint32_t winCap);
void launch_match_transpose(const mtb_match* buf, const uint32_t* bufRank, uint64_t region,
                            const unsigned long long* total, const uint64_t* readOff, uint32_t nReads, mtb_match* out,
                            int* err, hipStream_t s);
uint64_t match_window_elems(uint64_t Q);
void launch_dup_stats(const uint64_t* qkey, uint64_t Q, unsigned long long* out, hipStream_t s);
void launch_hamming_check(const uint64_t* a, const uint64_t* b, uint64_t n, uint8_t* sum, uint16_t* fwd, uint16_t* rev,
                          unsigned long long* bad, hipStream_t s);
void launch_pin_eval(int fn, const int64_t* param, const uint64_t* a, const uint64_t* b, uint64_t n, int64_t* out,
                     hipStream_t s);
void launch_match_windows(const uint64_t* qkey, uint64_t Q, const DbRec* db, uint64_t D, const AADir& dir,
                          int kmerFormat, uint64_t* win, hipStream_t s);

uint64_t path_bytes();
uint64_t clade_bytes();
hipError_t launch_segsort(const mtb_match* in, const uint64_t* mOff, uint32_t nReads, uint64_t M, mtb_match* out,
                          uint64_t* gScratch, uint32_t maxSeg, bool global, uint32_t* liveCnt, uint32_t mergeSeg,
                          uint32_t pruneMin, hipStream_t s, const SegMatch* seg = nullptr,
                          const uint64_t* inOff = nullptr, uint32_t inC = 0 ,
                          uint32_t* segLen = nullptr,
                          uint32_t* maxTmp = nullptr, int pruneAfter = 0, uint32_t* lists = nullptr);
inline uint32_t prune_min_matches(int minConsCnt, int minConsCntEuk, int maxCodonShift) {
    const int d = minConsCnt < minConsCntEuk ? minConsCnt : minConsCntEuk;
    const int sh = maxCodonShift > 0 ? maxCodonShift : 1;
    const int need = d <= 1 ? 1 : 1 + (d - 1 + sh - 1) / sh;
    return (uint32_t)(need < 2 ? 2 : need);
}
void launch_pack_live(const mtb_match* in, const uint64_t* mOff, const uint64_t* liveOff, uint32_t nReads,
                      mtb_match* out, int* err, hipStream_t s);
void launch_max_u32(const uint32_t* x, uint32_t n, uint32_t* out, hipStream_t s);
void launch_max_seg(const uint64_t* off, uint32_t n, uint32_t* out, hipStream_t s);
constexpr uint32_t kSegSortLds = 8192;
constexpr uint32_t kSegSortRegs = 512;
constexpr uint32_t kSegSortSparse = 2048;
constexpr uint64_t kMaxBatchMatches = 0xFFFFFFFFull;
void launch_assign(const mtb_match* matches, const uint64_t* mOff, const uint32_t* qlen, uint32_t nReads, uint64_t nM, const AssignArgs& a, const TaxDevice& t, const AssignScratch& s,
                   mtb_taxcnt* tcPool, mtb_result* results, unsigned long long* devStats, uint64_t* hostStats,
                   hipStream_t st);
void launch_regroup_chunks(const mtb_match* src, const uint32_t* cnt, uint32_t nChunks, uint32_t n, uint32_t* tot,
                           uint64_t* srcOff, uint64_t* mOff, void* scanTmp, mtb_match* dst, hipStream_t s);
void launch_taxcnt_len(const mtb_result* results, uint32_t nReads, uint32_t* len, hipStream_t s);
void launch_compact_taxcnt(const mtb_taxcnt* pool, const uint64_t* mOff, mtb_result* results, const uint64_t* tcOff,
                           uint32_t nReads, mtb_taxcnt* out, hipStream_t s);

constexpr int kEmTop = 10;
void launch_em_top(const mtb_match* M, const uint64_t* mOff, uint32_t n, const AssignScratch& s,
                   const mtb_result* results, void* scratch, void* maps, uint8_t* cnt, hipStream_t st);
void launch_em_pack(const void* maps, const uint8_t* cnt, uint32_t n, uint32_t* cnt32, uint64_t* off, void* scanTmp,
                    mtb_em_map* out, hipStream_t s);
void launch_species_kmers(const DbRec* db, uint64_t D, const int32_t* spOf, uint32_t maxTax, uint32_t* cnt,
                          hipStream_t s);
void launch_em_iteration(const float* score, const uint32_t* spIdx, const uint64_t* qOff, uint64_t nQ,
                         const uint64_t* pos, const double* p, const double* lf, double* wS,
                         unsigned long long* qCount, const uint64_t* sliceOff, uint64_t nSl, double* part,
                         const uint64_t* spSlice, uint32_t S, const uint8_t* isTop, double* pNew, double* absd,
                         int afterTen, double* delta, hipStream_t s);
void launch_em_reclassify(const float* score, const uint32_t* spIdx, const int32_t* spTax, const uint64_t* qOff,
                          const uint32_t* qId, uint64_t nQ, const double* p, const double* lf, const TaxDevice& t,
                          mtb_em_read* out, hipStream_t s);

constexpr int kTantanOffsets = 50;
struct TantanTables {
    double lr[25];
    double b2f[kTantanOffsets];
    double b2b, f2b, f2f;
    double minMask;
};
TantanTables make_tantan_tables(float maskProb);
uint64_t tantan_scale_elems(uint64_t bases, uint32_t n);
void launch_tantan_mask(const uint8_t* seq, const uint64_t* off, uint32_t n, const TantanTables& tt, float* prob,
                        double* scale, uint8_t* out, hipStream_t s);

}
```

Measured before the change: 33.29 million.

## Fuse run-flag computation into live-pack and build run index per read

Replaces the separate pack-live copy plus global tiled run-index (tile sums, global scan, per-element gScan/sScan arrays) with a per-read wave kernel that copies live matches and emits group/species run flags and counts in one pass. Run starts are then computed per read from small per-read offset scans, eliminating the per-match scan arrays and an extra pass over all matches. It also adds a register lookahead cursor that prefetches upcoming match records in the global path-matching kernels. The change alters buffer layout and indexing in the assign scratch struct, and it relies on runs never crossing read boundaries.

```diff
diff --git a/metabuli_work_amd/csrc/mtb_api.hip b/metabuli_work_amd/csrc/mtb_api.hip
--- a/metabuli_work_amd/csrc/mtb_api.hip
+++ b/metabuli_work_amd/csrc/mtb_api.hip
@@ -175,6 +175,7 @@
     uint32_t longCap = 0;
     DevBuf chunkIn, chunkCnt, chunkSrcOff;
     DevBuf liveCnt, liveOff;
+    DevBuf runFlag, runCnt, runScan;
     DevBuf segLen;
     DevBuf sizeLists;
     DevBuf digA, digB;
@@ -196,7 +197,7 @@
     std::vector<uint32_t> spKmers;
     std::string dbDir;
     DevBuf local, paths, comb, conn, spScore, spKeep,
-        gFlag, sFlag, pathCnt, gScan, sScan, gStart, sStart, clade, tcPool, tcLen, tcOff, tcOut, results;
+        pathCnt, gStart, sStart, runGroup, clade, tcPool, tcLen, tcOff, tcOut, results;
     uint32_t nReads = 0;
     uint64_t Q = 0, M = 0, nTaxcnt = 0;
     uint64_t Qall = 0;
@@ -666,8 +667,8 @@
     X(errFlag) X(ordKA) X(ordVA) X(ordKB) X(ordVB) X(matchWin) X(unitRead) X(unitInfo) X(waveList) X(waveCount) \
     X(devStats) X(mStage) X(mRank) X(mDirect) X(ovFlag) X(mTotal) X(qFrom) X(probeStats) X(longList) X(longCnt) \
     X(qStart) X(chunkIn) X(chunkCnt) X(chunkSrcOff) X(liveCnt) X(liveOff) X(segLen) X(sizeLists) X(digA) \
-    X(digB) X(binCnt) X(binTab) X(local) X(paths) X(comb) X(conn) X(spScore) X(spKeep) X(gFlag) X(sFlag) \
-    X(pathCnt) X(gScan) X(sScan) X(gStart) X(sStart) X(clade) X(tcPool) X(tcLen) X(tcOff) X(tcOut) X(results) \
+    X(digB) X(binCnt) X(binTab) X(local) X(paths) X(comb) X(conn) X(spScore) X(spKeep) X(runFlag) X(runCnt) \
+    X(runScan) X(pathCnt) X(gStart) X(sStart) X(runGroup) X(clade) X(tcPool) X(tcLen) X(tcOff) X(tcOut) X(results) \
     X(emMap) X(emCnt) X(emScratch) X(emPacked) X(emCnt32) X(emOff) X(maskOut1) X(maskOut2) X(maskProb) \
     X(maskScale) X(readLens) X(readCnt64)
 static std::vector<DevBuf*> batch_bufs(mtb_ctx* c) {
@@ -813,15 +814,24 @@
     const mtb_match* kIn = c->matchesSorted.as<mtb_match>();
     const uint64_t* kOff = c->mOff.as<uint64_t>();
     uint64_t kM = M;
+    HIP_TRY(c->runCnt.ensure(sizeof(uint32_t) * 2 * ((size_t)n + 1)));
+    HIP_TRY(c->runScan.ensure(sizeof(uint64_t) * 2 * ((size_t)n + 1)));
+    uint32_t* grpCnt = c->runCnt.as<uint32_t>();
+    uint32_t* runCnt = grpCnt + n + 1;
     if (prune) {
         exclusive_scan_u32(c->liveCnt.as<uint32_t>(), n, c->liveOff.as<uint64_t>(), c->scanTmp.p, s);
         HIP_TRY(hipMemcpyAsync(&kM, c->liveOff.as<uint64_t>() + n, sizeof(uint64_t), hipMemcpyDeviceToHost, s));
-        launch_pack_live(c->matchesSorted.as<mtb_match>(), c->mOff.as<uint64_t>(), c->liveOff.as<uint64_t>(), n,
-                         c->matches.as<mtb_match>(), c->errFlag.as<int>(), s);
         HIP_TRY(hipStreamSynchronize(s));
         if (kM > M) { set_error("internal error: K5 kept more matches than it sorted"); return MTB_ERR_INTERNAL; }
+        HIP_TRY(c->runFlag.ensure(std::max<uint64_t>(kM, 1)));
+        launch_run_flags(c->matchesSorted.as<mtb_match>(), c->mOff.as<uint64_t>(), c->liveOff.as<uint64_t>(), n,
+                         c->matches.as<mtb_match>(), c->runFlag.as<uint8_t>(), grpCnt, runCnt, c->errFlag.as<int>(),
+                         s);
         kIn = c->matches.as<mtb_match>();
         kOff = c->liveOff.as<uint64_t>();
+    } else {
+        HIP_TRY(c->runFlag.ensure(Mc));
+        launch_run_flags(kIn, kOff, kOff, n, nullptr, c->runFlag.as<uint8_t>(), grpCnt, runCnt, c->errFlag.as<int>(), s);
     }
     c->liveM = kM;
     c->stats[11] = kM;
@@ -851,13 +861,10 @@
                    {&c->spScore, sizeof(float) * Kc, nullptr},
                    {&c->spKeep, Kc, nullptr},
                    {&c->waveList, sizeof(uint64_t) * Kc, nullptr},
-                   {&c->gFlag, sizeof(uint32_t) * (Kc + 1), nullptr},
                    {&c->pathCnt, sizeof(uint32_t) * (Kc + 1), nullptr},
-                   {&c->sFlag, std::max<uint64_t>(sizeof(uint32_t) * (Kc + 1), run_index_tmp_bytes(Kc)), nullptr},
-                   {&c->gScan, sizeof(uint64_t) * (Kc + 1), nullptr},
-                   {&c->sScan, sizeof(uint64_t) * (Kc + 1), nullptr},
                    {&c->gStart, sizeof(uint64_t) * (Kc + 1), nullptr},
                    {&c->sStart, sizeof(uint64_t) * (Kc + 1), nullptr},
+                   {&c->runGroup, sizeof(uint64_t) * (Kc + 1), nullptr},
                    {&c->clade, clade_bytes() * Kc * c->cladePerMatch, nullptr},
                    {&c->tcPool, sizeof(mtb_taxcnt) * Kc, nullptr},
                    {&c->ordKA, sizeof(uint64_t) * (Mn + 1), nullptr},
@@ -895,26 +902,28 @@
                      need[2].p,
                      (uint8_t*)need[3].p,
                      (uint32_t*)need[7].p,
-                     (uint32_t*)need[9].p,
-                     (uint32_t*)need[8].p,
+                     (uint64_t*)need[8].p,
+                     (uint64_t*)need[9].p,
                      (uint64_t*)need[10].p,
-                     (uint64_t*)need[11].p,
-                     (uint64_t*)need[12].p,
-                     (uint64_t*)need[13].p,
+                     c->runFlag.as<uint8_t>(),
+                     grpCnt,
+                     runCnt,
+                     c->runScan.as<uint64_t>(),
+                     c->runScan.as<uint64_t>() + n + 1,
                      (float*)need[4].p,
                      (uint64_t*)need[6].p,
                      c->waveCount.as<uint32_t>(),
                      (uint8_t*)need[5].p,
                      c->scanTmp.p,
+                     (uint64_t*)need[13].p,
+                     (uint64_t*)need[14].p,
+                     (uint64_t*)need[15].p,
                      (uint64_t*)need[16].p,
-                     (uint64_t*)need[17].p,
-                     (uint64_t*)need[18].p,
-                     (uint64_t*)need[19].p,
                      c->radixCounts.as<uint32_t>(),
                      c->radixOffs.as<uint64_t>(),
-                     need[14].p,
+                     need[11].p,
                      c->cladePerMatch};
-    mtb_taxcnt* tcPool = (mtb_taxcnt*)need[15].p;
+    mtb_taxcnt* tcPool = (mtb_taxcnt*)need[12].p;
     c->stats[3] = M;
     c->stats[4] = maxSeg;
     launch_assign(kIn, kOff, c->qlen.as<uint32_t>(), n, kM, a, t, sc, tcPool,
diff --git a/metabuli_work_amd/csrc/mtb_assign.hip b/metabuli_work_amd/csrc/mtb_assign.hip
--- a/metabuli_work_amd/csrc/mtb_assign.hip
+++ b/metabuli_work_amd/csrc/mtb_assign.hip
@@ -1527,25 +1527,58 @@
                         lists);
 }
 
-__global__ void __launch_bounds__(256) k_pack_live(const mtb_match* __restrict__ in, const uint64_t* __restrict__ mOff,
+template <bool kCopy>
+__global__ void __launch_bounds__(256) k_run_flags(const mtb_match* __restrict__ in, const uint64_t* __restrict__ mOff,
                                                    const uint64_t* __restrict__ liveOff, uint32_t nReads,
-                                                   mtb_match* __restrict__ out, int* __restrict__ err) {
+                                                   mtb_match* __restrict__ out, uint8_t* __restrict__ flags,
+                                                   uint32_t* __restrict__ grpCnt, uint32_t* __restrict__ runCnt,
+                                                   int* __restrict__ err) {
     const uint32_t r = blockIdx.x * 4 + threadIdx.x / 64;
     const uint32_t lane = threadIdx.x & 63;
     if (r >= nReads) return;
-    const uint64_t live = liveOff[r + 1] - liveOff[r];
-    if (live > mOff[r + 1] - mOff[r] || liveOff[r + 1] > mOff[nReads]) {
-        if (lane == 0) atomicExch(err, kErrLiveCount);
+    const uint64_t lo = liveOff[r];
+    const uint64_t live = liveOff[r + 1] - lo;
+    if (kCopy && (live > mOff[r + 1] - mOff[r] || liveOff[r + 1] > mOff[nReads])) {
+        if (lane == 0) {
+            atomicExch(err, kErrLiveCount);
+            grpCnt[r] = 0;
+            runCnt[r] = 0;
+        }
         return;
     }
-    const uint64_t* src = reinterpret_cast<const uint64_t*>(in + mOff[r]);
-    uint64_t* dst = reinterpret_cast<uint64_t*>(out + liveOff[r]);
-    for (uint64_t w = lane; w < live * 3; w += 64) dst[w] = src[w];
-}
-
-void launch_pack_live(const mtb_match* in, const uint64_t* mOff, const uint64_t* liveOff, uint32_t nReads,
-                      mtb_match* out, int* err, hipStream_t s) {
-    if (nReads) k_pack_live<<<(nReads + 3) / 4, 256, 0, s>>>(in, mOff, liveOff, nReads, out, err);
+    const mtb_match* src = in + (kCopy ? mOff[r] : lo);
+    uint32_t ng = 0, ns = 0;
+    for (uint64_t e0 = 0; e0 < live; e0 += 64) {
+        const uint64_t e = e0 + lane;
+        const bool on = e < live;
+        mtb_match m = {};
+        if (on) m = src[e];
+        const uint32_t sp = m.species_id, fr = info_frame(m.qinfo);
+        uint32_t psp = __shfl_up(sp, 1, 64), pfr = __shfl_up(fr, 1, 64);
+        if (lane == 0 && e0 > 0) {
+            psp = src[e0 - 1].species_id;
+            pfr = info_frame(src[e0 - 1].qinfo);
+        }
+        const bool newSp = on && (e == 0 || psp != sp);
+        const bool newG = on && (newSp || pfr != fr);
+        if (on) {
+            if (kCopy) out[lo + e] = m;
+            flags[lo + e] = (uint8_t)((uint32_t)newG | (uint32_t)newSp << 1);
+        }
+        ng += (uint32_t)__popcll(__ballot(newG));
+        ns += (uint32_t)__popcll(__ballot(newSp));
+    }
+    if (lane == 0) {
+        grpCnt[r] = ng;
+        runCnt[r] = ns;
+    }
+}
+
+void launch_run_flags(const mtb_match* in, const uint64_t* mOff, const uint64_t* liveOff, uint32_t nReads,
+                      mtb_match* out, uint8_t* flags, uint32_t* grpCnt, uint32_t* runCnt, int* err, hipStream_t s) {
+    if (!nReads) return;
+    if (out) k_run_flags<true><<<(nReads + 3) / 4, 256, 0, s>>>(in, mOff, liveOff, nReads, out, flags, grpCnt, runCnt, err);
+    else k_run_flags<false><<<(nReads + 3) / 4, 256, 0, s>>>(in, mOff, liveOff, nReads, out, flags, grpCnt, runCnt, err);
 }
 
 __global__ void __launch_bounds__(256) k_max_seg(const uint64_t* __restrict__ off, uint32_t n, uint32_t* __restrict__ out) {
@@ -1626,12 +1659,58 @@
 constexpr int kRegPos = 4;
 constexpr uint64_t kBigGroup = 256;
 
+constexpr int kAhead = 2;
+template <typename R>
+struct IndexCursor {
+    R r;
+    __device__ __forceinline__ void init(uint64_t, uint64_t) {}
+    __device__ __forceinline__ void advance(uint64_t) {}
+    __device__ __forceinline__ uint32_t pos(uint64_t k) const { return r.pos(k); }
+    __device__ __forceinline__ uint32_t dna(uint64_t k) const { return r.dna(k); }
+    __device__ __forceinline__ uint32_t reh(uint64_t k) const { return r.reh(k); }
+    __device__ __forceinline__ uint32_t ham(uint64_t k) const { return r.ham(k); }
+};
 struct GlobalRecs {
     const mtb_match* __restrict__ M;
     __device__ __forceinline__ uint32_t pos(uint64_t k) const { return info_pos(M[k].qinfo); }
     __device__ __forceinline__ uint32_t dna(uint64_t k) const { return M[k].dna_encoding; }
     __device__ __forceinline__ uint32_t reh(uint64_t k) const { return M[k].right_end_hamming; }
     __device__ __forceinline__ uint32_t ham(uint64_t k) const { return M[k].hamming; }
+    using Cursor = IndexCursor<GlobalRecs>;
+    __device__ __forceinline__ Cursor cursor() const { return Cursor{*this}; }
+};
+struct GlobalAhead : GlobalRecs {
+    struct Cursor {
+        const mtb_match* __restrict__ M;
+        uint64_t last;
+        uint32_t p[kAhead + 1], dh[kAhead + 1], rh[kAhead + 1];
+        __device__ __forceinline__ void fetch(uint32_t& fp, uint32_t& fdh, uint32_t& frh, uint64_t i) const {
+            const uint32_t* w = reinterpret_cast<const uint32_t*>(M + min(i, last));
+            fp = w[0];
+            const uint2 t = *reinterpret_cast<const uint2*>(w + 4);
+            fdh = (t.x & 0xFFFFFFu) | (t.y & 0xFF0000u) << 8;
+            frh = t.y & 0xFFFFu;
+        }
+        __device__ __forceinline__ void init(uint64_t start, uint64_t end) {
+            last = end - 1;
+#pragma unroll
+            for (int j = 0; j <= kAhead; j++) fetch(p[j], dh[j], rh[j], start + j);
+        }
+        __device__ __forceinline__ void advance(uint64_t k) {
+#pragma unroll
+            for (int j = 0; j < kAhead; j++) {
+                p[j] = p[j + 1];
+                dh[j] = dh[j + 1];
+                rh[j] = rh[j + 1];
+            }
+            fetch(p[kAhead], dh[kAhead], rh[kAhead], k + kAhead);
+        }
+        __device__ __forceinline__ uint32_t pos(uint64_t) const { return p[0]; }
+        __device__ __forceinline__ uint32_t dna(uint64_t) const { return dh[0] & 0xFFFFFFu; }
+        __device__ __forceinline__ uint32_t reh(uint64_t) const { return rh[0]; }
+        __device__ __forceinline__ uint32_t ham(uint64_t) const { return dh[0] >> 24; }
+    };
+    __device__ __forceinline__ Cursor cursor() const { return Cursor{M}; }
 };
 struct LdsRecs {
     const uint32_t* p;
@@ -1642,10 +1721,12 @@
     __device__ __forceinline__ uint32_t dna(uint64_t k) const { return dh[k - base] & 0xFFFFFFu; }
     __device__ __forceinline__ uint32_t reh(uint64_t k) const { return rh[k - base]; }
     __device__ __forceinline__ uint32_t ham(uint64_t k) const { return dh[k - base] >> 24; }
+    using Cursor = IndexCursor<LdsRecs>;
+    __device__ __forceinline__ Cursor cursor() const { return Cursor{*this}; }
 };
 
 template <typename R>
-__device__ __forceinline__ bool match_paths_regs(const R& M, uint64_t start, uint64_t end,
+__device__ __forceinline__ bool match_paths_regs(const R& recs, uint64_t start, uint64_t end,
                                                  const AssignCfg& cfg, int minDepth, bool fwd,
                                                  Path* __restrict__ P, uint64_t& nPout, bool emitLone = false) {
     Path cp[kRegPos], np[kRegPos];
@@ -1654,6 +1735,8 @@
     int nc = 0, nn = 0;
     uint64_t nP = start;
     uint64_t k = start;
+    typename R::Cursor M = recs.cursor();
+    M.init(start, end);
     uint32_t currPos = M.pos(k);
     while (k < end) {
         if (M.pos(k) != currPos) break;
@@ -1673,6 +1756,7 @@
             }
         nc++;
         k++;
+        M.advance(k);
     }
     const bool stepped = k < end;
     while (k < end) {
@@ -1696,6 +1780,7 @@
                 }
             nn++;
             k++;
+            M.advance(k);
         }
         const int shift = (int)((nextPos - currPos) / 3);
         if (shift > 0 && shift <= cfg.maxCodonShift) {
@@ -1846,7 +1931,7 @@
 
 constexpr int kPathStage = 1024;
 
-template <bool kLds, int kW>
+template <bool kLds, int kW, bool kLook>
 __global__ void __launch_bounds__(64) __attribute__((amdgpu_waves_per_eu(kW))) k_match_paths(const mtb_match* __restrict__ M, const uint64_t* __restrict__ gStart,
                                                     const uint64_t* __restrict__ order, uint64_t nWork, AssignCfg cfg,
                                                     TaxView tax, Path* __restrict__ L, Path* __restrict__ P,
@@ -1877,6 +1962,8 @@
     }
     if (staged)
         match_paths_group(LdsRecs{sPos, sDh, sReh, spanLo}, M, g, start, end, cfg, tax, L, P, conn, pathCnt);
+    else if (kLook)
+        match_paths_group(GlobalAhead{M}, M, g, start, end, cfg, tax, L, P, conn, pathCnt);
     else
         match_paths_group(GlobalRecs{M}, M, g, start, end, cfg, tax, L, P, conn, pathCnt);
 }
@@ -1890,6 +1977,7 @@
     return !(shift > 0 && shift <= maxCodonShift);
 }
 
+template <bool kLook>
 __global__ void __launch_bounds__(64) k_match_paths_wave(const mtb_match* __restrict__ M,
                                                          const uint64_t* __restrict__ gStart,
                                                          const uint64_t* __restrict__ bigList, AssignCfg cfg,
@@ -1911,7 +1999,9 @@
     uint64_t cnt = 0;
     if (a < b) {
         uint64_t nPr = a;
-        if (!cfg.generic && match_paths_regs(GlobalRecs{M}, a, b, cfg, minDepth, fwd, P, nPr, multi)) cnt = nPr - a;
+        const bool regs = !cfg.generic && (kLook ? match_paths_regs(GlobalAhead{M}, a, b, cfg, minDepth, fwd, P, nPr, multi)
+                                                 : match_paths_regs(GlobalRecs{M}, a, b, cfg, minDepth, fwd, P, nPr, multi));
+        if (regs) cnt = nPr - a;
         else cnt = match_paths_serial(GlobalRecs{M}, a, b, cfg, minDepth, fwd, L, P, conn, multi) - a;
     }
     uint64_t inc = cnt;
@@ -2004,7 +2094,7 @@
 constexpr int kWaveCombineMax = 1024;
 
 __global__ void __launch_bounds__(256) k_combine_paths(const mtb_match* __restrict__ M, const uint64_t* __restrict__ sStart,
-                                                       uint64_t nS, const uint64_t* __restrict__ gScan,
+                                                       uint64_t nS, const uint64_t* __restrict__ runGroup,
                                                        const uint64_t* __restrict__ gStart,
                                                        const uint32_t* __restrict__ pathCnt,
                                                        const uint32_t* __restrict__ qlen, AssignCfg cfg,
@@ -2015,7 +2105,7 @@
     if (s >= nS) return;
     const uint64_t ss = sStart[s], se = sStart[s + 1];
     uint64_t w = ss;
-    for (uint64_t g = gScan[ss]; gStart[g] < se; g++) {
+    for (uint64_t g = runGroup[s]; gStart[g] < se; g++) {
         const uint64_t src = gStart[g];
         const uint32_t cnt = pathCnt[g];
         if (src != w)
@@ -2171,12 +2261,12 @@
 }
 
 __device__ long filter_redundant_serial(const mtb_match* __restrict__ M, uint64_t bestFirst, uint64_t bestSecond,
-                                        const uint64_t* __restrict__ gScan, const uint64_t* __restrict__ gStart,
+                                        uint64_t bestGroup, const uint64_t* __restrict__ gStart,
                                         uint32_t dnaShift, const TaxView& tax, mtb_taxcnt* __restrict__ tc) {
     uint32_t fc[6], fin[6], head[6];
     const mtb_match* B = M + bestFirst;
     int nf = 0;
-    for (uint64_t g = gScan[bestFirst]; nf < 6 && gStart[g] < bestSecond; g++) {
+    for (uint64_t g = bestGroup; nf < 6 && gStart[g] < bestSecond; g++) {
         fc[nf] = (uint32_t)(gStart[g] - bestFirst);
         fin[nf] = (uint32_t)(gStart[g + 1] - bestFirst);
         nf++;
@@ -2323,9 +2413,9 @@
 
 __global__ void __launch_bounds__(256) k_choose_taxon(const mtb_match* __restrict__ M, const uint64_t* __restrict__ mOff,
                                                       const uint32_t* __restrict__ qlen, uint32_t nReads,
-                                                      const uint64_t* __restrict__ sScan,
+                                                      const uint64_t* __restrict__ runOff,
                                                       const uint64_t* __restrict__ sStart,
-                                                      const uint64_t* __restrict__ gScan,
+                                                      const uint64_t* __restrict__ runGroup,
                                                       const uint64_t* __restrict__ gStart,
                                                       const float* __restrict__ spScore,
                                                       const uint8_t* __restrict__ spKeep, AssignCfg cfg, TaxView tax,
@@ -2340,15 +2430,15 @@
     mtb_result res = empty_result(readLength);
     if (n == 0) { results[r] = res; return; }
 
-    const uint64_t s0 = sScan[base], s1 = sScan[base + n];
+    const uint64_t s0 = runOff[r], s1 = runOff[r + 1];
     long meaningful = 0;
     float bestSpScore = 0.0f;
-    uint64_t bestFirst = 0, bestSecond = 0;
+    uint64_t bestFirst = 0, bestSecond = 0, bestRun = 0;
     for (uint64_t s = s0; s < s1; s++) {
         if (!spKeep[s]) continue;
         const float score = spScore[s];
         if (score > 0.f) meaningful++;
-        if (score > bestSpScore) { bestSpScore = score; bestFirst = sStart[s]; bestSecond = sStart[s + 1]; }
+        if (score > bestSpScore) { bestSpScore = score; bestFirst = sStart[s]; bestSecond = sStart[s + 1]; bestRun = s; }
     }
 
     float spTotal = 0.0f;
@@ -2387,7 +2477,7 @@
         return;
     }
     mtb_taxcnt* tc = tcP + base;
-    const long nTc = filter_redundant_serial(M, bestFirst, bestSecond, gScan, gStart, (uint32_t)cfg.dnaShift, tax, tc);
+    const long nTc = filter_redundant_serial(M, bestFirst, bestSecond, runGroup[bestRun], gStart, (uint32_t)cfg.dnaShift, tax, tc);
     classify_tail(res, tc, nTc, spTotal, bestTax, readLength, cfg, tax, cladeP + base * cladePerMatch,
                   n * (long)cladePerMatch);
     results[r] = res;
@@ -2410,9 +2500,9 @@
 
 __global__ void __launch_bounds__(64) k_choose_taxon_wave(const mtb_match* __restrict__ M, const uint64_t* __restrict__ mOff,
                                                           const uint32_t* __restrict__ qlen, uint32_t nReads,
-                                                          const uint64_t* __restrict__ sScan,
+                                                          const uint64_t* __restrict__ runOff,
                                                           const uint64_t* __restrict__ sStart,
-                                                          const uint64_t* __restrict__ gScan,
+                                                          const uint64_t* __restrict__ runGroup,
                                                           const uint64_t* __restrict__ gStart,
                                                           const float* __restrict__ spScore,
                                                           const uint8_t* __restrict__ spKeep, AssignCfg cfg,
@@ -2435,7 +2525,7 @@
         if (lane == 0) results[r] = res;
         return;
     }
-    const uint64_t s0 = sScan[base], s1 = sScan[base + n];
+    const uint64_t s0 = runOff[r], s1 = runOff[r + 1];
     long meaningful = 0;
     float bestSpScore = 0.0f;
     for (uint64_t s = s0 + lane; s < s1; s += 64) {
@@ -2449,7 +2539,7 @@
     float spTotal = 0.0f;
     int32_t bestTax = 0;
     bool isLCA = false;
-    uint64_t bestFirst = 0, bestSecond = 0;
+    uint64_t bestFirst = 0, bestSecond = 0, bestRun = 0;
     if (meaningful > 0) {
         for (uint64_t c = s0; c < s1; c += 64) {
             const uint64_t s = c + lane;
@@ -2457,6 +2547,7 @@
             const unsigned long long m = __ballot(hit);
             if (m) {
                 const uint64_t sb = c + (uint64_t)(__ffsll((long long)m) - 1);
+                bestRun = sb;
                 bestFirst = sStart[sb];
                 bestSecond = sStart[sb + 1];
                 break;
@@ -2571,7 +2662,7 @@
     }
     if (lane != 0) return;
     if (nTc < 0) {
-        nTc = filter_redundant_serial(M, bestFirst, bestSecond, gScan, gStart, dnaShift, tax, tc);
+        nTc = filter_redundant_serial(M, bestFirst, bestSecond, runGroup[bestRun], gStart, dnaShift, tax, tc);
     } else {
         for (long a = 1; a < nTc; a++) {
             mtb_taxcnt v = tc[a];
@@ -2603,9 +2694,9 @@
 __global__ void __launch_bounds__(256) k_choose_taxon_group(const mtb_match* __restrict__ M,
                                                             const uint64_t* __restrict__ mOff,
                                                             const uint32_t* __restrict__ qlen, uint32_t nReads,
-                                                            const uint64_t* __restrict__ sScan,
+                                                            const uint64_t* __restrict__ runOff,
                                                             const uint64_t* __restrict__ sStart,
-                                                            const uint64_t* __restrict__ gScan,
+                                                            const uint64_t* __restrict__ runGroup,
                                                             const uint64_t* __restrict__ gStart,
                                                             const float* __restrict__ spScore,
                                                             const uint8_t* __restrict__ spKeep, AssignCfg cfg,
@@ -2628,9 +2719,9 @@
     float spTotal = 0.0f;
     int32_t bestTax = 0;
     bool isLCA = false, filter = false;
-    uint64_t bestFirst = 0, bestSecond = 0;
+    uint64_t bestFirst = 0, bestSecond = 0, bestRun = 0;
     if (n > 0) {
-        const uint64_t s0 = sScan[base], s1 = sScan[base + n];
+        const uint64_t s0 = runOff[r], s1 = runOff[r + 1];
         long meaningful = 0;
         float bestSpScore = 0.0f;
         for (uint64_t s = s0 + gl; s < s1; s += kGroupLanes) {
@@ -2648,7 +2739,8 @@
                 const uint32_t m = (uint32_t)(__ballot(hit) >> gLane0) & 0xFFFFu;
                 if (m) {
                     const uint64_t sb = c + (uint64_t)(__ffs((int)m) - 1);
-                    bestFirst = sStart[sb];
+                    bestRun = sb;
+                bestFirst = sStart[sb];
                     bestSecond = sStart[sb + 1];
                     break;
                 }
@@ -2775,7 +2867,7 @@
         return;
     }
     if (nTc < 0) {
-        nTc = filter_redundant_serial(M, bestFirst, bestSecond, gScan, gStart, dnaShift, tax, tc);
+        nTc = filter_redundant_serial(M, bestFirst, bestSecond, runGroup[bestRun], gStart, dnaShift, tax, tc);
     } else {
         for (long a = 1; a < nTc; a++) {
             mtb_taxcnt v = tc[a];
@@ -2816,12 +2908,13 @@
     AssignCfg cfg{a.kmerFormat, a.dnaShift, a.maxCodonShift, a.denominator, a.minConsCnt, a.minConsCntEuk,
                   a.accessionLevel, a.minScore, a.minSpScore, a.tieRatio, a.generic, a.emulateAll, a.em};
     TaxView tv{t.nodeOf, t.nodeTax, t.parent, t.depth, t.flags, t.spParent, t.maxTax};
+    exclusive_scan_u32(s.grpCnt, nReads, s.grpOff, s.scanTmp, st);
+    exclusive_scan_u32(s.runCnt, nReads, s.runOff, s.scanTmp, st);
     if (nM) {
-        launch_run_index(matches, nM, reinterpret_cast<uint8_t*>(s.gFlag),
-                         reinterpret_cast<unsigned long long*>(s.sFlag), s.gScan, s.sScan, s.gStart, s.sStart, st);
+        launch_run_starts(s.runFlag, mOff, s.grpOff, s.runOff, nReads, s.gStart, s.sStart, s.runGroup, st);
         uint64_t cnt[2] = {0, 0};
-        hipMemcpyAsync(&cnt[0], s.gScan + nM, sizeof(uint64_t), hipMemcpyDeviceToHost, st);
-        hipMemcpyAsync(&cnt[1], s.sScan + nM, sizeof(uint64_t), hipMemcpyDeviceToHost, st);
+        hipMemcpyAsync(&cnt[0], s.grpOff + nReads, sizeof(uint64_t), hipMemcpyDeviceToHost, st);
+        hipMemcpyAsync(&cnt[1], s.runOff + nReads, sizeof(uint64_t), hipMemcpyDeviceToHost, st);
         hipStreamSynchronize(st);
         hostStats[0] = cnt[0];
         hostStats[2] = cnt[1];
@@ -2838,29 +2931,36 @@
                 if (waves) hipMemsetAsync(s.waveCount, 0, sizeof(uint32_t), st);
                 const char* nl = getenv("MTB_PATHS_NOLDS");
                 const int nlw = nl ? atoi(nl) : 0;
-#define MTB_PATHS(L, W)                                                                                             \
-    k_match_paths<L, W><<<(unsigned)((heavy + 63) / 64), 64, 0, st>>>(                                              \
+                const char* la = getenv("MTB_K6_LOOKAHEAD");
+                const bool look = !la || atoi(la) != 0;
+#define MTB_PATHS(L, W, A)                                                                                          \
+    k_match_paths<L, W, A><<<(unsigned)((heavy + 63) / 64), 64, 0, st>>>(                                              \
         matches, s.gStart, inB ? s.ordKB : s.ordKA, heavy, cfg, tv, (Path*)s.local, (Path*)s.paths, s.conn,         \
         s.pathCnt, waves ? s.waveList : nullptr, s.waveCount)
-                if (nlw == 6) MTB_PATHS(false, 6);
-                else if (nlw == 5) MTB_PATHS(false, 5);
-                else if (nlw == 4) MTB_PATHS(false, 4);
-                else MTB_PATHS(true, 1);
+                if (nlw == 6) MTB_PATHS(false, 6, false);
+                else if (nlw == 5) MTB_PATHS(false, 5, false);
+                else if (nlw == 4 && look) MTB_PATHS(false, 4, true);
+                else if (nlw == 4) MTB_PATHS(false, 4, false);
+                else if (look) MTB_PATHS(true, 1, true);
+                else MTB_PATHS(true, 1, false);
 #undef MTB_PATHS
                 if (waves) {
                     uint32_t nBig = 0;
                     hipMemcpyAsync(&nBig, s.waveCount, sizeof(uint32_t), hipMemcpyDeviceToHost, st);
                     hipStreamSynchronize(st);
-                    if (nBig)
-                        k_match_paths_wave<<<nBig, 64, 0, st>>>(matches, s.gStart, s.waveList, cfg, tv, (Path*)s.local,
-                                                                (Path*)s.paths, s.conn, s.pathCnt);
+                    if (nBig && look)
+                        k_match_paths_wave<true><<<nBig, 64, 0, st>>>(matches, s.gStart, s.waveList, cfg, tv, (Path*)s.local,
+                                                                      (Path*)s.paths, s.conn, s.pathCnt);
+                    else if (nBig)
+                        k_match_paths_wave<false><<<nBig, 64, 0, st>>>(matches, s.gStart, s.waveList, cfg, tv, (Path*)s.local,
+                                                                       (Path*)s.paths, s.conn, s.pathCnt);
                 }
             }
         }
         if (cnt[1]) {
             hipMemsetAsync(s.waveCount, 0, sizeof(uint32_t), st);
             k_combine_paths<<<(unsigned)((cnt[1] + 255) / 256), 256, 0, st>>>(
-                matches, s.sStart, cnt[1], s.gScan, s.gStart, s.pathCnt, qlen, cfg, (Path*)s.paths, (Path*)s.comb,
+                matches, s.sStart, cnt[1], s.runGroup, s.gStart, s.pathCnt, qlen, cfg, (Path*)s.paths, (Path*)s.comb,
                 s.spScore, s.spKeep, s.waveList, s.waveCount);
             uint32_t nWave = 0;
             hipMemcpyAsync(&nWave, s.waveCount, sizeof(uint32_t), hipMemcpyDeviceToHost, st);
@@ -2873,25 +2973,23 @@
             }
             hostStats[3] = nWave;
         }
-    } else {
-        hipMemsetAsync(s.sScan, 0, sizeof(uint64_t), st);
     }
     const bool wave = a.waveTaxon >= 0 ? a.waveTaxon == 1 : (!a.generic && nM > (uint64_t)kWavePerReadMatches * nReads);
     const bool group = a.waveTaxon == 2 || (a.waveTaxon < 0 && !wave && !a.generic);
     if (group) {
-        k_choose_taxon_group<<<(nReads + 15) / 16, 256, 0, st>>>(matches, mOff, qlen, nReads, s.sScan, s.sStart,
-                                                                 s.gScan, s.gStart, s.spScore, s.spKeep, cfg, tv,
+        k_choose_taxon_group<<<(nReads + 15) / 16, 256, 0, st>>>(matches, mOff, qlen, nReads, s.runOff, s.sStart,
+                                                                 s.runGroup, s.gStart, s.spScore, s.spKeep, cfg, tv,
                                                                  (Clade*)s.clade, s.cladePerMatch, tcPool, results);
     } else if (wave) {
         k_read_size_keys<<<(nReads + 255) / 256, 256, 0, st>>>(mOff, nReads, s.ordKA);
         const uint64_t* order = longest_first(nReads, 24, s, st);
-        k_choose_taxon_wave<<<nReads, 64, 0, st>>>(matches, mOff, qlen, nReads, s.sScan, s.sStart, s.gScan, s.gStart,
+        k_choose_taxon_wave<<<nReads, 64, 0, st>>>(matches, mOff, qlen, nReads, s.runOff, s.sStart, s.runGroup, s.gStart,
                                                    s.spScore, s.spKeep, cfg, tv, (Clade*)s.clade, s.cladePerMatch,
                                                    tcPool, results, order);
     } else {
         const unsigned ctT = nReads < 256u * 256u ? 64u : 256u;
-        k_choose_taxon<<<(nReads + ctT - 1) / ctT, ctT, 0, st>>>(matches, mOff, qlen, nReads, s.sScan, s.sStart,
-                                                             s.gScan, s.gStart, s.spScore, s.spKeep, cfg, tv,
+        k_choose_taxon<<<(nReads + ctT - 1) / ctT, ctT, 0, st>>>(matches, mOff, qlen, nReads, s.runOff, s.sStart,
+                                                             s.runGroup, s.gStart, s.spScore, s.spKeep, cfg, tv,
                                                              (Clade*)s.clade, s.cladePerMatch, tcPool, results);
     }
 }
@@ -2962,7 +3060,7 @@
 };
 
 __global__ void k_em_top(const mtb_match* __restrict__ M, const uint64_t* __restrict__ mOff, uint32_t n,
-                         const uint64_t* __restrict__ sScan, const uint64_t* __restrict__ sStart,
+                         const uint64_t* __restrict__ runOff, const uint64_t* __restrict__ sStart,
                          const float* __restrict__ spScore, const uint8_t* __restrict__ spKeep,
                          const mtb_result* __restrict__ results, EmPair* __restrict__ scratch,
                          EmPair* __restrict__ maps, uint8_t* __restrict__ cnt) {
@@ -2970,8 +3068,7 @@
     if (r >= n) return;
     cnt[r] = 0;
     if (!results[r].is_classified) return;
-    const uint64_t base = mOff[r], end = mOff[r + 1];
-    const uint64_t s0 = sScan[base], s1 = sScan[end];
+    const uint64_t s0 = runOff[r], s1 = runOff[r + 1];
     EmPair* v = scratch + s0;
     long k = 0;
     for (uint64_t s = s0; s < s1; s++)
@@ -2985,7 +3082,7 @@
 void launch_em_top(const mtb_match* M, const uint64_t* mOff, uint32_t n, const AssignScratch& s,
                    const mtb_result* results, void* scratch, void* maps, uint8_t* cnt, hipStream_t st) {
     if (!n) return;
-    k_em_top<<<(n + 255) / 256, 256, 0, st>>>(M, mOff, n, s.sScan, s.sStart, s.spScore, s.spKeep, results,
+    k_em_top<<<(n + 255) / 256, 256, 0, st>>>(M, mOff, n, s.runOff, s.sStart, s.spScore, s.spKeep, results,
                                               (EmPair*)scratch, (EmPair*)maps, cnt);
 }
 
diff --git a/metabuli_work_amd/csrc/mtb_kernels.hip b/metabuli_work_amd/csrc/mtb_kernels.hip
--- a/metabuli_work_amd/csrc/mtb_kernels.hip
+++ b/metabuli_work_amd/csrc/mtb_kernels.hip
@@ -102,98 +102,44 @@
 
 uint64_t scan_tmp_elems(uint64_t n) { return (n + kScanTile - 1) / kScanTile + 1; }
 
-constexpr int kRunItems = 32;
-constexpr int kRunTile = kBlock * kRunItems;
-
-__global__ void __launch_bounds__(256) k_run_tiles(const mtb_match* __restrict__ M, uint64_t nM,
-                                                   uint8_t* __restrict__ flags, unsigned long long* __restrict__ tileSum) {
-    const uint64_t base = (uint64_t)blockIdx.x * kRunTile;
-    unsigned long long s = 0;
-#pragma unroll 8
-    for (int k = 0; k < kRunItems; k++) {
-        const uint64_t i = base + (uint64_t)k * kBlock + threadIdx.x;
-        if (i >= nM) break;
-        uint32_t g = 1, sp = 1;
-        if (i > 0) {
-            const uint64_t qa = M[i - 1].qinfo, qb = M[i].qinfo;
-            const bool newSp = info_seq(qa) != info_seq(qb) || M[i - 1].species_id != M[i].species_id;
-            sp = newSp;
-            g = newSp || info_frame(qa) != info_frame(qb);
-        }
-        flags[i] = (uint8_t)(g | sp << 1);
-        s += (unsigned long long)g | (unsigned long long)sp << 32;
-    }
-    unsigned long long tot;
-    block_exclusive_scan(s, &tot);
-    if (threadIdx.x == 0) tileSum[blockIdx.x] = tot;
-}
-
-__global__ void __launch_bounds__(256) k_run_index(const uint8_t* __restrict__ flags, uint64_t nM,
-                                                   const unsigned long long* __restrict__ tileSum,
-                                                   uint64_t* __restrict__ gScan, uint64_t* __restrict__ sScan,
-                                                   uint64_t* __restrict__ gStart, uint64_t* __restrict__ sStart) {
-    __shared__ uint32_t sIdx[kRunTile];
-    __shared__ uint8_t sF[kRunTile];
-    const uint64_t base = (uint64_t)blockIdx.x * kRunTile;
-    const uint32_t nT = (uint32_t)min<uint64_t>(kRunTile, nM - base);
-    const int tid = threadIdx.x;
-    if (nT == kRunTile) {
-        const uint4* src = reinterpret_cast<const uint4*>(flags + base);
-        uint4* dst = reinterpret_cast<uint4*>(sF);
-        for (int x = tid; x < kRunTile / 16; x += kBlock) dst[x] = src[x];
-    } else {
-        for (uint32_t x = tid; x < nT; x += kBlock) sF[x] = flags[base + x];
-    }
-    __syncthreads();
-    uint32_t f[kRunItems];
-    unsigned long long s = 0;
-#pragma unroll
-    for (int k = 0; k < kRunItems; k++) {
-        const uint32_t x = (uint32_t)tid * kRunItems + k;
-        f[k] = x < nT ? sF[x] : 0u;
-        s += (unsigned long long)(f[k] & 1u) | (unsigned long long)(f[k] >> 1) << 32;
-    }
-    unsigned long long tot;
-    const unsigned long long ex = block_exclusive_scan(s, &tot);
-    const unsigned long long tb = tileSum[blockIdx.x];
-    const uint64_t gBase = tb & 0xFFFFFFFFull, sBase = tb >> 32;
-#pragma unroll
-    for (int kind = 0; kind < 2; kind++) {
-        uint32_t run = kind ? (uint32_t)(ex >> 32) : (uint32_t)ex;
-#pragma unroll
-        for (int k = 0; k < kRunItems; k++) {
-            sIdx[tid * kRunItems + k] = run;
-            run += (f[k] >> kind) & 1u;
-        }
-        __syncthreads();
-        uint64_t* scan = kind ? sScan : gScan;
-        uint64_t* start = kind ? sStart : gStart;
-        const uint64_t b0 = kind ? sBase : gBase;
-        for (uint32_t x = tid; x < nT; x += kBlock) {
-            const uint64_t v = b0 + sIdx[x];
-            scan[base + x] = v;
-            if ((sF[x] >> kind) & 1u) start[v] = base + x;
-        }
-        __syncthreads();
-    }
-    if (blockIdx.x == gridDim.x - 1 && tid == 0) {
-        const unsigned long long all = tileSum[gridDim.x];
-        gScan[nM] = all & 0xFFFFFFFFull;
-        sScan[nM] = all >> 32;
-        gStart[all & 0xFFFFFFFFull] = nM;
-        sStart[all >> 32] = nM;
-    }
-}
-
-uint64_t run_index_tmp_bytes(uint64_t nM) { return 8 * ((nM + kRunTile - 1) / kRunTile + 2); }
-
-void launch_run_index(const mtb_match* M, uint64_t nM, uint8_t* flags, unsigned long long* tileSum, uint64_t* gScan,
-                      uint64_t* sScan, uint64_t* gStart, uint64_t* sStart, hipStream_t s) {
-    if (nM == 0) return;
-    const uint64_t tiles = (nM + kRunTile - 1) / kRunTile;
-    k_run_tiles<<<(unsigned)tiles, kBlock, 0, s>>>(M, nM, flags, tileSum);
-    k_scan_tile_sums<<<1, kBlock, 0, s>>>(tileSum, tiles);
-    k_run_index<<<(unsigned)tiles, kBlock, 0, s>>>(flags, nM, tileSum, gScan, sScan, gStart, sStart);
+__global__ void __launch_bounds__(256) k_run_starts(const uint8_t* __restrict__ flags, const uint64_t* __restrict__ mOff,
+                                                    const uint64_t* __restrict__ grpOff,
+                                                    const uint64_t* __restrict__ runOff, uint32_t nReads,
+                                                    uint64_t* __restrict__ gStart, uint64_t* __restrict__ sStart,
+                                                    uint64_t* __restrict__ runGroup) {
+    const uint32_t r = blockIdx.x * 4 + threadIdx.x / 64;
+    const uint32_t lane = threadIdx.x & 63;
+    if (r >= nReads) return;
+    const uint64_t lo = mOff[r], live = mOff[r + 1] - lo;
+    const uint64_t g0 = grpOff[r], s0 = runOff[r];
+    const uint64_t gN = grpOff[r + 1] - g0, sN = runOff[r + 1] - s0;
+    const unsigned long long below = (1ull << lane) - 1;
+    uint64_t jg = 0, js = 0;
+    for (uint64_t e0 = 0; e0 < live; e0 += 64) {
+        const uint64_t e = e0 + lane;
+        const uint32_t f = e < live ? flags[lo + e] : 0u;
+        const unsigned long long mg = __ballot(f & 1u), ms = __ballot(f & 2u);
+        const uint64_t g = jg + __popcll(mg & below);
+        if ((f & 1u) && g < gN) gStart[g0 + g] = lo + e;
+        if (f & 2u) {
+            const uint64_t s = js + __popcll(ms & below);
+            if (s < sN) {
+                sStart[s0 + s] = lo + e;
+                runGroup[s0 + s] = g0 + g;
+            }
+        }
+        jg += __popcll(mg);
+        js += __popcll(ms);
+    }
+    if (r == nReads - 1 && lane == 0) {
+        gStart[grpOff[nReads]] = mOff[nReads];
+        sStart[runOff[nReads]] = mOff[nReads];
+    }
+}
+
+void launch_run_starts(const uint8_t* flags, const uint64_t* mOff, const uint64_t* grpOff, const uint64_t* runOff,
+                       uint32_t nReads, uint64_t* gStart, uint64_t* sStart, uint64_t* runGroup, hipStream_t s) {
+    if (nReads) k_run_starts<<<(nReads + 3) / 4, 256, 0, s>>>(flags, mOff, grpOff, runOff, nReads, gStart, sStart, runGroup);
 }
 void exclusive_scan_u32(const uint32_t* in, uint64_t n, uint64_t* out, void* tmp, hipStream_t s) {
     scan_impl<uint32_t>(in, n, out, (unsigned long long*)tmp, s);
diff --git a/metabuli_work_amd/csrc/mtb_launch.h b/metabuli_work_amd/csrc/mtb_launch.h
--- a/metabuli_work_amd/csrc/mtb_launch.h
+++ b/metabuli_work_amd/csrc/mtb_launch.h
@@ -50,8 +50,12 @@
     void* paths;
     void* comb;
     uint8_t* conn;
-    uint32_t *gFlag, *sFlag, *pathCnt;
-    uint64_t *gScan, *sScan, *gStart, *sStart;
+    uint32_t* pathCnt;
+    uint64_t *gStart, *sStart;
+    uint64_t* runGroup;
+    const uint8_t* runFlag;
+    const uint32_t *grpCnt, *runCnt;
+    uint64_t *grpOff, *runOff;
     float* spScore;
     uint64_t* waveList;
     uint32_t* waveCount;
@@ -73,9 +77,8 @@
     for (uint64_t i = (uint64_t)blockIdx.x * blockDim.x + threadIdx.x; i < (n); i += (uint64_t)gridDim.x * blockDim.x)
 void exclusive_scan_u32(const uint32_t* in, uint64_t n, uint64_t* out, void* tmp, hipStream_t s);
 void exclusive_scan_u64(const uint64_t* in, uint64_t n, uint64_t* out, void* tmp, hipStream_t s);
-uint64_t run_index_tmp_bytes(uint64_t nM);
-void launch_run_index(const mtb_match* M, uint64_t nM, uint8_t* flags, unsigned long long* tileSum, uint64_t* gScan,
-                      uint64_t* sScan, uint64_t* gStart, uint64_t* sStart, hipStream_t s);
+void launch_run_starts(const uint8_t* flags, const uint64_t* mOff, const uint64_t* grpOff, const uint64_t* runOff,
+                       uint32_t nReads, uint64_t* gStart, uint64_t* sStart, uint64_t* runGroup, hipStream_t s);
 
 void launch_read_meta(const uint64_t* off1, const uint64_t* off2, uint32_t n, int paired, ReadMeta* meta,
                       uint32_t* qlen, uint32_t* maxW, uint32_t* readLens, hipStream_t s);
@@ -270,8 +273,8 @@
     const int need = d <= 1 ? 1 : 1 + (d - 1 + sh - 1) / sh;
     return (uint32_t)(need < 2 ? 2 : need);
 }
-void launch_pack_live(const mtb_match* in, const uint64_t* mOff, const uint64_t* liveOff, uint32_t nReads,
-                      mtb_match* out, int* err, hipStream_t s);
+void launch_run_flags(const mtb_match* in, const uint64_t* mOff, const uint64_t* liveOff, uint32_t nReads,
+                      mtb_match* out, uint8_t* flags, uint32_t* grpCnt, uint32_t* runCnt, int* err, hipStream_t s);
 void launch_max_u32(const uint32_t* x, uint32_t n, uint32_t* out, hipStream_t s);
 void launch_max_seg(const uint64_t* off, uint32_t n, uint32_t* out, hipStream_t s);
 constexpr uint32_t kSegSortLds = 8192;
```

After: 34.13 million (median of 6 runs). +2.5%, better.
